# Kotstantinovskiy/SonicDiffusionBayesLab

Hardware: AMD Instinct MI355X
Metric: 512x512 images/sec at 50 DDIM steps (higher is better)
Workload: dtype bf16; 1 GPU; SD-1.5 512x512 DDIM 50 steps, CFG 7.5, batch=8/GPU (BASELINE configs[1]); global_batch=8, sample_size=64, parallelism=batch-shard x1, weights=SD-1.5-shaped synthetic seed 1234

## Files before the change

include/sd_hip.h:

```cpp
#ifndef SD_HIP_H
#define SD_HIP_H

#ifdef __cplusplus
extern "C" {
#endif

typedef struct sd_unet sd_unet;

typedef struct sd_unet_config {
    int sample_size;
    int in_channels;
    int out_channels;
    int num_levels;
    int block_out_channels[8];
    int layers_per_block;
    int attn_levels[8];
    int cross_attention_dim;
    int num_heads;
    int norm_num_groups;
    float norm_eps;
    int context_len;
    int weight_dtype;
    float fp8_act_scale_norm;
    float fp8_act_scale_ff;
// ... 26 lines not shown
long long sd_unet_workspace_bytes(sd_unet* u, int unet_batch, int cache_branch_id);

long long sd_unet_workspace_bytes_hw(sd_unet* u, int unet_batch, int cache_branch_id, int latent_h, int latent_w);

int sd_unet_set_context(sd_unet* u, void* stream, const float* encoder_hidden_states, int unet_batch,
                        int cache_branch_id, void* workspace, long long workspace_bytes);
int sd_unet_set_context_hw(sd_unet* u, void* stream, const float* encoder_hidden_states, int unet_batch,
                           int cache_branch_id, int latent_h, int latent_w, void* workspace, long long workspace_bytes);

int sd_unet_set_timestep_cond(sd_unet* u, void* stream, const float* cond);

int sd_unet_set_inpaint_cond_hw(sd_unet* u, void* stream, const float* mask, const float* masked_latents, int batch,
                                int latent_h, int latent_w);

int sd_unet_set_ip_adapter_hw(sd_unet* u, void* stream, const float* image_embeds, int unet_batch, int cache_branch_id,
                              int latent_h, int latent_w, float scale, void* workspace, long long workspace_bytes);

int sd_controlnet_create(const sd_unet_config* cfg, const int cond_embed_channels[4], sd_unet** out);
long long sd_controlnet_residual_bytes_hw(const sd_unet* u, int unet_batch, int latent_h, int latent_w);
int sd_controlnet_set_cond_hw(sd_unet* u, void* stream, const float* cond_image, int batch, int latent_h, int latent_w);
int sd_controlnet_forward_hw(sd_unet* u, void* stream, const float* latents, int latent_batch, int unet_batch, int latent_h,
                             int latent_w, float timestep, void* residuals, void* workspace, long long workspace_bytes);
int sd_unet_set_control_residuals_hw(sd_unet* u, const void* residuals, float scale, int unet_batch, int latent_h, int latent_w);

int sd_unet_set_tome(sd_unet* u, double ratio, int max_downsample);
int sd_unet_tome_block_count_hw(sd_unet* u, int latent_h, int latent_w);
int sd_unet_tome_block_info_hw(sd_unet* u, int block, int latent_h, int latent_w, int* h, int* w, int* r, long long* choice_off);
int sd_unet_set_tome_choice_hw(sd_unet* u, void* stream, const unsigned char* choice, long long n, int latent_h, int latent_w);
int sd_unet_tome_matching_hw(sd_unet* u, void* stream, int block, int unet_batch, int cache_branch_id, void* workspace, int* kept,
                             int* merged, int* dst_idx, int* tok, int* r, int* batch);

enum { SD_CACHE_OFF = 0, SD_CACHE_FULL_AND_STORE = 1, SD_CACHE_SKIP = 2 };

int sd_unet_forward(sd_unet* u, void* stream, const float* latents, int latent_batch, int unet_batch,
                    float timestep, float* eps_out, void* workspace, long long workspace_bytes, int cache_mode,
                    int cache_branch_id);
int sd_unet_forward_hw(sd_unet* u, void* stream, const float* latents, int latent_batch, int unet_batch, int latent_h,
                       int latent_w, float timestep, float* eps_out, void* workspace, long long workspace_bytes,
                       int cache_mode, int cache_branch_id);

typedef struct sd_unet sd_vae;
int sd_vae_create(const sd_unet_config* cfg, sd_vae** out);
int sd_vae_decode(sd_vae* v, void* stream, const float* latents, int batch, float latent_scale, float* images_out,
                  void* workspace, long long workspace_bytes);
int sd_vae_decode_hw(sd_vae* v, void* stream, const float* latents, int batch, int latent_h, int latent_w, float latent_scale,
                     float* images_out, void* workspace, long long workspace_bytes);

int sd_vae_encoder_create(const sd_unet_config* cfg, sd_vae** out);
int sd_vae_encode_hw(sd_vae* v, void* stream, const float* images, int batch, int latent_h, int latent_w, float* moments_out,
                     void* workspace, long long workspace_bytes);
int sd_vae_posterior_sample(void* stream, const float* moments, const float* noise_or_null, float scale, float* latents_out,
                            int batch, long long hw);

typedef struct sd_unet sd_taesd;
int sd_taesd_decoder_create(sd_taesd** out);
int sd_taesd_encoder_create(sd_taesd** out);
int sd_taesd_decode_hw(sd_taesd* v, void* stream, const float* latents, int batch, int latent_h, int latent_w, int out_mode,
                       float* images_out, void* workspace, long long workspace_bytes);
int sd_taesd_encode_hw(sd_taesd* v, void* stream, const float* images01, int batch, int latent_h, int latent_w, float* latents_out,
                       void* workspace, long long workspace_bytes);
int sd_op_conv64(void* stream, const void* X, const void* Wpacked, const float* bias, const void* R, void* Y, int B, int Hin,
                 int Win, int mode, int relu);
long long sd_op_conv64_pack(const float* w_oihw, void* out);
int sd_op_taesd_entry(void* stream, const float* x, const float* Wt, const float* bias, void* y, int B, int H, int W, int Cin,
                      int decoder);
int sd_op_taesd_exit(void* stream, const void* x, const void* Wp, const float* bias, float* y, int B, int H, int W, int Cout,
// ... 152 lines not shown
                    float eps);
int sd_op_tome_match(void* stream, const void* x, const unsigned char* choice, int B, int h, int w, int C, float* node_max,
                     int* node_idx, int* tok);
int sd_op_tome_select(void* stream, const float* node_max, const int* node_idx, int B, int num_src, int r, int* kept, int* merged,
                      int* dst_idx);
int sd_op_tome_merge(void* stream, const void* x, const int* tok, const int* kept, const int* merged, const int* dst_idx, void* out,
                     long long ldo, int B, int h, int w, int C, int r);
int sd_op_tome_unmerge(void* stream, const void* y, long long ldy, const void* residual, const int* tok, const int* kept,
                       const int* merged, const int* dst_idx, void* out, int B, int h, int w, int C, int r);
int sd_op_attention(void* stream, const void* Q, long long ldq, const void* K, long long ldk, const void* V,
                    long long ldv, void* O, long long ldo, int B, int heads, int Nq, int Nk, int D, float scale);
int sd_op_gemm_qkv_headmajor(void* stream, const void* X, long long ldx, const void* W, void* Q, void* KV, int M, int C,
                             int tokens, int K);
int sd_op_attention_headmajor(void* stream, const void* Q, long long ldq, const void* K, const void* V, void* O,
                              long long ldo, int B, int heads, int Nq, int Nk, int D, float scale);
int sd_op_clip_attention(void* stream, const void* qkv, void* out, int B, int L, int H, int heads);
int sd_op_vit_attention(void* stream, const void* qkv, void* out, int B, int L, int H, int heads);
int sd_op_bert_attention(void* stream, const void* q, long long ldq, const void* k, const void* v, long long ldkv,
                         const int* mask, void* out, long long ldo, int B, int heads, int Lq, int Lk);
int sd_op_reward_head(void* stream, const void* hidden, long long row_stride, const float* w, const float* bias, float mean,
                      float std, int B, int H, float* rewards, float* features);
int sd_op_clip_preprocess(void* stream, const unsigned char* images, int B, int H, int W, int S, int P, unsigned char* crop,
                          void* patches);
int sd_op_conv_in(void* stream, const float* x, int Bsrc, const float* Wt, const float* bias, void* y, int B, int H,
                  int W, int Cin, int Cout);
int sd_op_conv_in_cond(void* stream, const float* x, int Bsrc, const float* cond, int Bcond, const float* Wt,
                       const float* bias, void* y, int B, int H, int W, int Cout);
int sd_op_conv_in_add(void* stream, const float* x, int Bsrc, const void* addend, int Badd, const float* Wt, const float* bias,
                      void* y, int B, int H, int W, int Cout);
int sd_op_residual_add(void* stream, void* x, const long long* dst_off, const void* r, const long long* src_off,
                       const long long* count, int nseg, float scale);
int sd_op_conv_out(void* stream, const void* x, const void* Wp, const float* bias, float* y, int B, int H, int W,
                   int Cin, int Cout);
int sd_op_time_embedding(void* stream, float t, const void* W1, const float* b1, const void* W2, const float* b2,
                         float* scratch, float* temb, int dim_in, int dim);
int sd_op_timestep_cond(void* stream, float t, const float* cond, const void* Wc, float* row, float* emb, int cond_dim,
                        int dim);

int sd_op_ln_partials(int kind, int M, int N);
int sd_op_gemm_rowstats(void* stream, const void* X, long long ldx, const void* W, const float* bias, const void* R,
                        long long ldr, void* C, long long ldc, int M, int N, int K, float* rowstats);
int sd_op_gemm_ln(void* stream, const void* X, long long ldx, const void* Wg, const float* c1, const float* c2,
                  const float* rowstats, int parts, float eps, void* C, long long ldc, int M, int N, int K, int epi);
int sd_op_gemm_plan(void* stream, const void* X, long long ldx, const void* X2, long long ldx2, int K1, const void* W,
                    const float* bias, const float* bias2, const void* R, long long ldr, void* C, long long ldc, int M, int N,
                    int K, float* rowstats, float* stats, const float* ln_rs, int ln_parts, const float* ln_c1, float ln_eps,
                    void* KV, int hm_tokens);
int sd_op_xattn_fused_rowstats(void* stream, const void* X, const void* R, void* Y, const void* At, const void* Bw,
                               const float* bias, int M, int C, int rows_per_sample, int L, float* rowstats);
int sd_op_ip_xattn(void* stream, const void* R, void* Rout, const void* A, const void* Bt, const float* gamma, const float* beta,
                   float eps, long long M, int C, int rows_per_sample, int heads, int T);
int sd_op_xattn_fused(void* stream, const void* X, const void* R, void* Y, const void* At, const void* Bw,
                      const float* bias, int M, int C, int rows_per_sample, int L);
int sd_op_xattn_fused_ln(void* stream, const void* X, const void* R, void* Y, const void* At, const void* Bw,
                         const float* bias, int M, int C, int rows_per_sample, int L, const float* ln_rowstats, int ln_parts,
                         long long ln_rows, const float* c2, float eps, float* rowstats);
int sd_op_conv3x3_ablate(void* stream, const void* X, const void* W, void* Y, int B, int Hin, int Win, int Cin, int Cout,
                         int ablate);
int sd_op_xattn_fused_stamps(void* stream, const void* X, const void* R, void* Y, const void* At, const void* Bw,
                             const float* bias, int M, int C, int rows_per_sample, int L, unsigned long long* stamps);

int sd_op_gemm_fp8(void* stream, const void* X, long long ldx, const void* W, const float* wscale, float xscale,
                   const float* bias, const void* R, long long ldr, void* C, long long ldc, int M, int N, int K, int epi,
                   int out_fp8, float oscale);
int sd_op_conv3x3_fp8(void* stream, const void* X, const void* W, const float* wscale, float xscale, const float* bias,
                      const float* bias2, const void* R, void* Y, int B, int Hin, int Win, int Cin, int Cout, int stride,
// ... 13 lines not shown
```

sonicdiffusionbayeslab_amd/_lib.py:

```python
from __future__ import annotations

import ctypes as C
import os
import re
from typing import Optional

HERE = os.path.dirname(os.path.abspath(__file__))
LIB_PATH = os.environ.get("SD_AMD_LIB", os.path.join(HERE, "lib", "libsdhip.so"))
HEADER_PATH = os.path.normpath(os.path.join(HERE, "..", "include", "sd_hip.h"))

ABLATE_LIB_PATH = os.path.join(HERE, "lib", "libsdhip_ablate.so")

_lib: Optional[C.CDLL] = None
_ablate: Optional[C.CDLL] = None


class SdUnetConfig(C.Structure):
    _fields_ = [
        ("sample_size", C.c_int), ("in_channels", C.c_int), ("out_channels", C.c_int),
        ("num_levels", C.c_int), ("block_out_channels", C.c_int * 8), ("layers_per_block", C.c_int),
        ("attn_levels", C.c_int * 8), ("cross_attention_dim", C.c_int), ("num_heads", C.c_int),
        ("norm_num_groups", C.c_int), ("norm_eps", C.c_float), ("context_len", C.c_int),
        ("weight_dtype", C.c_int), ("fp8_act_scale_norm", C.c_float), ("fp8_act_scale_ff", C.c_float),
        ("time_cond_proj_dim", C.c_int),
# ... 36 lines not shown
        ("intermediate_size", C.c_int), ("max_positions", C.c_int), ("layer_norm_eps", C.c_float), ("hidden_act", C.c_int),
        ("position_embedding_absolute", C.c_int), ("max_text_len", C.c_int), ("reward_mean", C.c_float), ("reward_std", C.c_float),
    ]


class SdHipError(RuntimeError):
    pass


def declared_symbols() -> list:
    src = open(HEADER_PATH).read()
    src = re.sub(r"/\*.*?\*/", "", src, flags=re.S)
    return sorted(set(re.findall(r"\b(sd_[a-z0-9_]+)\s*\(", src)))


_vp, _i, _ll, _f = C.c_void_p, C.c_int, C.c_longlong, C.c_float
_SIGS = {
    "sd_last_error": (C.c_char_p, []),
    "sd_abi_version": (_i, []),
    "sd_unet_create": (_i, [C.POINTER(SdUnetConfigFull), C.POINTER(_vp)]),
    "sd_unet_destroy": (None, [_vp]),
    "sd_unet_num_params": (_i, [_vp]),
    "sd_unet_param_info": (_i, [_vp, _i, C.c_char_p, _i, C.POINTER(_ll), C.POINTER(_i)]),
    "sd_unet_load_param": (_i, [_vp, C.c_char_p, _vp, _ll]),
    "sd_unet_finalize": (_i, [_vp]),
    "sd_unet_debug_packed": (_ll, [_vp, C.c_char_p, _vp, _ll]),
    "sd_unet_calibrate_fp8": (_i, [_vp, _vp, _vp, _i, _i, _f, _f, _vp, _ll]),
    "sd_unet_fp8_scale_count": (_i, [_vp]),
    "sd_unet_fp8_scale_info": (_i, [_vp, _i, C.c_char_p, _i, C.POINTER(_f), C.POINTER(_f)]),
    "sd_unet_set_fp8_scale": (_i, [_vp, C.c_char_p, _f]),
    "sd_unet_workspace_bytes": (_ll, [_vp, _i, _i]),
    "sd_unet_set_context": (_i, [_vp, _vp, _vp, _i, _i, _vp, _ll]),
    "sd_unet_set_timestep_cond": (_i, [_vp, _vp, _vp]),
    "sd_unet_forward": (_i, [_vp, _vp, _vp, _i, _i, _f, _vp, _vp, _ll, _i, _i]),
    "sd_unet_workspace_bytes_hw": (_ll, [_vp, _i, _i, _i, _i]),
    "sd_unet_set_context_hw": (_i, [_vp, _vp, _vp, _i, _i, _i, _i, _vp, _ll]),
    "sd_unet_forward_hw": (_i, [_vp, _vp, _vp, _i, _i, _i, _i, _f, _vp, _vp, _ll, _i, _i]),
    "sd_unet_forward_profiled": (_i, [_vp, _vp, _vp, _i, _i, _f, _vp, _vp, _ll, _i, _i, C.POINTER(C.c_double),
                                      C.POINTER(_ll), C.POINTER(C.c_double), C.POINTER(C.c_double)]),
    "sd_unet_forward_op_times": (_ll, [_vp, _vp, _vp, _i, _i, _f, _vp, _vp, _ll, _i, _i, C.c_char_p, _ll]),
    "sd_vae_create": (_i, [C.POINTER(SdUnetConfigFull), C.POINTER(_vp)]),
    "sd_vae_decode": (_i, [_vp, _vp, _vp, _i, _f, _vp, _vp, _ll]),
    "sd_vae_decode_hw": (_i, [_vp, _vp, _vp, _i, _i, _i, _f, _vp, _vp, _ll]),
    "sd_vae_encoder_create": (_i, [C.POINTER(SdUnetConfigFull), C.POINTER(_vp)]),
    "sd_vae_encode_hw": (_i, [_vp, _vp, _vp, _i, _i, _i, _vp, _vp, _ll]),
    "sd_vae_posterior_sample": (_i, [_vp, _vp, _vp, _f, _vp, _i, _ll]),
    "sd_taesd_decoder_create": (_i, [C.POINTER(_vp)]),
    "sd_taesd_encoder_create": (_i, [C.POINTER(_vp)]),
    "sd_taesd_decode_hw": (_i, [_vp, _vp, _vp, _i, _i, _i, _i, _vp, _vp, _ll]),
    "sd_taesd_encode_hw": (_i, [_vp, _vp, _vp, _i, _i, _i, _vp, _vp, _ll]),
    "sd_op_conv64": (_i, [_vp, _vp, _vp, _vp, _vp, _vp, _i, _i, _i, _i, _i]),
    "sd_op_conv64_pack": (_ll, [_vp, _vp]),
    "sd_op_taesd_entry": (_i, [_vp, _vp, _vp, _vp, _vp, _i, _i, _i, _i, _i]),
    "sd_op_taesd_exit": (_i, [_vp, _vp, _vp, _vp, _vp, _i, _i, _i, _i, _i]),
    "sd_clip_create": (_i, [C.POINTER(SdClipConfig), C.POINTER(_vp)]),
    "sd_clip_encode": (_i, [_vp, _vp, _vp, _i, _vp, _vp, _ll]),
    "sd_clip_create_projected": (_i, [C.POINTER(SdClipConfig), _i, _i, C.POINTER(_vp)]),
    "sd_clip_text_embeds_workspace_bytes": (_ll, [_vp, _i]),
    "sd_clip_text_embeds": (_i, [_vp, _vp, _vp, _i, _vp, _vp, _ll]),
    "sd_clip_vision_create": (_i, [C.POINTER(SdClipVisionConfig), C.POINTER(_vp)]),
    "sd_clip_vision_workspace_bytes": (_ll, [_vp, _i, _i, _i]),
    "sd_clip_vision_encode": (_i, [_vp, _vp, _vp, _i, _i, _i, _vp, _vp, _ll]),
    "sd_clip_score": (_i, [_vp, _vp, _vp, _i, _i, _vp, _vp]),
    "sd_image_reward_create": (_i, [C.POINTER(SdImageRewardConfig), C.POINTER(_vp)]),
    "sd_image_reward_workspace_bytes": (_ll, [_vp, _i, _i, _i]),
    "sd_image_reward_score": (_i, [_vp, _vp, _vp, _vp, _vp, _i, _i, _i, _i, _vp, _vp, _vp, _ll]),
# ... 29 lines not shown
    "sd_controlnet_create": (_i, [C.POINTER(SdUnetConfigFull), C.POINTER(_i), C.POINTER(_vp)]),
    "sd_controlnet_residual_bytes_hw": (_ll, [_vp, _i, _i, _i]),
    "sd_controlnet_set_cond_hw": (_i, [_vp, _vp, _vp, _i, _i, _i]),
    "sd_controlnet_forward_hw": (_i, [_vp, _vp, _vp, _i, _i, _i, _i, _f, _vp, _vp, _ll]),
    "sd_unet_set_control_residuals_hw": (_i, [_vp, _vp, _f, _i, _i, _i]),
    "sd_op_conv_in_add": (_i, [_vp, _vp, _i, _vp, _i, _vp, _vp, _vp, _i, _i, _i, _i]),
    "sd_op_residual_add": (_i, [_vp, _vp, _vp, _vp, _vp, _vp, _i, _f]),
    "sd_op_conv_in_cond": (_i, [_vp, _vp, _i, _vp, _i, _vp, _vp, _vp, _i, _i, _i, _i]),
    "sd_op_gemm": (_i, [_vp, _vp, _ll, _vp, _ll, _i, _vp, _vp, _vp, _vp, _ll, _vp, _ll, _i, _i, _i, _i]),
    "sd_op_gemm_tile_rows": (_i, [_i, _i, _i]),
    "sd_op_gemm_splitk": (_i, [_i, _i, _i, _i]),
    "sd_op_gemm_batched": (_i, [_vp, _vp, _ll, _vp, _ll, _i, _vp, _vp, _ll, _vp, _ll, _i, _i, _i, _i, _i]),
    "sd_op_gemm_batched_softmax_ln": (_i, [_vp, _vp, _ll, _vp, _ll, _i, _vp, _ll, _i, _i, _i, _i, _vp, _i, _vp, _vp, _f]),
    "sd_op_conv3x3": (_i, [_vp, _vp, _vp, _vp, _vp, _vp, _vp, _i, _i, _i, _i, _i, _i, _i]),
    "sd_op_conv3x3_shortcut": (_i, [_vp, _vp, _vp, _vp, _vp, _i, _vp, _i, _vp, _vp, _i, _i, _i, _i, _i]),
    "sd_op_conv3x3_shortcut_groupnorm": (_i, [_vp, _vp, _vp, _vp, _vp, _i, _vp, _i, _vp, _vp, _i, _i, _i, _i, _i,
                                              _vp, _vp, _vp, _i, _f, _i]),
    "sd_op_conv3x3_down_asym": (_i, [_vp, _vp, _vp, _vp, _vp, _i, _i, _i, _i, _i]),
    "sd_op_conv3x3_ablate": (_i, [_vp, _vp, _vp, _vp, _i, _i, _i, _i, _i, _i]),
    "sd_op_conv3x3_upsample_subpixel": (_i, [_vp, _vp, _vp, _vp, _vp, _i, _i, _i, _i, _i]),
    "sd_op_conv3x3_upsample_subpixel_groupnorm": (_i, [_vp, _vp, _vp, _vp, _vp, _i, _i, _i, _i, _i, _vp, _vp, _vp, _i, _f, _i]),
    "sd_op_groupnorm": (_i, [_vp, _vp, _i, _vp, _i, _vp, _vp, _vp, _i, _i, _i, _f, _i]),
    "sd_op_conv3x3_groupnorm": (_i, [_vp, _vp, _vp, _vp, _vp, _vp, _vp, _i, _i, _i, _i, _i, _vp, _vp, _vp, _i, _f, _i]),
    "sd_op_conv3x3_splitk": (_i, [_i, _i, _i, _i, _i, _i, _i]),
    "sd_op_conv3x3_kernel": (_i, [_i, _i, _i, _i, _i, _i, _i, _i]),
    "sd_op_softmax_rows": (_i, [_vp, _vp, _ll, _i, _f]),
    "sd_op_layernorm": (_i, [_vp, _vp, _vp, _vp, _vp, _i, _i, _f]),
    "sd_op_attention": (_i, [_vp, _vp, _ll, _vp, _ll, _vp, _ll, _vp, _ll, _i, _i, _i, _i, _i, _f]),
    "sd_op_gemm_qkv_headmajor": (_i, [_vp, _vp, _ll, _vp, _vp, _vp, _i, _i, _i, _i]),
    "sd_op_attention_headmajor": (_i, [_vp, _vp, _ll, _vp, _vp, _vp, _ll, _i, _i, _i, _i, _i, _f]),
    "sd_op_clip_attention": (_i, [_vp, _vp, _vp, _i, _i, _i, _i]),
    "sd_op_conv_in": (_i, [_vp, _vp, _i, _vp, _vp, _vp, _i, _i, _i, _i, _i]),
    "sd_op_conv_out": (_i, [_vp, _vp, _vp, _vp, _vp, _i, _i, _i, _i, _i]),
    "sd_op_time_embedding": (_i, [_vp, _f, _vp, _vp, _vp, _vp, _vp, _vp, _i, _i]),
    "sd_op_timestep_cond": (_i, [_vp, _f, _vp, _vp, _vp, _vp, _i, _i]),
    "sd_op_ln_partials": (_i, [_i, _i, _i]),
    "sd_op_gemm_rowstats": (_i, [_vp, _vp, _ll, _vp, _vp, _vp, _ll, _vp, _ll, _i, _i, _i, _vp]),
    "sd_op_gemm_plan": (_i, [_vp, _vp, _ll, _vp, _ll, _i, _vp, _vp, _vp, _vp, _ll, _vp, _ll, _i, _i, _i, _vp, _vp, _vp, _i, _vp, _f,
                            _vp, _i]),
    "sd_op_gemm_ln": (_i, [_vp, _vp, _ll, _vp, _vp, _vp, _vp, _i, _f, _vp, _ll, _i, _i, _i, _i]),
    "sd_op_xattn_fused_rowstats": (_i, [_vp, _vp, _vp, _vp, _vp, _vp, _vp, _i, _i, _i, _i, _vp]),
    "sd_op_xattn_fused": (_i, [_vp, _vp, _vp, _vp, _vp, _vp, _vp, _i, _i, _i, _i]),
    "sd_op_xattn_fused_ln": (_i, [_vp, _vp, _vp, _vp, _vp, _vp, _vp, _i, _i, _i, _i, _vp, _i, _ll, _vp, _f, _vp]),
    "sd_op_xattn_fused_stamps": (_i, [_vp, _vp, _vp, _vp, _vp, _vp, _vp, _i, _i, _i, _i, _vp]),
    "sd_op_gemm_fp8": (_i, [_vp, _vp, _ll, _vp, _vp, _f, _vp, _vp, _ll, _vp, _ll, _i, _i, _i, _i, _i, _f]),
    "sd_op_conv3x3_fp8": (_i, [_vp, _vp, _vp, _vp, _f, _vp, _vp, _vp, _vp, _i, _i, _i, _i, _i, _i, _i]),
    "sd_op_groupnorm_fp8": (_i, [_vp, _vp, _i, _vp, _i, _vp, _vp, _vp, _i, _i, _i, _f, _i, _i, _f]),
    "sd_op_layernorm_fp8": (_i, [_vp, _vp, _vp, _vp, _vp, _i, _i, _i, _f, _f]),
    "sd_op_quantize_fp8": (_i, [_vp, _vp, _vp, _ll, _i, _i, _f]),
    "sd_op_amax_e4m3": (_i, [_vp, _vp, _ll, _vp]),
    "sd_unet_set_tome": (_i, [_vp, C.c_double, _i]),
    "sd_unet_tome_block_count_hw": (_i, [_vp, _i, _i]),
    "sd_unet_tome_block_info_hw": (_i, [_vp, _i, _i, _i, C.POINTER(_i), C.POINTER(_i), C.POINTER(_i), C.POINTER(_ll)]),
    "sd_unet_set_tome_choice_hw": (_i, [_vp, _vp, _vp, _ll, _i, _i]),
    "sd_unet_tome_matching_hw": (_i, [_vp, _vp, _i, _i, _i, _vp, _vp, _vp, _vp, _vp, C.POINTER(_i), C.POINTER(_i)]),
    "sd_op_tome_match": (_i, [_vp, _vp, _vp, _i, _i, _i, _i, _vp, _vp, _vp]),
    "sd_op_tome_select": (_i, [_vp, _vp, _vp, _i, _i, _i, _vp, _vp, _vp]),
    "sd_op_tome_merge": (_i, [_vp, _vp, _vp, _vp, _vp, _vp, _vp, _ll, _i, _i, _i, _i, _i]),
    "sd_op_tome_unmerge": (_i, [_vp, _vp, _ll, _vp, _vp, _vp, _vp, _vp, _vp, _i, _i, _i, _i, _i]),
}


def load() -> C.CDLL:
    global _lib
    if _lib is not None:
        return _lib
# ... 42 lines not shown
```

sonicdiffusionbayeslab_amd/csrc/common.h:

```cpp
#pragma once
#include <hip/hip_runtime.h>
#include <stdint.h>

typedef unsigned short bf16_t;

typedef __attribute__((ext_vector_type(8))) short bf16x8;
typedef __attribute__((ext_vector_type(4))) short bf16x4;
typedef __attribute__((ext_vector_type(4))) float f32x4;
typedef __attribute__((ext_vector_type(16))) float f32x16;
typedef __attribute__((ext_vector_type(2))) __bf16 bf16x2_t;
typedef __attribute__((ext_vector_type(2))) float f32x2_t;
typedef __attribute__((ext_vector_type(4))) unsigned u32x4;
typedef __attribute__((ext_vector_type(2))) unsigned u32x2;

typedef __attribute__((ext_vector_type(8))) int i32x8;
typedef __attribute__((ext_vector_type(8))) unsigned u32x8;
__device__ __forceinline__ i32x8 cat_u32x4(u32x4 lo, u32x4 hi) {
    const u32x8 r = __builtin_shufflevector(lo, hi, 0, 1, 2, 3, 4, 5, 6, 7);
    return __builtin_bit_cast(i32x8, r);
}

#define LDS_PTR(p) ((__attribute__((address_space(3))) void*)(p))
#define GLB_PTR(p) ((const __attribute__((address_space(1))) void*)(p))

__device__ __forceinline__ float bf2f(bf16_t u) { return __builtin_bit_cast(float, (unsigned)u << 16); }
__device__ __forceinline__ float bflo(unsigned u) { return __builtin_bit_cast(float, u << 16); }
__device__ __forceinline__ float bfhi(unsigned u) { return __builtin_bit_cast(float, u & 0xffff0000u); }
__device__ __forceinline__ bf16_t f2bf(float f) {
    __bf16 b = (__bf16)f;
    return __builtin_bit_cast(bf16_t, b);
}
__device__ __forceinline__ unsigned pack2bf(float lo, float hi) {
    f32x2_t v = {lo, hi};
    bf16x2_t r = __builtin_convertvector(v, bf16x2_t);
    return __builtin_bit_cast(unsigned, r);
}

__device__ __forceinline__ unsigned pack4fp8(float a, float b, float c, float d) {
    a = __builtin_amdgcn_fmed3f(a, -448.f, 448.f); b = __builtin_amdgcn_fmed3f(b, -448.f, 448.f);
    c = __builtin_amdgcn_fmed3f(c, -448.f, 448.f); d = __builtin_amdgcn_fmed3f(d, -448.f, 448.f);
    const int r = __builtin_amdgcn_cvt_pk_fp8_f32(a, b, 0, false);
    return (unsigned)__builtin_amdgcn_cvt_pk_fp8_f32(c, d, r, true);
}

__device__ __forceinline__ void glds16(const void* gsrc, void* lds_wave_base) {
    __builtin_amdgcn_global_load_lds(GLB_PTR(gsrc), LDS_PTR(lds_wave_base), 16, 0, 0);
}

__device__ __forceinline__ float silu_f(float x) {
    return x * __builtin_amdgcn_rcpf(1.0f + __builtin_amdgcn_exp2f(-1.4426950408889634f * x));
}
__device__ __forceinline__ float gelu_erf_f(float x) {
    const float z = fabsf(x) * 0.70710678118654752f;
    const float t = __builtin_amdgcn_rcpf(__builtin_fmaf(0.47047f, z, 1.0f));
    const float poly = t * (0.3480242f + t * (-0.0958798f + t * 0.7478556f));
    const float e = __builtin_amdgcn_exp2f(z * z * -1.4426950408889634f);
    const float half_erfc = 0.5f * poly * e;
    const float phi = x < 0.f ? half_erfc : 1.0f - half_erfc;
    return x * phi;
}

__device__ __forceinline__ f32x2_t geglu_pair(f32x2_t value, f32x2_t gate) {
    constexpr float C = 4.35f;
    const f32x2_t xc = {__builtin_amdgcn_fmed3f(gate[0], -C, C), __builtin_amdgcn_fmed3f(gate[1], -C, C)};
    const f32x2_t t = xc * (1.0f / C);
    const f32x2_t u = t * t;
    auto k = [](float c) { return f32x2_t{c, c}; };
    f32x2_t p = __builtin_elementwise_fma(u, k(-8.173780021e-01f), k(4.634953387e+00f));
    p = __builtin_elementwise_fma(p, u, k(-1.175370409e+01f));
    p = __builtin_elementwise_fma(p, u, k(1.781238736e+01f));
    p = __builtin_elementwise_fma(p, u, k(-1.828480159e+01f));
    p = __builtin_elementwise_fma(p, u, k(1.371556223e+01f));
    p = __builtin_elementwise_fma(p, u, k(-7.893326951e+00f));
    p = __builtin_elementwise_fma(p, u, k(3.560156552e+00f));
    p = __builtin_elementwise_fma(p, u, k(-1.257849752e+00f));
    p = __builtin_elementwise_fma(p, u, k(3.989407778e-01f));
    const f32x2_t phi = __builtin_elementwise_fma(xc, p, k(0.5f));
    return value * gate * phi;
}

template <int SHR>
__device__ __forceinline__ float row_shr_add(float v) {
    const int sh = __builtin_amdgcn_update_dpp(0, __builtin_bit_cast(int, v), 0x110 + SHR, 0xf, 0xf, true);
    return v + __builtin_bit_cast(float, sh);
// ... 102 lines not shown
```

sonicdiffusionbayeslab_amd/csrc/kernels.h:

```cpp
#pragma once
#include <vector>

#include "common.h"

struct GemmArgs {
    const bf16_t* X = nullptr;
    long ldx = 0;
    const bf16_t* X2 = nullptr;
    long ldx2 = 0;
    int K1 = 0;
    const bf16_t* W = nullptr;
    long ldw = 0;
    const float* bias = nullptr;
    const float* bias2 = nullptr;
    const bf16_t* R = nullptr;
    long ldr = 0;
    bf16_t* C = nullptr;
    long ldc = 0;
    int M = 0, N = 0, K = 0;
    int Hin = 0, Win = 0, Cin = 0, Hout = 0, Wout = 0, stride = 1, up = 0;
    int asym = 0;
    int splitk = 1;
    float* slab = nullptr;
    int defer_reduce = 0;
// ... 46 lines not shown
    const float* bias = nullptr;
    const bf16_t* R = nullptr;
    bf16_t* Y = nullptr;
    int B = 0, Hin = 0, Win = 0;
    int mode = 0;
    int relu = 0;
    int Hout = 0, Wout = 0, tiles_y = 0, tiles_x = 0, ntiles = 0;
    unsigned xbytes = 0;
};
int sd_conv64_out_size(int in, int mode);
void sd_conv64_pack(const float* w_oihw , bf16_t* out);
int sd_launch_conv64(const Conv64Args& a, hipStream_t stream);
int sd_launch_taesd_entry(const float* x, const float* Wt, const float* bias, bf16_t* y, int B, int H, int W, int Cin, int decoder,
                          hipStream_t stream);
int sd_launch_taesd_exit(const bf16_t* x, const bf16_t* Wp, const float* bias, float* y, int B, int H, int W, int Cout, int out_mode,
                         hipStream_t stream);

struct GroupNormArgs {
    const bf16_t* x1 = nullptr; int C1 = 0;
    const bf16_t* x2 = nullptr; int C2 = 0;
    const float* gamma = nullptr; const float* beta = nullptr;
    bf16_t* y = nullptr;
    int out_fp8 = 0, Cpad = 0;
    float oscale = 1.0f;
    const float* stats1 = nullptr; const float* stats2 = nullptr;
    const float* slab = nullptr; int splitk = 0;
    const float* sbias = nullptr; const float* sbias2 = nullptr;
    const bf16_t* sR = nullptr; long sldr = 0;
    bf16_t* x1w = nullptr;
    float* partial = nullptr;
    int B = 0, HW = 0, groups = 32, nsplit = 0;
    float eps = 1e-5f;
    int silu = 0;
};
int sd_groupnorm_nsplit(int B, int HW);
bool sd_groupnorm_uses_small(int B, int HW, int C1, int C2, int groups);
bool sd_groupnorm_slab_ok(int B, int HW, int C1, int C2, int groups);
size_t sd_groupnorm_scratch_bytes(int B, int HW, int groups);
int sd_launch_groupnorm(const GroupNormArgs& a, hipStream_t stream);

int sd_launch_softmax_rows(bf16_t* s, long rows, int cols, float scale, hipStream_t stream);
int sd_launch_softmax_rows_long(bf16_t* s, long rows, int cols, float scale, hipStream_t stream);
int sd_launch_pqconv(const float* x, const float* W, const float* bias, float* y, int B, int HW, float in_scale,
                     hipStream_t stream);

int sd_launch_layernorm(const bf16_t* x, const float* gamma, const float* beta, bf16_t* y, int rows, int C,
                        float eps, hipStream_t stream);
int sd_launch_layernorm_fp8(const bf16_t* x, const float* gamma, const float* beta, void* y, int rows, int C, int Cpad,
                            float eps, float oscale, hipStream_t stream);
int sd_launch_amax_e4m3(const void* y, long nbytes, unsigned* out, hipStream_t stream);
int sd_launch_quantize_fp8(const bf16_t* x, void* y, long rows, int C, int Cpad, float scale, hipStream_t stream);

struct AttnArgs {
    const bf16_t* Q = nullptr; long ldq = 0;
    const bf16_t* K = nullptr; long ldk = 0;
    const bf16_t* V = nullptr; long ldv = 0;
    bf16_t* O = nullptr; long ldo = 0;
    int B = 0, heads = 0, Nq = 0, Nk = 0, D = 0;
    float scale = 0.f;
    const void* consts = nullptr;
    int kv_head_major = 0;
    int q_prescaled = 0;
    int xcd_order = 1;
};
int sd_launch_attention(const AttnArgs& a, hipStream_t stream);

int sd_launch_gemv(const float* x, const bf16_t* W, const float* b, float* y, int N, int K, int silu_in,
                   hipStream_t stream);
int sd_launch_timestep_sinusoid(float t, float* out, int dim, hipStream_t stream);
int sd_launch_timestep_sinusoid_row(float t, const float* row, float* out, int dim, hipStream_t stream);
int sd_launch_f32_to_bf16(const float* src, bf16_t* dst, long n, hipStream_t stream);
int sd_launch_transpose_bf16(const bf16_t* src, bf16_t* dst, int B, int R, int Cc, hipStream_t stream, int perm16 = 0);

int sd_launch_retile32(const bf16_t* src, bf16_t* dst, int B, int R, int K, int RT, hipStream_t stream);
int sd_launch_replicate(const void* src, void* dst, long bytes, int rep, hipStream_t stream);

int sd_tome_check(int h, int w, int C, const char* who);
int sd_launch_tome_partition(const unsigned char* choice, int h, int w, int* tok, hipStream_t stream);
int sd_launch_tome_match(const bf16_t* x, const unsigned char* choice, int B, int h, int w, int C, float* node_max, int* node_idx,
                         int* tok, float* inv, hipStream_t stream);
int sd_launch_tome_select(const float* node_max, const int* node_idx, int B, int num_src, int r, int* kept, int* merged, int* dst_idx,
                          hipStream_t stream);
int sd_launch_tome_merge(const bf16_t* x, const int* tok, const int* kept, const int* merged, const int* dst_idx, bf16_t* out,
                         long ldo, int B, int h, int w, int C, int r, hipStream_t stream);
int sd_launch_tome_unmerge(const bf16_t* y, long ldy, const bf16_t* residual, const int* tok, const int* kept, const int* merged,
                           const int* dst_idx, bf16_t* out, int B, int h, int w, int C, int r, hipStream_t stream);

struct XattnArgs {
    const bf16_t* X = nullptr;
    const bf16_t* R = nullptr;
    bf16_t* Y = nullptr;
    const bf16_t* At = nullptr;
    const bf16_t* Bw = nullptr;
    const float* bias = nullptr;
    int M = 0, C = 0, rows_per_sample = 0, L = 0;
    float* rowstats = nullptr;
    const float* ln_rs = nullptr; int ln_np = 0; long ln_rows = 0;
    const float* ln_c2 = nullptr;
    float ln_eps = 1e-5f;
    unsigned long long* stamps = nullptr;
};
bool sd_xattn_fused_applicable(int rows_per_sample, int C, int heads, int L);
// ... 23 lines not shown
                        hipStream_t stream);
int sd_launch_vit_attention(const bf16_t* qkv, bf16_t* out, int B, int L, int H, int heads, hipStream_t stream);
int sd_launch_pool_rows(const bf16_t* src, const int* ids, int B, int L, int H, int eos_id, bf16_t* dst, hipStream_t stream);
int sd_launch_clip_score(const float* img, const float* txt, int B, int P, float* raw, float* score, hipStream_t stream);

int sd_bert_attention_check(int B, int Lq, int Lk, int heads);
int sd_bert_mask_check(const int* host_mask, int B, int Lk);
int sd_launch_bert_attention(const bf16_t* q, long ldq, const bf16_t* k, const bf16_t* v, long ldkv, const int* mask, bf16_t* out,
                             long ldo, int B, int heads, int Lq, int Lk, hipStream_t stream);
int sd_launch_reward_head(const bf16_t* hidden, long row_stride, const float* w, const float* wb, float mean, float stdv, int B,
                          int H, float* rewards, float* features, hipStream_t stream);

int sd_launch_conv_in(const float* x, int Bsrc, const float* Wt , const float* bias,
                      bf16_t* y, int B, int H, int W, int Cin, int Cout, hipStream_t stream);
int sd_launch_conv_in_cond(const float* x, int Bsrc, const float* cond, int Bcond, const float* Wt, const float* bias,
                           bf16_t* y, int B, int H, int W, int Cout, hipStream_t stream);
constexpr int SD_MAX_RES_SEGMENTS = 16;
int sd_launch_conv_in_add(const float* x, int Bsrc, const bf16_t* addend, int Badd, const float* Wt, const float* bias,
                          bf16_t* y, int B, int H, int W, int Cout, hipStream_t stream);
int sd_launch_residual_add(bf16_t* const* x, const bf16_t* const* r, const long* n, int nseg, float scale, hipStream_t stream);
int sd_launch_nchw_to_nhwc_bf16(const float* src, bf16_t* dst, int B, int C, long hw, hipStream_t stream);
int sd_launch_inpaint_cond_pack(const float* mask, const float* masked, float* cond, int B, long hw, hipStream_t stream);
int sd_launch_inpaint_prepare(const float* img, const float* mask, float* masked, float* lmask, int B, int H, int W,
                              hipStream_t stream);
int sd_launch_conv_in_image(const float* img, const float* Wt , const float* bias, bf16_t* y, int B, int H,
                            int W, int Cout, hipStream_t stream);
int sd_launch_vae_enc_out(const bf16_t* x, const bf16_t* Wp , const float* bias, const float* Wq ,
                          const float* bq, float* y, int B, int H, int W, int Cin, hipStream_t stream);
int sd_launch_vae_posterior(const float* moments, const float* noise, float scale, float* z, int B, int C, long hw,
                            hipStream_t stream);
int sd_launch_conv_out(const bf16_t* x, const bf16_t* Wp , const float* bias, float* y, int B,
                       int H, int W, int Cin, int Cout, hipStream_t stream);

struct StepCoef {
    float px, pe, p1, p2, pn;
    float yx, ye;
    float mx, me;
    float p3;
};
int sd_launch_sched_step(const float* eps, int cfg, float guidance, const float* x, const float* m1,
                         const float* m2, const float* m3, const float* noise, float* prev, float* y2, float* m_out,
                         StepCoef c, long n, hipStream_t stream);
int sd_launch_cfg_rescale_factors(const float* eps, int batch, long n_per_sample, float guidance, float rescale, float* k_out,
                                  hipStream_t stream);
int sd_launch_sched_step_rescaled(const float* eps, int cfg, float guidance, const float* x, const float* m1,
                                  const float* m2, const float* m3, const float* noise, float* prev, float* y2,
                                  float* m_out, StepCoef c, const float* k, long n_per_sample, long n, hipStream_t stream);
int sd_launch_sched_step_inpaint(const float* eps, int cfg, float guidance, const float* x, const float* m1,
                                 const float* m2, const float* m3, const float* noise, float* prev, float* y2,
                                 float* m_out, StepCoef c, const float* k, long n_per_sample, long n, const float* init,
                                 const float* blend_noise, const float* mask, float a, float s, long hw, hipStream_t stream);

int sd_launch_inception_conv(const bf16_t* x, const bf16_t* w, const float* bias, bf16_t* y, int B, int Hin, int Win, int Cin,
                             int Cout, int kh, int kw, int stride, int ph, int pw, int ldy, int coff, int relu ,
                             hipStream_t stream);
int sd_launch_inception_pool(const bf16_t* x, bf16_t* y, int B, int H, int W, int C, int stride, int pad, int avg, int ldy,
                             int coff, hipStream_t stream);
int sd_launch_inception_mean(const bf16_t* x, float* out, int B, int HW, int C, hipStream_t stream);
int sd_launch_inception_resize(const unsigned char* img, void* out, int B, int H, int W, int S, int out_fp32, hipStream_t stream);
```

sonicdiffusionbayeslab_amd/csrc/model.h:

```cpp
#pragma once
#include "../../include/sd_hip.h"
#include "common.h"
#include "kernels.h"

#include <stdlib.h>
#include <string.h>
#include <sys/mman.h>

#include <algorithm>
#include <map>
#include <new>
#include <set>
#include <string>
#include <tuple>
#include <unordered_map>
#include <vector>

namespace sdhip {

constexpr size_t NOFF = (size_t)-1;
constexpr int T_LATENTS = -2, T_EPS = -3;
constexpr int MAX_CONTROL_RES = SD_MAX_RES_SEGMENTS;

struct ParamSpec {
// ... 27 lines not shown
    size_t w = NOFF, b = NOFF, g = NOFF, be = NOFF;
    long b2idx = 0;
    int M = 0, N = 0, K = 0, K1 = 0, epi = 0;
    int B = 0, Hin = 0, Win = 0, Cin = 0, Hout = 0, Wout = 0, stride = 1, up = 0;
    int C1 = 0, C2 = 0, HW = 0, silu = 0, nsplit = 0;
    float eps = 0.f;
    int heads = 0, D = 0, Nq = 0, Nk = 0;
    long ldq = 0, ldk = 0, ldv = 0, ldo = 0, qoff = 0, koff = 0, voff = 0;
    int silu_in = 0, splitk = 1;
    int pool_by_ids = 0;
    int key_mask = 0;
    int defer = 0, slab_t = -1, slab_k = 0, slab_r = -1, slab_b2t = -1;
    size_t slab_b = NOFF;
    long slab_b2idx = 0;
    int wt = -1;
    size_t wx = NOFF;
    long xoff = 0, woff_el = 0, coff = 0, ldx_o = 0, ldw_o = 0, ldc_o = 0;
    float scale = 0.f;
    long wbs = 0;
    int rpb = 0, sm_valid = 0;
    int dt = 0, out_fp8 = 0, Cpad = 0, Kalg = 0;
    int sname = -1;
    int stats = -1, s1 = -1, s2 = -1;
    int subpix = 0;
    int asym = 0;
    int hm = 0;
    int qps = 0;
    int rs = -1, lnrs = -1, lnnp = 0;
    size_t c1 = NOFF;
    size_t wsc = NOFF;
    float xs = 1.f, os = 1.f;
    int scx1 = -1, scx2 = -1, scc1 = 0, scc2 = 0;
    size_t scw = NOFF;
    int nres = 0;
    int res_t[MAX_CONTROL_RES];
    int nwrap = 0;
    Wrap wraps[3];
};

struct HostBlob {
    unsigned char* p = nullptr;
    size_t n = 0, cap = 0;
    unsigned char* data() { return p; }
    const unsigned char* data() const { return p; }
    size_t size() const { return n; }
    bool empty() const { return n == 0; }
    bool reserve(size_t bytes) {
        if (bytes <= cap) return true;
        void* q = mmap(nullptr, bytes, PROT_READ | PROT_WRITE, MAP_PRIVATE | MAP_ANONYMOUS | MAP_POPULATE, -1, 0);
        if (q == MAP_FAILED) return false;
        (void)madvise(q, bytes, MADV_HUGEPAGE);
        if (p) { memcpy(q, p, n); munmap(p, cap); }
        p = (unsigned char*)q; cap = bytes;
        return true;
    }
    void resize(size_t bytes) {
        if (bytes > cap && !reserve(std::max(bytes, cap * 2))) throw std::bad_alloc();
        n = bytes;
    }
    void release() { if (p) munmap(p, cap); p = nullptr; n = cap = 0; }
    ~HostBlob() { release(); }
    HostBlob() = default;
    HostBlob(const HostBlob&) = delete;
    HostBlob& operator=(const HostBlob&) = delete;
};

struct Tn {
    size_t bytes = 0;
    int def = -1, last = -1;
    bool persistent = false;
    bool ctx = false;
    bool ctx_ip = false;
    size_t off = NOFF;
};

struct Plan {
    int UB = 0, branch = -1;
    int rep = 1;
    int lh = 0, lw = 0;
    int ip = 0;
    struct IpFold { int at, bt, C; size_t wqT, wo, wkv; int heads; };
    std::vector<IpFold> ip_fold;
    int ip_e = -1, ip_proj = -1, ip_tok = -1, ip_kv = -1;
    int cn = 0;
    std::vector<size_t> cn_off;
    std::vector<long> cn_count;
    struct TomeBlock { int tok, kept, merged, dst_idx, B, h, w, r; long choice_off; };
    std::vector<TomeBlock> tome;
    long tome_choice_bytes = 0;
    std::vector<Tn> tensors;
    std::vector<Op> ops;
    std::vector<char> skipped;
    std::vector<int> ctx_kv;
    std::vector<size_t> ctx_w;
    std::vector<int> ctx_c;
    int ctx_bf16 = -1;
    struct Fold { int kv, at, bw, C, heads; size_t wqT, wo; bool perm; int c2 = -1; size_t lnu = NOFF; int c1 = -1; size_t ones = NOFF; };
    std::vector<Fold> ctx_fold;
    int ctx_fold_scratch = -1;
    std::map<std::string, int> taps;
    size_t total_bytes = 0;
    ClipPrepGeom geom;
    std::vector<int> prep_tab;
    const int* dtab = nullptr;
};

}

struct sd_unet {
    int kind = 0;
    sd_unet_config cfg;
    sd_clip_config clip;
    sd_clip_vision_config vis;
    sd_image_reward_config ir;
    const int* ir_ids = nullptr;
    const int* ir_mask = nullptr;
    float* ir_features = nullptr;
    int text_proj = 0;
    int eos_id = -1;
    std::map<std::pair<int, int>, int*> prep_tabs;
    std::vector<sdhip::ParamSpec> params;
    std::unordered_map<std::string, int> pindex;
    std::unordered_map<std::string, size_t> woff;
    sdhip::HostBlob hblob;
    char* dweights = nullptr;
    bool finalized = false;
    bool debug_taps = false;
    bool fp8 = false;
    float s_norm = 8.f, s_ff = 2.f;
    std::vector<std::string> act_names;
    std::unordered_map<std::string, int> act_index;
    std::vector<float> act_scale, act_amax;
    int act_id(const std::string& name, float dflt) {
        auto it = act_index.find(name);
        if (it != act_index.end()) return it->second;
        act_index[name] = (int)act_names.size();
        act_names.push_back(name); act_scale.push_back(dflt); act_amax.push_back(0.f);
        return (int)act_names.size() - 1;
    }
    std::map<std::tuple<int, int, int, int, int, int, int, long long, int>, sdhip::Plan> plans;
    int last_rep = 1, last_ip = 0, last_cn = 0;
    int last_h = 0, last_w = 0;
    std::unordered_map<std::string, long> tproj_off;
    long tproj_total = 0;
    float* dcond = nullptr;
    bool cond_set = false;
    float* dinpaint = nullptr;
    size_t inpaint_cap = 0;
    int inpaint_b = 0, inpaint_h = 0, inpaint_w = 0;
    std::set<std::tuple<int, int, int, int>> ip_keys;
    const char* ctrl_res = nullptr;
    float ctrl_scale = 0.f;
    int ctrl_ub = 0, ctrl_h = 0, ctrl_w = 0;
    bool ctrl_enabled = false;
    bf16_t* cn_embed = nullptr;
    char* cn_scratch = nullptr;
    size_t cn_embed_cap = 0, cn_scratch_cap = 0;
    int cn_b = 0, cn_h = 0, cn_w = 0;
    int cond_embed[4] = {0, 0, 0, 0};
    double tome_ratio = 0.0;
    int tome_max_downsample = 0;
    unsigned char* tome_choice = nullptr;
    size_t tome_choice_cap = 0;
    long tome_choice_n = 0;
    bool unet_like() const { return kind == 0 || kind == 5; }
};

namespace sdhip {

inline int level_heads(const sd_unet_config& c, int level) {
    return c.num_heads_per_level[level] > 0 ? c.num_heads_per_level[level] : c.num_heads;
}
inline int block_heads(const sd_unet_config& c, const std::string& p) {
    if (p.compare(0, 12, "down_blocks.") == 0) return level_heads(c, atoi(p.c_str() + 12));
    if (p.compare(0, 10, "up_blocks.") == 0) return level_heads(c, c.num_levels - 1 - atoi(p.c_str() + 10));
    return level_heads(c, c.num_levels - 1);
}

void enumerate_params(sd_unet* u);
// ... 37 lines not shown
```

sonicdiffusionbayeslab_amd/csrc/norm.hip:

```cpp
#include "common.h"
#include "kernels.h"

#include <stdlib.h>

#include <algorithm>
#include <type_traits>

namespace {

struct GnGeom {
    int nchunks, rows_par, threads, cpg, C;
};

__host__ __device__ inline GnGeom gn_geom(int C, int groups) {
    GnGeom g;
    g.C = C;
    g.nchunks = C / 8;
    g.rows_par = g.nchunks >= 256 ? 1 : 256 / g.nchunks;
    const int act = g.rows_par * g.nchunks;
    g.threads = (act + 63) / 64 * 64;
    g.cpg = C / groups;
    return g;
}

// ... 97 lines not shown
    for (int i = tid; i < total; i += 256) {
        const int blk = i / cpg, c = gi * cpg + (i - blk * cpg);
        const long gb = (long)b * nblk + blk;
        const f32x2_t v = *(const f32x2_t*)(c < a.C1 ? a.stats1 + (gb * a.C1 + c) * 2 : a.stats2 + (gb * a.C2 + (c - a.C1)) * 2);
        s += v[0];
        q += v[1];
    }
    s = wave_sum(s);
    q = wave_sum(q);
    if (lane == 0) { red[wave * 2] = s; red[wave * 2 + 1] = q; }
    __syncthreads();
    if (tid == 0) {
        s = (red[0] + red[2]) + (red[4] + red[6]);
        q = (red[1] + red[3]) + (red[5] + red[7]);
        const float cnt = (float)a.HW * (float)cpg;
        const float mean = s / cnt;
        const float var = fmaxf(q / cnt - mean * mean, 0.f);
        float* st = a.partial + (long)a.B * a.nsplit * a.groups * 2 + (long)idx * 2;
        st[0] = mean;
        st[1] = rsqrtf(var + a.eps);
    }
}

template <bool SILU, bool FP8>
__global__ void gn_apply_kernel(const GroupNormArgs a) {
    const GnGeom g = gn_geom(a.C1 + a.C2, a.groups);
    const int tid = threadIdx.x;
    const int split = blockIdx.x, b = blockIdx.y;
    const bool active = tid < g.rows_par * g.nchunks;
    if (!active) return;
    const int prow = tid / g.nchunks, ch = tid - prow * g.nchunks;
    const int c0 = ch * 8;
    const float* st = a.partial + (long)a.B * a.nsplit * a.groups * 2 + (long)b * a.groups * 2;
    const int g0 = c0 / g.cpg, g1 = (c0 + 7) / g.cpg;
    const int nb = min(8, (g0 + 1) * g.cpg - c0);
    const float m0 = st[g0 * 2], r0 = st[g0 * 2 + 1], m1 = st[g1 * 2], r1 = st[g1 * 2 + 1];
    float sc[8], sf[8];
    {
        const f32x4 ga = *(const f32x4*)(a.gamma + c0), gb = *(const f32x4*)(a.gamma + c0 + 4);
        const f32x4 ba = *(const f32x4*)(a.beta + c0), bb = *(const f32x4*)(a.beta + c0 + 4);
#pragma unroll
        for (int j = 0; j < 8; ++j) {
            const float gm = j < 4 ? ga[j & 3] : gb[j & 3], bt = j < 4 ? ba[j & 3] : bb[j & 3];
            const float mean = j < nb ? m0 : m1, rstd = j < nb ? r0 : r1;
            sc[j] = rstd * gm;
            sf[j] = bt - mean * sc[j];
        }
    }
    const int per = (a.HW + a.nsplit - 1) / a.nsplit;
    const int pbeg = split * per, pend = min(a.HW, pbeg + per);
    auto apply = [&](const u32x4 v, long pix) {
        float f[8] = {bflo(v[0]), bfhi(v[0]), bflo(v[1]), bfhi(v[1]),
                      bflo(v[2]), bfhi(v[2]), bflo(v[3]), bfhi(v[3])};
#pragma unroll
        for (int j = 0; j < 8; ++j) {
            f[j] = f[j] * sc[j] + sf[j];
            if (SILU) f[j] = silu_f(f[j]);
        }
        if (FP8) {
            char* yr = (char*)a.y + pix * a.Cpad;
            const u32x2 o = {pack4fp8(f[0] * a.oscale, f[1] * a.oscale, f[2] * a.oscale, f[3] * a.oscale),
                             pack4fp8(f[4] * a.oscale, f[5] * a.oscale, f[6] * a.oscale, f[7] * a.oscale)};
            *(u32x2*)(yr + c0) = o;
            if (ch == g.nchunks - 1)
                for (int k = g.C; k < a.Cpad; k += 16) *(u32x4*)(yr + k) = u32x4{0u, 0u, 0u, 0u};
            return;
        }
        u32x4 o = {pack2bf(f[0], f[1]), pack2bf(f[2], f[3]), pack2bf(f[4], f[5]), pack2bf(f[6], f[7])};
        *(u32x4*)(a.y + pix * g.C + c0) = o;
    };
    const long base = (long)b * a.HW;
    const int rp = g.rows_par;
    int p = pbeg + prow;
    for (; p + 3 * rp < pend; p += 4 * rp) {
        const u32x4 v0 = *(const u32x4*)gn_src(a, base + p, c0);
        const u32x4 v1 = *(const u32x4*)gn_src(a, base + p + rp, c0);
        const u32x4 v2 = *(const u32x4*)gn_src(a, base + p + 2 * rp, c0);
        const u32x4 v3 = *(const u32x4*)gn_src(a, base + p + 3 * rp, c0);
        apply(v0, base + p); apply(v1, base + p + rp); apply(v2, base + p + 2 * rp); apply(v3, base + p + 3 * rp);
    }
    for (; p < pend; p += rp) apply(*(const u32x4*)gn_src(a, base + p, c0), base + p);
}

__device__ __forceinline__ float2 gn_unit_sums(const u32x2 v) {
    const float f0 = bflo(v[0]), f1 = bfhi(v[0]), f2 = bflo(v[1]), f3 = bfhi(v[1]);
    return make_float2((f0 + f1) + (f2 + f3), (f0 * f0 + f1 * f1) + (f2 * f2 + f3 * f3));
}
__device__ __forceinline__ void gn_mean_rstd(float ts, float tq, float cnt, float eps, float& mean, float& rstd) {
    mean = ts / cnt;
    rstd = rsqrtf(fmaxf(tq / cnt - mean * mean, 0.f) + eps);
}
template <bool SILU, bool FP8>
__device__ __forceinline__ void gn_unit_store(const GroupNormArgs& a, const u32x2 v, float mean, float rstd, long pix, int c, int C) {
    const f32x4 gm = *(const f32x4*)(a.gamma + c), bt = *(const f32x4*)(a.beta + c);
    float f[4] = {bflo(v[0]), bfhi(v[0]), bflo(v[1]), bfhi(v[1])};
#pragma unroll
    for (int jj = 0; jj < 4; ++jj) {
        f[jj] = (f[jj] - mean) * rstd * gm[jj] + bt[jj];
        if (SILU) f[jj] = silu_f(f[jj]);
    }
    if (FP8) {
        *(unsigned*)((char*)a.y + pix * a.Cpad + c) = pack4fp8(f[0] * a.oscale, f[1] * a.oscale, f[2] * a.oscale, f[3] * a.oscale);
// ... 400 lines not shown
    SD_REQUIRE(s && rows > 0, "softmax_rows: empty");
    SD_REQUIRE(cols % 8 == 0 && cols > 0 && cols <= 4096, "softmax_rows: cols=%d must be a multiple of 8 and <= 4096", cols);
    hipLaunchKernelGGL(softmax_rows_kernel, dim3((unsigned)((rows + 3) / 4)), dim3(256), 0, stream, s, rows, cols, scale);
    SD_CHECK_HIP(hipGetLastError());
    return 0;
}

size_t sd_groupnorm_scratch_bytes(int B, int HW, int groups) {
    return ((size_t)B * sd_groupnorm_nsplit(B, HW) * groups * 2 + (size_t)B * groups * 2) * sizeof(float);
}

int sd_groupnorm_nsplit(int B, int HW) {
    int n = (2048 + B - 1) / B;
    if (n > HW / 8) n = HW / 8;
    if (n < 1) n = 1;
    if (n > 256) n = 256;
    return n;
}

bool sd_groupnorm_uses_small(int B, int HW, int C1, int C2, int groups) {
    static const bool no_small = getenv("SD_GN_NO_SMALL") != nullptr;
    const int C = C1 + C2;
    return !no_small && HW <= 256 && (long)HW * (C / groups) <= 10240 && (C / groups) % 4 == 0 && C1 % 4 == 0 && B <= 65535;
}

bool sd_groupnorm_slab_ok(int B, int HW, int C1, int C2, int groups) {
    if (!sd_groupnorm_uses_small(B, HW, C1, C2, groups)) return false;
    const int cpg = (C1 + C2) / groups, G = cpg >= 80 ? 1 : 80 / cpg;
    return cpg >= 20 && cpg <= 80 && groups % G == 0 && C2 % 4 == 0 && (long)B * HW * C1 < (1L << 29);
}

int sd_launch_groupnorm(const GroupNormArgs& a, hipStream_t stream) {
    const int C = a.C1 + a.C2;
    SD_REQUIRE(a.x1 && a.y && a.gamma && a.beta && a.partial, "groupnorm: null operand");
    SD_REQUIRE(!a.out_fp8 || (a.Cpad >= C && a.Cpad % 128 == 0 && C % 16 == 0 && a.oscale > 0.f),
               "groupnorm fp8 out: Cpad=%d must be a multiple of 128 >= C=%d (C a multiple of 16)", a.Cpad, C);
    SD_REQUIRE(a.C1 % 8 == 0 && a.C2 % 8 == 0 && (a.C2 == 0 || a.x2), "groupnorm: C1=%d C2=%d must be multiples of 8", a.C1, a.C2);
    SD_REQUIRE(a.groups > 0 && a.groups <= 64 && C % a.groups == 0 && (C / a.groups >= 8 || C / a.groups == 4),
               "groupnorm: C=%d groups=%d needs C/groups >= 8 (or == 4)", C, a.groups);
    SD_REQUIRE(a.nsplit >= 1 && a.nsplit <= a.HW && a.B > 0 && a.HW > 0, "groupnorm: bad split %d for HW=%d", a.nsplit, a.HW);
    const GnGeom g = gn_geom(C, a.groups);
    SD_REQUIRE(g.threads <= 1024, "groupnorm: C=%d too wide", C);
    if (a.slab) {
        const int cpg = C / a.groups, G = cpg >= 80 ? 1 : 80 / cpg, ncol = G * (cpg / 4);
        SD_REQUIRE(a.splitk > 1 && a.splitk <= 64 && a.x1w && !a.out_fp8 && (!a.sR || a.sldr >= a.C1) && (a.C2 == 0 || a.x2),
                   "groupnorm with a deferred split-K reduce: splitk=%d, bf16 output, x1w and a residual stride >= C1", a.splitk);
        SD_REQUIRE(sd_groupnorm_slab_ok(a.B, a.HW, a.C1, a.C2, a.groups), "groupnorm with a deferred split-K reduce: HW=%d C=%d+%d "
                   "is not a shape gn_slab_kernel takes", a.HW, a.C1, a.C2);
        const dim3 grid(a.groups / G, a.B), blk((32 * ncol + 63) / 64 * 64);
        const size_t smem = ((size_t)G * a.HW * (cpg / 4) + 4 * G) * sizeof(float2);
        auto go = [&](auto kern) { hipLaunchKernelGGL(kern, grid, blk, smem, stream, a); };
        auto pick = [&](auto mi, auto un) {
            constexpr int MI = decltype(mi)::value, UN = decltype(un)::value;
            if (a.silu) go(gn_slab_kernel<true, MI, UN>); else go(gn_slab_kernel<false, MI, UN>);
        };
        using std::integral_constant;
        const int iters = (a.HW + 31) / 32, k = a.splitk;
        if (iters <= 2) {
            if (k % 8 == 0) pick(integral_constant<int, 2>{}, integral_constant<int, 8>{});
            else if (k % 4 == 0) pick(integral_constant<int, 2>{}, integral_constant<int, 4>{});
            else if (k % 2 == 0) pick(integral_constant<int, 2>{}, integral_constant<int, 2>{});
            else pick(integral_constant<int, 2>{}, integral_constant<int, 1>{});
        } else if (iters <= 4) {
            if (k % 4 == 0) pick(integral_constant<int, 4>{}, integral_constant<int, 4>{});
            else if (k % 2 == 0) pick(integral_constant<int, 4>{}, integral_constant<int, 2>{});
            else pick(integral_constant<int, 4>{}, integral_constant<int, 1>{});
        } else {
            if (k % 2 == 0) pick(integral_constant<int, 8>{}, integral_constant<int, 2>{});
            else pick(integral_constant<int, 8>{}, integral_constant<int, 1>{});
        }
        SD_CHECK_HIP(hipGetLastError());
        return 0;
    }
    if (sd_groupnorm_uses_small(a.B, a.HW, a.C1, a.C2, a.groups)) {
        const int units = (a.HW * (C / a.groups / 4) + 255) / 256;
        const dim3 grid(a.groups, a.B);
        auto go = [&](auto kern) { hipLaunchKernelGGL(kern, grid, dim3(256), 0, stream, a); };
        auto pick = [&](auto mu) {
            constexpr int MU = decltype(mu)::value;
            if (a.out_fp8) { if (a.silu) go(gn_small_kernel<true, true, MU>); else go(gn_small_kernel<false, true, MU>); }
            else { if (a.silu) go(gn_small_kernel<true, false, MU>); else go(gn_small_kernel<false, false, MU>); }
        };
        if (units <= 3) pick(std::integral_constant<int, 3>{});
        else if (units <= 5) pick(std::integral_constant<int, 5>{});
        else pick(std::integral_constant<int, 10>{});
        SD_CHECK_HIP(hipGetLastError());
        return 0;
    }
    dim3 grid(a.nsplit, a.B);
    if (a.stats1 != nullptr) {
        SD_REQUIRE(a.HW % 64 == 0 && (a.C2 == 0 || a.stats2 != nullptr), "groupnorm: producer statistics need HW %% 64 == 0 and both sources");
        hipLaunchKernelGGL(gn_finalize_stats_kernel, dim3(a.B * a.groups), dim3(256), 0, stream, a);
    } else {
        hipLaunchKernelGGL(gn_stats_kernel, grid, dim3(g.threads), (g.threads + g.nchunks) * sizeof(float4), stream, a);
        hipLaunchKernelGGL(gn_finalize_kernel, dim3((a.B * a.groups + 3) / 4), dim3(256), 0, stream, a);
    }
    if (a.out_fp8) {
        if (a.silu) hipLaunchKernelGGL((gn_apply_kernel<true, true>), grid, dim3(g.threads), 0, stream, a);
        else hipLaunchKernelGGL((gn_apply_kernel<false, true>), grid, dim3(g.threads), 0, stream, a);
    } else {
        if (a.silu) hipLaunchKernelGGL((gn_apply_kernel<true, false>), grid, dim3(g.threads), 0, stream, a);
        else hipLaunchKernelGGL((gn_apply_kernel<false, false>), grid, dim3(g.threads), 0, stream, a);
    }
    SD_CHECK_HIP(hipGetLastError());
    return 0;
}

static int launch_layernorm(const bf16_t* x, const float* gamma, const float* beta, bf16_t* y, int rows, int C, float eps,
                            bool fp8, int Cpad, float oscale, hipStream_t stream) {
    SD_REQUIRE(x && y && gamma && beta, "layernorm: null operand");
    SD_REQUIRE(C % 8 == 0 && C > 0 && C <= 1536, "layernorm: C=%d must be a multiple of 8 and <= 1536", C);
    SD_REQUIRE(rows > 0, "layernorm: no rows");
    SD_REQUIRE(!fp8 || (Cpad == (C + 127) / 128 * 128 && C % 16 == 0 && oscale > 0.f && Cpad - C <= 64 * 16),
               "layernorm fp8 out: Cpad=%d must be C=%d rounded up to 128 (C a multiple of 16)", Cpad, C);
    auto grouped = [&](auto kern, int lpr) {
        const int rows_per_block = 4 * (64 / lpr);
        hipLaunchKernelGGL(kern, dim3((rows + rows_per_block - 1) / rows_per_block), dim3(256), 0, stream, x, gamma, beta, y,
                           rows, eps, oscale);
    };
    if (fp8) {
        if (C == 320) grouped(layernorm_grouped_kernel<8, true>, 8);
        else if (C == 640) grouped(layernorm_grouped_kernel<16, true>, 16);
        else if (C == 1280) grouped(layernorm_grouped_kernel<32, true>, 32);
        else
            hipLaunchKernelGGL(layernorm_kernel<true>, dim3((rows + 3) / 4), dim3(256), 0, stream, x, gamma, beta, y, rows, C,
                               eps, Cpad, oscale);
    } else {
        if (C == 320) grouped(layernorm_grouped_kernel<8, false>, 8);
        else if (C == 640) grouped(layernorm_grouped_kernel<16, false>, 16);
// ... 38 lines not shown
```

sonicdiffusionbayeslab_amd/csrc/ops.hip:

```cpp
#include "model.h"

#include <stdlib.h>

namespace sdhip {

static void* g_scratch = nullptr;
static size_t g_scratch_bytes = 0;
void* op_scratch(size_t bytes) {
    if (bytes > g_scratch_bytes) {
        (void)hipDeviceSynchronize();
        if (g_scratch) (void)hipFree(g_scratch);
        g_scratch = nullptr;
        g_scratch_bytes = 0;
        if (hipMalloc(&g_scratch, bytes) != hipSuccess) return nullptr;
        g_scratch_bytes = bytes;
    }
    return g_scratch;
}

}

using namespace sdhip;

static void conv3x3_args(GemmArgs& a, const void* X, const void* W, const float* bias, const float* bias2, const void* R, void* Y,
// ... 410 lines not shown
                                  const float* bias, void* y, int B, int H, int W, int Cout) {
    return sd_launch_conv_in_cond(x, Bsrc, cond, Bcond, Wt, bias, (bf16_t*)y, B, H, W, Cout, (hipStream_t)stream);
}

extern "C" int sd_op_conv_in_add(void* stream, const float* x, int Bsrc, const void* addend, int Badd, const float* Wt,
                                 const float* bias, void* y, int B, int H, int W, int Cout) {
    return sd_launch_conv_in_add(x, Bsrc, (const bf16_t*)addend, Badd, Wt, bias, (bf16_t*)y, B, H, W, Cout, (hipStream_t)stream);
}

extern "C" int sd_op_residual_add(void* stream, void* x, const long long* dst_off, const void* r, const long long* src_off,
                                  const long long* count, int nseg, float scale) {
    SD_REQUIRE(x && r && dst_off && src_off && count, "sd_op_residual_add: null argument");
    SD_REQUIRE(nseg >= 1 && nseg <= MAX_CONTROL_RES, "sd_op_residual_add: %d segments (1 .. %d)", nseg, MAX_CONTROL_RES);
    bf16_t* xs[MAX_CONTROL_RES];
    const bf16_t* rs[MAX_CONTROL_RES];
    long n[MAX_CONTROL_RES];
    for (int k = 0; k < nseg; ++k) {
        SD_REQUIRE(dst_off[k] >= 0 && src_off[k] >= 0 && count[k] > 0, "sd_op_residual_add: segment %d", k);
        xs[k] = (bf16_t*)x + dst_off[k]; rs[k] = (const bf16_t*)r + src_off[k]; n[k] = (long)count[k];
    }
    return sd_launch_residual_add(xs, rs, n, nseg, scale, (hipStream_t)stream);
}

extern "C" int sd_op_conv_in(void* stream, const float* x, int Bsrc, const float* Wt, const float* bias, void* y, int B,
                             int H, int W, int Cin, int Cout) {
    return sd_launch_conv_in(x, Bsrc, Wt, bias, (bf16_t*)y, B, H, W, Cin, Cout, (hipStream_t)stream);
}

extern "C" int sd_op_conv_out(void* stream, const void* x, const void* Wp, const float* bias, float* y, int B, int H,
                              int W, int Cin, int Cout) {
    return sd_launch_conv_out((const bf16_t*)x, (const bf16_t*)Wp, bias, y, B, H, W, Cin, Cout, (hipStream_t)stream);
}

extern "C" int sd_op_time_embedding(void* stream, float t, const void* W1, const float* b1, const void* W2,
                                    const float* b2, float* scratch, float* temb, int dim_in, int dim) {
    int rc;
    if ((rc = sd_launch_timestep_sinusoid(t, scratch, dim_in, (hipStream_t)stream))) return rc;
    if ((rc = sd_launch_gemv(scratch, (const bf16_t*)W1, b1, scratch + dim_in, dim, dim_in, 0, (hipStream_t)stream))) return rc;
    return sd_launch_gemv(scratch + dim_in, (const bf16_t*)W2, b2, temb, dim, dim, 1, (hipStream_t)stream);
}

extern "C" int sd_op_timestep_cond(void* stream, float t, const float* cond, const void* Wc, float* row, float* emb,
                                   int cond_dim, int dim) {
    SD_REQUIRE(cond && Wc && row && emb, "timestep_cond: null operand");
    SD_REQUIRE(((uintptr_t)cond & 15) == 0 && cond_dim > 0, "timestep_cond: cond must be 16-byte aligned, cond_dim > 0");
    int rc;
    if ((rc = sd_launch_gemv(cond, (const bf16_t*)Wc, nullptr, row, dim, cond_dim, 0, (hipStream_t)stream))) return rc;
    return sd_launch_timestep_sinusoid_row(t, row, emb, dim, (hipStream_t)stream);
}

extern "C" int sd_op_gemm_fp8(void* stream, const void* X, long long ldx, const void* W, const float* wscale, float xscale,
                              const float* bias, const void* R, long long ldr, void* C, long long ldc, int M, int N, int K,
                              int epi, int out_fp8, float oscale) {
    if (ensure_zero_page()) return -2;
    SD_REQUIRE(epi == 0 || epi == 1, "sd_op_gemm_fp8: epi %d (0 = std, 1 = GEGLU)", epi);
    SD_REQUIRE(xscale > 0.f && (!out_fp8 || (epi == 1 && oscale > 0.f)), "sd_op_gemm_fp8: bad scales / fp8 output needs the GEGLU epilogue");
    GemmArgs a;
    a.X = (const bf16_t*)X; a.ldx = ldx; a.K1 = K; a.W = (const bf16_t*)W; a.bias = bias; a.R = (const bf16_t*)R; a.ldr = ldr;
    a.C = (bf16_t*)C; a.ldc = ldc; a.M = M; a.N = N; a.K = K; a.zero_page = zero_page();
    a.dt = 1; a.wscale = wscale; a.xscale_inv = 1.0f / xscale; a.out_fp8 = out_fp8; a.oscale = oscale;
    a.splitk = epi ? 1 : op_gemm_splitk(M, N, K, 1);
    if (splitk_slab(a, "sd_op_gemm_fp8")) return -1;
    return sd_launch_gemm(a, epi, (hipStream_t)stream);
}

extern "C" int sd_op_conv3x3_fp8(void* stream, const void* X, const void* W, const float* wscale, float xscale,
// ... 119 lines not shown
```

sonicdiffusionbayeslab_amd/csrc/plan.hip:

```cpp
#include "model.h"

#include <stdlib.h>

namespace sdhip {

namespace {

struct Builder {
    sd_unet* u;
    Plan& pl;
    int UB;
    std::vector<Wrap> wrapstack;
    std::map<int, int> stats_of;
    std::map<int, float> tscale;
    static std::string stem(const std::string& key) {
        const size_t n = key.rfind(".weight");
        return n == std::string::npos ? key : key.substr(0, n);
    }
    std::string error;
    float xscale(int t) {
        auto it = tscale.find(t);
        if (it == tscale.end()) {
            if (error.empty()) error = "fp8 consumer of a tensor without a scale";
            return 1.0f;
// ... 34 lines not shown
    int ctx_tensor(size_t bytes) {
        const int id = tensor(bytes, true);
        pl.tensors[id].ctx = true;
        return id;
    }
    int ctx_ip_tensor(size_t bytes) {
        const int id = ctx_tensor(bytes);
        pl.tensors[id].ctx_ip = true;
        return id;
    }
    int tensor(size_t bytes, bool persistent = false) {
        Tn t;
        t.bytes = (bytes + 255) / 256 * 256;
        t.persistent = persistent;
        pl.tensors.push_back(t);
        return (int)pl.tensors.size() - 1;
    }
    size_t W(const std::string& k) {
        auto it = u->woff.find(k);
        if (it == u->woff.end()) {
            if (error.empty()) error = "missing packed weight " + k;
            return 0;
        }
        return it->second;
    }
    Op& push(Op op) {
        op.nwrap = (int)wrapstack.size();
        for (int i = 0; i < op.nwrap; ++i) op.wraps[i] = wrapstack[i];
        pl.ops.push_back(op);
        return pl.ops.back();
    }
    static int pad128(int c) { return (c + 127) / 128 * 128; }
    int gn(int x1, int c1, int x2, int c2, int hw, const std::string& g, const std::string& b, float eps, int silu,
           bool fq = false) {
        Op o; o.kind = OP_GN; o.x1 = x1; o.C1 = c1; o.x2 = x2; o.C2 = c2; o.HW = hw; o.B = UB;
        o.g = W(g); o.be = W(b); o.eps = eps; o.silu = silu;
        o.nsplit = sd_groupnorm_nsplit(UB, hw);
        o.aux = tensor(sd_groupnorm_scratch_bytes(UB, hw, u->cfg.norm_num_groups));
        if (hw % 64 == 0 && !sd_groupnorm_uses_small(UB, hw, c1, c2, u->cfg.norm_num_groups) && stats_of.count(x1) &&
            (x2 < 0 || stats_of.count(x2))) {
            o.s1 = stats_of[x1];
            o.s2 = x2 >= 0 ? stats_of[x2] : -1;
        }
        if (fq) {
            o.out_fp8 = 1; o.Cpad = pad128(c1 + c2); o.sname = u->act_id(stem(g), u->s_norm); o.os = u->act_scale[o.sname];
            o.out = tensor((size_t)UB * hw * o.Cpad); tscale[o.out] = o.os;
        } else o.out = tensor((size_t)UB * hw * (c1 + c2) * 2);
        push(o);
        return o.out;
    }
    int conv3(int x, int hin, int win, int cin, int cout, int stride, int up, const std::string& w, const std::string& b,
              long b2idx, int b2t, int r, bool fq = false) {
        Op o; o.kind = OP_CONV3; o.x1 = x; o.B = UB; o.Hin = hin; o.Win = win; o.Cin = cin; o.N = cout;
        o.stride = stride; o.up = up;
        o.Hout = ((hin << up) + 2 - 3) / stride + 1;
        o.Wout = ((win << up) + 2 - 3) / stride + 1;
        o.M = UB * o.Hout * o.Wout; o.K = 9 * cin; o.Kalg = o.K;
        o.b = W(b); o.b2t = b2t; o.b2idx = b2idx; o.r = r;
        if (fq) { o.dt = 1; o.Cin = pad128(cin); o.K = 9 * o.Cin; o.w = W(w + ".fp8"); o.wsc = W(w + ".scale"); o.xs = xscale(x); }
        else o.w = W(w);
        static const bool subpix_off = getenv("SD_CONV_SUBPIXEL") && atoi(getenv("SD_CONV_SUBPIXEL")) == 0;
        if (up && !fq && !subpix_off && u->kind == 0 && stride == 1 && r < 0 && b2t < 0 && (hin * win) % 64 == 0 &&
            u->woff.count(w + ".sub")) {
            o.subpix = 1; o.K = 4 * cin; o.Kalg = 4 * cin;
            o.w = W(w + ".sub"); o.splitk = 1;
            o.out = tensor((size_t)o.M * cout * 2);
            if ((hin * win) % 128 == 0) want_stats(o, o.M, cout);
            push(o);
            return o.out;
        }
        o.splitk = sd_conv3x3_splitk(o.M, o.N, o.Cin, hin, win, stride, up, o.dt);
        if (o.splitk > 1) o.aux = tensor((size_t)o.splitk * o.M * o.N * 4);
        o.out = tensor((size_t)o.M * cout * 2);
        GemmArgs g;
        g.M = o.M; g.N = o.N; g.Cin = o.Cin; g.K = o.K; g.ldw = o.K; g.Hin = hin; g.Win = win; g.Hout = o.Hout; g.Wout = o.Wout;
        g.stride = stride; g.up = up; g.dt = o.dt;
        if (sd_conv_halo_mode(g) != 2) want_stats(o, o.M, cout);
        push(o);
        return o.out;
    }
    int gemm(int x1, int k1, int x2, int k2, int M, int N, const std::string& w, const std::string& b, int r, int epi,
             bool fq = false, const std::string& oname = "") {
        Op o; o.kind = OP_GEMM; o.x1 = x1; o.x2 = x2; o.K1 = k1; o.K = k1 + k2; o.Kalg = o.K; o.M = M; o.N = N; o.epi = epi;
        o.b = b.empty() ? NOFF : W(b); o.r = r;
        if (fq) { o.dt = 1; o.K = o.K1 = pad128(k1); o.w = W(w + ".fp8"); o.wsc = W(w + ".scale"); o.xs = xscale(x1); }
        else o.w = W(w);
        o.splitk = epi ? 1 : sd_gemm_splitk(M, N, o.dt ? o.K / 2 : o.K, o.dt ? 128 : 0);
        if (o.splitk > 1) o.aux = tensor((size_t)o.splitk * M * N * 4);
        if (!oname.empty()) {
            o.out_fp8 = 1; o.sname = u->act_id(oname, u->s_ff); o.os = u->act_scale[o.sname]; o.Cpad = pad128(N / 2);
            o.out = tensor((size_t)M * o.Cpad); tscale[o.out] = o.os;
        } else o.out = tensor((size_t)M * (epi ? N / 2 : N) * 2);
        push(o);
        return o.out;
    }
    int ln(int x, int M, int C, const std::string& g, const std::string& b, bool fq = false, float eps = 1e-5f) {
        Op o; o.kind = OP_LN; o.x1 = x; o.M = M; o.N = C; o.g = W(g); o.be = W(b); o.eps = eps;
        if (fq) {
            o.out_fp8 = 1; o.Cpad = pad128(C); o.sname = u->act_id(stem(g), u->s_norm); o.os = u->act_scale[o.sname];
            o.out = tensor((size_t)M * o.Cpad); tscale[o.out] = o.os;
        } else o.out = tensor((size_t)M * C * 2);
        push(o);
        return o.out;
    }
    int attn(int q, long qoff, long ldq, int kv, long koff, long voff, long ldkv, int nq, int nk, int C, int heads) {
        Op o; o.kind = OP_ATTN; o.x1 = q; o.x2 = kv; o.qoff = qoff; o.koff = koff; o.voff = voff;
        o.ldq = ldq; o.ldk = o.ldv = ldkv; o.ldo = C; o.B = UB; o.heads = heads; o.D = C / heads;
        o.Nq = nq; o.Nk = nk;
        o.out = tensor((size_t)UB * nq * C * 2);
        push(o);
        return o.out;
    }
    bool shortcut_fuse = !(getenv("SD_SHORTCUT_FUSE") && atoi(getenv("SD_SHORTCUT_FUSE")) == 0);
    int resnet(const std::string& p, int x1, int c1, int x2, int c2, int cout, int rh, int rw, int tproj_t) {
        const int hw = rh * rw, cin = c1 + c2, M = UB * hw;
        const bool fq = u->fp8;
        int t1 = gn(x1, c1, x2, c2, hw, p + "norm1.weight", p + "norm1.bias", u->cfg.norm_eps, 1, fq);
        int t2 = conv3(t1, rh, rw, cin, cout, 1, 0, p + "conv1.weight", p + "conv1.bias", u->tproj_off.at(p), tproj_t, -1, fq);
        int t3 = gn(t2, cout, -1, 0, hw, p + "norm2.weight", p + "norm2.bias", u->cfg.norm_eps, 1, fq);
        int sc = x1;
        if (cin != cout) {
            GemmArgs g;
            g.M = M; g.N = cout; g.Cin = cout; g.K = 9 * cout; g.ldw = g.K; g.Hin = g.Hout = rh; g.Win = g.Wout = rw;
            g.Csc1 = c1; g.Csc2 = x2 >= 0 ? c2 : 0;
            if (shortcut_fuse && !fq && u->unet_like() && u->woff.count(p + "conv2.bias+shortcut") && sd_conv_halo_shortcut_applicable(g)) {
                const int out = conv3(t3, rh, rw, cout, cout, 1, 0, p + "conv2.weight", p + "conv2.bias+shortcut", 0, -1, -1, fq);
                Op& o = pl.ops.back();
                o.scx1 = x1; o.scc1 = c1; o.scx2 = x2; o.scc2 = g.Csc2; o.scw = W(p + "conv_shortcut.weight");
                o.Kalg += cin;
                return out;
            }
            sc = gemm(x1, c1, x2, c2, M, cout, p + "conv_shortcut.weight", p + "conv_shortcut.bias", -1, 0);
        }
        return conv3(t3, rh, rw, cout, cout, 1, 0, p + "conv2.weight", p + "conv2.bias", 0, -1, sc, fq);
    }
    int tome_r(int rh, int rw, int C) {
        if (u->kind != 0 || u->fp8 || !(u->tome_ratio > 0.0) || rh <= 0 || pl.lh / rh > u->tome_max_downsample) return 0;
        const int N = rh * rw;
        if (rh % 2 || rw % 2 || N > 16384 || C % 64 || C > 1536) {
            if (error.empty()) error = "Token Merging needs even token-grid sides, at most 16384 tokens and C a multiple of 64 up to 1536 on "
                                       "every merging level (" + std::to_string(rh) + "x" + std::to_string(rw) + ", C = " + std::to_string(C) + ")";
            return 0;
        }
        return std::min(N - N / 4, (int)((double)N * u->tome_ratio));
    }
    int n_transformers = 0;
// ... 391 lines not shown
    void build_image_reward() {
        int Lv = 0;
        const int img = build_blip_vision(&Lv);
        if (img < 0) return;
        pl.taps["image_tokens"] = img;
        build_blip_text(img, Lv);
    }

    void build() {
        if (u->kind == 6) { build_image_reward(); return; }
        if (u->kind == 1) { build_vae(); return; }
        if (u->kind == 2) { build_clip(); return; }
        if (u->kind == 3) { build_vit(); return; }
        if (u->kind == 4) { build_vae_encoder(); return; }
        const sd_unet_config& c = u->cfg;
        const int nl = c.num_levels, c0 = c.block_out_channels[0], temb = 4 * c0;
        const int L = c.context_len;
        pl.ctx_bf16 = ctx_tensor((size_t)UB * L * c.cross_attention_dim * 2);
        size_t fold_max = 0;
        for (int i = 0; i < nl; ++i)
            if (c.attn_levels[i] || i == nl - 1) fold_max = std::max(fold_max, (size_t)level_heads(c, i) * 80 * c.block_out_channels[i]);
        pl.ctx_fold_scratch = ctx_tensor((size_t)3 * UB * fold_max * 2);
        if (pl.ip) {
            const int T = c.ip_adapter_tokens, CD = c.cross_attention_dim;
            int cmax = 0;
            for (int i = 0; i < nl; ++i) cmax = std::max(cmax, c.block_out_channels[i]);
            pl.ip_e = ctx_ip_tensor((size_t)UB * c.ip_adapter_embed_dim * 2);
            pl.ip_proj = ctx_ip_tensor((size_t)UB * T * CD * 2);
            pl.ip_tok = ctx_ip_tensor((size_t)UB * T * CD * 2);
            pl.ip_kv = ctx_ip_tensor((size_t)UB * T * 2 * cmax * 2);
        }
        int t_sin = tensor((size_t)c0 * 4), t_h1 = tensor((size_t)temb * 4), t_emb = tensor((size_t)temb * 4);
        int t_proj = tensor((size_t)u->tproj_total * 4);
        { Op o; o.kind = OP_SINUSOID; o.out = t_sin; o.N = c0; push(o); }
        { Op o; o.kind = OP_GEMV; o.x1 = t_sin; o.out = t_h1; o.N = temb; o.K = c0; o.w = W("time_embedding.linear_1.weight"); o.b = W("time_embedding.linear_1.bias"); push(o); }
        { Op o; o.kind = OP_GEMV; o.x1 = t_h1; o.out = t_emb; o.N = temb; o.K = temb; o.silu_in = 1; o.w = W("time_embedding.linear_2.weight"); o.b = W("time_embedding.linear_2.bias"); push(o); }
        { Op o; o.kind = OP_GEMV; o.x1 = t_emb; o.out = t_proj; o.N = (int)u->tproj_total; o.K = temb; o.silu_in = 1; o.w = W("tproj.weight"); o.b = W("tproj.bias"); push(o); }
        int rh = pl.lh, rw = pl.lw;
        int h;
        if (pl.rep > 1) { prefix_rep = pl.rep; UB /= pl.rep; }
        { Op o; o.kind = OP_CONV_IN; o.x1 = T_LATENTS; o.B = UB; o.Hin = rh; o.Win = rw; o.Cin = c.in_channels; o.N = c0;
          o.w = W("conv_in.weight"); o.b = W("conv_in.bias"); o.out = tensor((size_t)UB * rh * rw * c0 * 2); push(o); h = o.out; }
        const int h_skip = prefix_rep > 1 ? replicate(h, (size_t)UB * rh * rw * c0 * 2, prefix_rep) : h;
        pl.taps["conv_in"] = h_skip;
        int ch = c0;
        std::vector<int> skips{h_skip}, skip_ch{c0}, skip_hw{rh * rw};
        for (int i = 0; i < nl; ++i) {
            const int co = c.block_out_channels[i];
            const std::string bp = "down_blocks." + std::to_string(i) + ".";
            wrapstack.push_back(Wrap{0, i, 0});
            for (int j = 0; j < c.layers_per_block; ++j) {
                wrapstack.push_back(Wrap{0, i, j});
                h = resnet(bp + "resnets." + std::to_string(j) + ".", h, ch, -1, 0, co, rh, rw, t_proj);
                ch = co;
                if (c.attn_levels[i]) h = transformer(bp + "attentions." + std::to_string(j) + ".", h, co, rh, rw);
                wrapstack.pop_back();
                skips.push_back(h); skip_ch.push_back(co); skip_hw.push_back(rh * rw);
            }
            if (i < nl - 1) {
                wrapstack.push_back(Wrap{0, i, c.layers_per_block});
                const std::string d = bp + "downsamplers.0.conv.";
                h = conv3(h, rh, rw, co, co, 2, 0, d + "weight", d + "bias", 0, -1, -1);
                wrapstack.pop_back();
                rh /= 2; rw /= 2;
                skips.push_back(h); skip_ch.push_back(co); skip_hw.push_back(rh * rw);
            }
            wrapstack.pop_back();
            pl.taps["down" + std::to_string(i)] = h;
        }
        wrapstack.push_back(Wrap{1, 0, 0});
// ... 26 lines not shown
                if ((long)UB * skip_hw[i] * skip_ch[i] != pl.cn_count[i]) { error = "ControlNet residual layout"; return; }
                o.res_t[i] = skips[i];
                o.M += (int)pl.cn_count[i];
                stats_of.erase(skips[i]);
            }
            push(o);
        }
        skips.pop_back(); skip_ch.pop_back(); skip_hw.pop_back();
        const int nres = c.layers_per_block + 1;
        for (int i = 0; i < nl; ++i) {
            const int lev = nl - 1 - i, co = c.block_out_channels[lev], rb = nl - 1 - i;
            const std::string bp = "up_blocks." + std::to_string(i) + ".";
            wrapstack.push_back(Wrap{2, rb, 0});
            for (int j = 0; j < nres; ++j) {
                const int s = skips.back(), sc = skip_ch.back();
                skips.pop_back(); skip_ch.pop_back();
                const int rl = nres - 1 - j;
                wrapstack.push_back(Wrap{2, rb, rl});
                h = resnet(bp + "resnets." + std::to_string(j) + ".", h, ch, s, sc, co, rh, rw, t_proj);
                ch = co;
                if (c.attn_levels[lev]) h = transformer(bp + "attentions." + std::to_string(j) + ".", h, co, rh, rw);
                wrapstack.pop_back();
            }
            if (i < nl - 1) {
                wrapstack.push_back(Wrap{2, rb, 0});
                const std::string up = bp + "upsamplers.0.conv.";
                h = conv3(h, rh, rw, co, co, 1, 1, up + "weight", up + "bias", 0, -1, -1);
                wrapstack.pop_back();
                rh *= 2; rw *= 2;
            }
            wrapstack.pop_back();
            pl.taps["up" + std::to_string(i)] = h;
        }
        int g = gn(h, ch, -1, 0, rh * rw, "conv_norm_out.weight", "conv_norm_out.bias", c.norm_eps, 1);
        { Op o; o.kind = OP_CONV_OUT; o.x1 = g; o.out = T_EPS; o.B = UB; o.Hin = rh; o.Win = rw; o.Cin = ch; o.N = c.out_channels;
          o.w = W("conv_out.weight"); o.b = W("conv_out.bias"); push(o); }
    }
};

bool wrap_skipped(const Wrap& w, int branch) {
    const int cache_layer_id = branch % 3, cache_block_id = branch / 3;
    if (w.block_i > cache_block_id || w.type == 1) return true;
    if (w.block_i < cache_block_id) return false;
    return w.type == 0 ? w.layer_i >= cache_layer_id : w.layer_i > cache_layer_id;
}

void op_tensors(const Op& o, int ins[32], int& nin) {
    nin = 0;
    for (int t : {o.x1, o.x2, o.r, o.b2t, o.wt, o.s1, o.s2, o.lnrs, o.slab_t, o.slab_r, o.slab_b2t, o.scx1, o.scx2})
        if (t >= 0) ins[nin++] = t;
    for (int k = 0; k < o.nres; ++k) ins[nin++] = o.res_t[k];
}

void fuse_deferred_reduce(sd_unet* u, Plan& pl) {
    if (getenv("SD_GN_SLAB") && atoi(getenv("SD_GN_SLAB")) == 0) return;
    const int nops = (int)pl.ops.size();
    auto skipped = [&](const Op& o) {
        if (pl.branch < 0) return false;
        for (int k = 0; k < o.nwrap; ++k)
            if (wrap_skipped(o.wraps[k], pl.branch)) return true;
        return false;
    };
    std::vector<int> producer(pl.tensors.size(), -1);
    for (int i = 0; i < nops; ++i)
        if (pl.ops[i].out >= 0) producer[pl.ops[i].out] = i;
    for (int g = 0; g < nops; ++g) {
        Op& G = pl.ops[g];
        if (G.kind != OP_GN || G.out_fp8 || G.x1 < 0 || !sd_groupnorm_slab_ok(G.B, G.HW, G.C1, G.C2, u->cfg.norm_num_groups)) continue;
        const int p = producer[G.x1];
        if (p < 0 || p >= g) continue;
        Op& P = pl.ops[p];
        if (P.kind != OP_CONV3 && !(P.kind == OP_GEMM && P.epi == 0)) continue;
        if (P.splitk <= 1 || P.splitk > 64 || P.aux < 0 || P.dt || P.out_fp8 || P.defer || P.subpix) continue;
        if (P.kind == OP_GEMM && (P.coff || P.ldc_o || P.hm || P.rs >= 0 || P.lnrs >= 0)) continue;
        if ((long)G.B * G.HW != P.M || G.C1 != P.N || skipped(P) != skipped(G)) continue;
        bool first_reader = true;
        for (int i = p + 1; i < g && first_reader; ++i) {
            int ins[32], nin;
            op_tensors(pl.ops[i], ins, nin);
            for (int k = 0; k < nin; ++k)
                if (ins[k] == P.out) first_reader = false;
        }
// ... 161 lines not shown
```

sonicdiffusionbayeslab_amd/csrc/small.hip:

```cpp
#include "common.h"
#include "kernels.h"

namespace {

__device__ __forceinline__ float sinusoid_at(float t, int i, int dim) {
    const int half = dim / 2;
    const int k = i < half ? i : i - half;
    const float f = expf(-9.210340371976184f * (float)k / (float)half);
    const float e = t * f;
    return i < half ? cosf(e) : sinf(e);
}

__global__ void sinusoid_kernel(float t, float* __restrict__ out, int dim) {
    const int i = blockIdx.x * blockDim.x + threadIdx.x;
    if (i >= dim) return;
    out[i] = sinusoid_at(t, i, dim);
}

__global__ void sinusoid_row_kernel(float t, const float* __restrict__ row, float* __restrict__ out, int dim) {
    const int i = blockIdx.x * blockDim.x + threadIdx.x;
    if (i >= dim) return;
    out[i] = sinusoid_at(t, i, dim) + row[i];
}

__global__ __launch_bounds__(256) void gemv_kernel(const float* __restrict__ x, const bf16_t* __restrict__ W,
                                                   const float* __restrict__ b, float* __restrict__ y, int N, int K,
                                                   int silu_in) {
    const int lane = threadIdx.x & 63;
    const int n = blockIdx.x * 4 + (threadIdx.x >> 6);
    if (n >= N) return;
    const bf16_t* wr = W + (long)n * K;
    float acc = 0.f;
    for (int ch = lane; ch < K / 8; ch += 64) {
        const u32x4 w = *(const u32x4*)(wr + ch * 8);
        const f32x4 x0 = *(const f32x4*)(x + ch * 8), x1 = *(const f32x4*)(x + ch * 8 + 4);
        float xv[8] = {x0[0], x0[1], x0[2], x0[3], x1[0], x1[1], x1[2], x1[3]};
        if (silu_in) {
#pragma unroll
            for (int j = 0; j < 8; ++j) xv[j] = silu_f(xv[j]);
        }
        acc += bflo(w[0]) * xv[0] + bfhi(w[0]) * xv[1] + bflo(w[1]) * xv[2] + bfhi(w[1]) * xv[3] +
               bflo(w[2]) * xv[4] + bfhi(w[2]) * xv[5] + bflo(w[3]) * xv[6] + bfhi(w[3]) * xv[7];
    }
    acc = wave_sum(acc);
    if (lane == 0) y[n] = acc + (b ? b[n] : 0.f);
}

template <int CIN, bool IMG = false>
__global__ void conv_in_kernel(const float* __restrict__ x, int Bsrc, const float* __restrict__ Wt,
                               const float* __restrict__ bias, bf16_t* __restrict__ y, int H, int W, int Cout) {
    extern __shared__ __attribute__((aligned(16))) char smem[];
    float* patch = (float*)smem;
    const int yrow = blockIdx.x, b = blockIdx.y;
    const int bs = b % Bsrc;
    const int tid = threadIdx.x;
    const int PW = W + 2;
    for (int i = tid; i < CIN * 3 * PW; i += blockDim.x) {
        const int ci = i / (3 * PW), rem = i - ci * 3 * PW;
        const int dy = rem / PW, px = rem - dy * PW;
        const int iy = yrow + dy - 1, ix = px - 1;
        float v = 0.f;
        if (iy >= 0 && iy < H && ix >= 0 && ix < W) {
            v = x[(((long)bs * CIN + ci) * H + iy) * W + ix];
            if (IMG) v = 2.f * v - 1.f;
        }
        patch[i] = v;
    }
    __syncthreads();
    const int co = tid * 2;
    if (co >= Cout) return;
    float w0[CIN * 9], w1[CIN * 9];
#pragma unroll
    for (int k = 0; k < CIN * 9; ++k) {
        w0[k] = Wt[k * Cout + co];
        w1[k] = Wt[k * Cout + co + 1];
    }
    const float b0 = bias[co], b1 = bias[co + 1];
    bf16_t* yr = y + (((long)b * H + yrow) * W) * Cout + co;
// ... 253 lines not shown
        const bf16_t* src[T];
        bool ok[T];
#pragma unroll
        for (int t = 0; t < T; ++t) {
            const int iy = oy[t] + tap / 3 - 1, ix = ox[t] + tap % 3 - 1;
            ok[t] = valid[t] && iy >= 0 && iy < H && ix >= 0 && ix < W;
            const int cy = min(max(iy, 0), H - 1), cx = min(max(ix, 0), W - 1);
            src[t] = x + (base[t] + (long)cy * W + cx) * Cin + kg * 8;
        }
#pragma unroll 10
        for (int c0 = 0; c0 < Cin; c0 += 32) {
            bf16x8 wf = *(const bf16x8*)(wrow + (tap * Cin + c0) * 2);
            wf = l15 < 4 ? wf : zero8;
#pragma unroll
            for (int t = 0; t < T; ++t) {
                bf16x8 xf = *(const bf16x8*)(src[t] + c0);
                xf = ok[t] ? xf : zero8;
                acc[t] = __builtin_amdgcn_mfma_f32_16x16x32_bf16(wf, xf, acc[t], 0, 0, 0);
            }
        }
    }
    if (kg == 0) {
#pragma unroll
        for (int t = 0; t < T; ++t) {
            if (!valid[t]) continue;
            const long b = base[t] / ((long)H * W);
#pragma unroll
            for (int j = 0; j < 4; ++j)
                if (j < Cout) y[((b * Cout + j) * H + oy[t]) * W + ox[t]] = acc[t][j] + bias[j];
        }
    }
}

__global__ void sched_step_kernel(const float* __restrict__ eps, int cfg, float guidance,
                                  const float* __restrict__ x, const float* __restrict__ m1,
                                  const float* __restrict__ m2, const float* __restrict__ m3,
                                  const float* __restrict__ noise, float* __restrict__ prev,
                                  float* __restrict__ y2, float* __restrict__ m_out, StepCoef c, long n4) {
    const long i = (long)blockIdx.x * blockDim.x + threadIdx.x;
    if (i >= n4) return;
    f32x4 e = ((const f32x4*)eps)[i];
    if (cfg) {
        const f32x4 et = ((const f32x4*)eps)[i + n4];
        e = e + guidance * (et - e);
    }
    const f32x4 xv = ((const f32x4*)x)[i];
    f32x4 p = c.px * xv + c.pe * e;
    if (m1) p += c.p1 * ((const f32x4*)m1)[i];
    if (m2) p += c.p2 * ((const f32x4*)m2)[i];
    if (m3) p += c.p3 * ((const f32x4*)m3)[i];
    if (noise) p += c.pn * ((const f32x4*)noise)[i];
    if (y2) ((f32x4*)y2)[i] = c.yx * xv + c.ye * e;
    if (m_out) ((f32x4*)m_out)[i] = c.mx * xv + c.me * e;
    ((f32x4*)prev)[i] = p;
}

constexpr int RESCALE_THREADS = 512;

__device__ __forceinline__ f32x4 cfg_combine(f32x4 e, f32x4 et, float guidance) { return e + guidance * (et - e); }

__device__ __forceinline__ double wave_sum_f64(double v) {
#pragma unroll
    for (int o = 32; o > 0; o >>= 1) v += __shfl_xor(v, o);
    return v;
}

// ... 218 lines not shown
}

int sd_launch_f32_to_bf16(const float* src, bf16_t* dst, long n, hipStream_t stream) {
    SD_REQUIRE(src && dst && n > 0 && n % 4 == 0, "f32_to_bf16: n=%ld must be a positive multiple of 4", n);
    const long n4 = n / 4;
    hipLaunchKernelGGL(f32_to_bf16_kernel, dim3((unsigned)((n4 + 255) / 256)), dim3(256), 0, stream, src, dst, n4);
    SD_CHECK_HIP(hipGetLastError());
    return 0;
}

int sd_launch_timestep_sinusoid(float t, float* out, int dim, hipStream_t stream) {
    SD_REQUIRE(out && dim > 0 && dim % 2 == 0, "sinusoid: bad dim %d", dim);
    hipLaunchKernelGGL(sinusoid_kernel, dim3((dim + 255) / 256), dim3(256), 0, stream, t, out, dim);
    SD_CHECK_HIP(hipGetLastError());
    return 0;
}

int sd_launch_timestep_sinusoid_row(float t, const float* row, float* out, int dim, hipStream_t stream) {
    SD_REQUIRE(row && out && dim > 0 && dim % 2 == 0, "sinusoid_row: bad operands (dim %d)", dim);
    hipLaunchKernelGGL(sinusoid_row_kernel, dim3((dim + 255) / 256), dim3(256), 0, stream, t, row, out, dim);
    SD_CHECK_HIP(hipGetLastError());
    return 0;
}

int sd_launch_gemv(const float* x, const bf16_t* W, const float* b, float* y, int N, int K, int silu_in,
                   hipStream_t stream) {
    SD_REQUIRE(x && W && y, "gemv: null operand");
    SD_REQUIRE(K % 8 == 0 && N > 0, "gemv: K=%d must be a multiple of 8", K);
    hipLaunchKernelGGL(gemv_kernel, dim3((N + 3) / 4), dim3(256), 0, stream, x, W, b, y, N, K, silu_in);
    SD_CHECK_HIP(hipGetLastError());
    return 0;
}

__global__ void xattn_expand_kernel(const bf16_t* __restrict__ kv, bf16_t* __restrict__ out, int L, int C, int NH,
                                    int col_off, float scale, int S) {
    const int row = blockIdx.x;
    const int j = row % S, h = (row / S) % NH, b = row / (S * NH);
    const int d = C / NH;
    const bf16_t* src = kv + ((long)b * L + (j < L ? j : 0)) * 2 * C + col_off;
    bf16_t* dst = out + (long)row * C;
    for (int c = threadIdx.x * 2; c < C; c += blockDim.x * 2) {
        unsigned v = 0;
        if (j < L && c / d == h) {
            const unsigned u = *(const unsigned*)(src + c);
            v = pack2bf(bflo(u) * scale, bfhi(u) * scale);
        }
        *(unsigned*)(dst + c) = v;
    }
}

__global__ void transpose_bf16_kernel(const bf16_t* __restrict__ src, bf16_t* __restrict__ dst, int R, int Cc, int perm16) {
    __shared__ bf16_t tile[32][33];
    const int b = blockIdx.z, r0 = blockIdx.y * 32, c0 = blockIdx.x * 32;
    const int tx = threadIdx.x & 31, ty = threadIdx.x >> 5;
    const bf16_t* s = src + (long)b * R * Cc;
    bf16_t* d = dst + (long)b * R * Cc;
    for (int i = ty; i < 32; i += 8)
        if (r0 + i < R && c0 + tx < Cc) tile[i][tx] = s[(long)(r0 + i) * Cc + c0 + tx];
    __syncthreads();
    for (int i = ty; i < 32; i += 8)
        if (c0 + i < Cc && r0 + tx < R) {
            int rr = r0 + tx;
            if (perm16) rr = (rr & ~12) | ((rr & 4) << 1) | ((rr & 8) >> 1);
            d[(long)(c0 + i) * R + rr] = tile[tx][i];
        }
}
// ... 151 lines not shown
int sd_launch_conv_in_image(const float* img, const float* Wt, const float* bias, bf16_t* y, int B, int H, int W, int Cout,
                            hipStream_t stream) {
    SD_REQUIRE(img && Wt && bias && y, "conv_in_image: null operand");
    SD_REQUIRE(Cout % 2 == 0 && Cout / 2 <= 1024, "conv_in_image: Cout=%d", Cout);
    SD_REQUIRE(B > 0 && B <= 65535 && H > 0 && W > 0 && W <= 4096, "conv_in_image: B=%d H=%d W=%d", B, H, W);
    const int threads = (Cout / 2 + 63) / 64 * 64;
    const size_t smem = (size_t)3 * 3 * (W + 2) * sizeof(float);
    SD_REQUIRE(smem <= 64 * 1024, "conv_in_image: W=%d needs %zu bytes of LDS (64 KiB per workgroup)", W, smem);
    hipLaunchKernelGGL((conv_in_kernel<3, true>), dim3(H, B), dim3(threads), smem, stream, img, B, Wt, bias, y, H, W, Cout);
    SD_CHECK_HIP(hipGetLastError());
    return 0;
}

int sd_launch_conv_out(const bf16_t* x, const bf16_t* Wp, const float* bias, float* y, int B, int H, int W, int Cin,
                       int Cout, hipStream_t stream) {
    SD_REQUIRE(x && Wp && bias && y, "conv_out: null operand");
    SD_REQUIRE(Cin % 8 == 0 && Cout >= 1 && Cout <= 4, "conv_out: Cin=%d Cout=%d", Cin, Cout);
    const long npix = (long)B * H * W;
    static const bool no_mfma = getenv("SD_CONV_OUT_VALU") != nullptr;
    const size_t smem = (size_t)4 * 9 * Cin * 2;
    if (!no_mfma && Cin % 32 == 0 && smem <= 64 * 1024) {
        static const int tiles = getenv("SD_CONV_OUT_TILES") ? atoi(getenv("SD_CONV_OUT_TILES")) : 1;
        if (tiles == 2)
            hipLaunchKernelGGL(conv_out_mfma_kernel<2>, dim3((unsigned)((npix + 127) / 128)), dim3(256), smem, stream, x, Wp, bias, y,
                               B, H, W, Cin, Cout);
        else
            hipLaunchKernelGGL(conv_out_mfma_kernel<1>, dim3((unsigned)((npix + 63) / 64)), dim3(256), smem, stream, x, Wp, bias, y,
                               B, H, W, Cin, Cout);
        SD_CHECK_HIP(hipGetLastError());
        return 0;
    }
    hipLaunchKernelGGL(conv_out_kernel, dim3((unsigned)((npix + 3) / 4)), dim3(256), 0, stream, x, Wp, bias, y, B, H, W,
                       Cin, Cout);
    SD_CHECK_HIP(hipGetLastError());
    return 0;
}

int sd_launch_sched_step(const float* eps, int cfg, float guidance, const float* x, const float* m1,
                         const float* m2, const float* m3, const float* noise, float* prev, float* y2, float* m_out,
                         StepCoef c, long n, hipStream_t stream) {
    SD_REQUIRE(eps && x && prev, "sched_step: null operand");
    SD_REQUIRE(n > 0 && n % 4 == 0, "sched_step: n=%ld must be a positive multiple of 4", n);
    const long n4 = n / 4;
    hipLaunchKernelGGL(sched_step_kernel, dim3((unsigned)((n4 + 255) / 256)), dim3(256), 0, stream, eps, cfg, guidance,
                       x, m1, m2, m3, noise, prev, y2, m_out, c, n4);
    SD_CHECK_HIP(hipGetLastError());
    return 0;
}

int sd_launch_cfg_rescale_factors(const float* eps, int batch, long n_per_sample, float guidance, float rescale, float* k_out,
                                  hipStream_t stream) {
    SD_REQUIRE(eps && k_out, "cfg_rescale_factors: null operand");
    SD_REQUIRE(batch > 0 && batch <= 65535, "cfg_rescale_factors: batch=%d", batch);
    SD_REQUIRE(n_per_sample >= 4 && n_per_sample % 4 == 0,
               "cfg_rescale_factors: n_per_sample=%ld must be a positive multiple of 4", n_per_sample);
    hipLaunchKernelGGL(cfg_rescale_factors_kernel, dim3(batch), dim3(RESCALE_THREADS), 0, stream, eps, batch,
                       n_per_sample / 4, guidance, rescale, k_out);
    SD_CHECK_HIP(hipGetLastError());
    return 0;
}

int sd_launch_sched_step_rescaled(const float* eps, int cfg, float guidance, const float* x, const float* m1,
                                  const float* m2, const float* m3, const float* noise, float* prev, float* y2,
                                  float* m_out, StepCoef c, const float* k, long n_per_sample, long n, hipStream_t stream) {
    SD_REQUIRE(eps && x && prev && k, "sched_step_rescaled: null operand");
    SD_REQUIRE(n > 0 && n % 4 == 0, "sched_step_rescaled: n=%ld must be a positive multiple of 4", n);
// ... 31 lines not shown
```

sonicdiffusionbayeslab_amd/csrc/unet.hip:

```cpp
#include "model.h"

#include <stdarg.h>
#include <stdio.h>
#include <stdlib.h>

#include <chrono>

static thread_local char g_err[1024] = "";
void sd_set_error(const char* fmt, ...) {
    va_list ap;
    va_start(ap, fmt);
    vsnprintf(g_err, sizeof(g_err), fmt, ap);
    va_end(ap);
}
extern "C" const char* sd_last_error(void) { return g_err; }
extern "C" int sd_abi_version(void) { return 3; }

static void* g_zero_page = nullptr;

namespace sdhip {

int ensure_zero_page() {
    if (g_zero_page) return 0;
    SD_CHECK_HIP(hipMalloc(&g_zero_page, 4096));
    SD_CHECK_HIP(hipMemset(g_zero_page, 0, 4096));
    const unsigned short one_chunk[8] = {0x3F80, 0, 0, 0, 0, 0, 0, 0};
    SD_CHECK_HIP(hipMemcpy((char*)g_zero_page + 256, one_chunk, sizeof(one_chunk), hipMemcpyHostToDevice));
    return 0;
}
const void* zero_page() { return g_zero_page; }

int run_op(sd_unet* u, const Plan& pl, const Op& o, char* ws, const float* latents, int latent_batch, float* eps_out,
           float timestep, hipStream_t stream) {
    auto T = [&](int id) -> char* { return id >= 0 ? ws + pl.tensors[id].off : id == T_EPS ? (char*)eps_out : nullptr; };
    const char* wb = u->dweights;
    switch (o.kind) {
        case OP_SINUSOID:
            if (u->cond_set) return sd_launch_timestep_sinusoid_row(timestep, u->dcond, (float*)T(o.out), o.N, stream);
            return sd_launch_timestep_sinusoid(timestep, (float*)T(o.out), o.N, stream);
        case OP_GEMV:
            return sd_launch_gemv((const float*)T(o.x1), (const bf16_t*)(wb + o.w), (const float*)(wb + o.b),
                                  (float*)T(o.out), o.N, o.K, o.silu_in, stream);
        case OP_CONV_IN:
            if (u->kind == 0 && o.Cin == 9) {
                SD_REQUIRE(u->inpaint_b > 0, "forward: this UNet has in_channels = 9 and no inpainting condition is set "
                                             "(sd_unet_set_inpaint_cond_hw: mask and masked-image latents)");
                SD_REQUIRE(u->inpaint_h == o.Hin && u->inpaint_w == o.Win && o.B % u->inpaint_b == 0,
                           "forward: the inpainting condition was set for batch %d at %dx%d, the forward runs batch %d at %dx%d",
                           u->inpaint_b, u->inpaint_h, u->inpaint_w, o.B, o.Hin, o.Win);
                return sd_launch_conv_in_cond(latents, latent_batch, u->dinpaint, u->inpaint_b, (const float*)(wb + o.w),
                                              (const float*)(wb + o.b), (bf16_t*)T(o.out), o.B, o.Hin, o.Win, o.N, stream);
            }
            if (u->kind == 5) {
                SD_REQUIRE(u->cn_b > 0, "controlnet_forward: no conditioning image is set (sd_controlnet_set_cond_hw)");
                SD_REQUIRE(u->cn_h == o.Hin && u->cn_w == o.Win && o.B % u->cn_b == 0,
                           "controlnet_forward: the conditioning image was set for batch %d at %dx%d, the forward runs batch %d at %dx%d",
                           u->cn_b, u->cn_h, u->cn_w, o.B, o.Hin, o.Win);
                return sd_launch_conv_in_add(latents, latent_batch, u->cn_embed, u->cn_b, (const float*)(wb + o.w),
                                             (const float*)(wb + o.b), (bf16_t*)T(o.out), o.B, o.Hin, o.Win, o.N, stream);
            }
            return sd_launch_conv_in(o.x1 >= 0 ? (const float*)T(o.x1) : latents, o.x1 >= 0 ? o.B : latent_batch,
                                     (const float*)(wb + o.w), (const float*)(wb + o.b), (bf16_t*)T(o.out), o.B, o.Hin,
                                     o.Win, o.Cin, o.N, stream);
        case OP_PQCONV:
            return sd_launch_pqconv(latents, (const float*)(wb + o.w), (const float*)(wb + o.b), (float*)T(o.out), o.B,
                                    o.HW, timestep , stream);
        case OP_SOFTMAX:
            if (o.N > 4096) return sd_launch_softmax_rows_long((bf16_t*)T(o.x1), o.M, o.N, o.scale, stream);
            return sd_launch_softmax_rows((bf16_t*)T(o.x1), o.M, o.N, o.scale, stream);
        case OP_GN: {
            GroupNormArgs a;
            a.x1 = (const bf16_t*)T(o.x1); a.C1 = o.C1; a.x2 = (const bf16_t*)T(o.x2); a.C2 = o.C2;
            a.gamma = (const float*)(wb + o.g); a.beta = (const float*)(wb + o.be);
            a.y = (bf16_t*)T(o.out); a.partial = (float*)T(o.aux);
            a.B = o.B; a.HW = o.HW; a.groups = u->cfg.norm_num_groups; a.nsplit = o.nsplit; a.eps = o.eps; a.silu = o.silu;
            a.out_fp8 = o.out_fp8; a.Cpad = o.Cpad; a.oscale = o.os;
            a.stats1 = (const float*)T(o.s1); a.stats2 = (const float*)T(o.s2);
            if (o.slab_t >= 0) {
                a.slab = (const float*)T(o.slab_t); a.splitk = o.slab_k; a.x1w = (bf16_t*)T(o.x1);
                a.sbias = o.slab_b != NOFF ? (const float*)(wb + o.slab_b) : nullptr;
                a.sbias2 = o.slab_b2t >= 0 ? (const float*)T(o.slab_b2t) + o.slab_b2idx : nullptr;
                a.sR = (const bf16_t*)T(o.slab_r); a.sldr = o.C1;
            }
            return sd_launch_groupnorm(a, stream);
        }
        case OP_CONV3: {
            GemmArgs a;
            a.X = (const bf16_t*)T(o.x1); a.W = (const bf16_t*)(wb + o.w); a.bias = (const float*)(wb + o.b);
            a.bias2 = o.b2t >= 0 ? (const float*)T(o.b2t) + o.b2idx : nullptr;
            a.R = (const bf16_t*)T(o.r); a.ldr = o.N; a.C = (bf16_t*)T(o.out); a.ldc = o.N;
            a.M = o.M; a.N = o.N; a.K = o.K; a.K1 = o.K;
            a.Hin = o.Hin; a.Win = o.Win; a.Cin = o.Cin; a.Hout = o.Hout; a.Wout = o.Wout; a.stride = o.stride; a.up = o.up;
            a.zero_page = g_zero_page; a.splitk = o.splitk; a.slab = (float*)T(o.aux); a.defer_reduce = o.defer;
            if (o.dt) { a.dt = 1; a.wscale = (const float*)(wb + o.wsc); a.xscale_inv = 1.0f / o.xs; }
            a.stats = (float*)T(o.stats);
            a.asym = o.asym;
            if (o.subpix) { a.subpix = 1; a.up = 0; a.w_batch_stride = (long)o.N * 4 * o.Cin; }
            if (o.scw != NOFF) {
                a.Xs1 = (const bf16_t*)T(o.scx1); a.Csc1 = o.scc1; a.Xs2 = (const bf16_t*)T(o.scx2); a.Csc2 = o.scc2;
                a.Wsc = (const bf16_t*)(wb + o.scw); a.ldwsc = o.scc1 + o.scc2;
            }
            return sd_launch_conv3x3(a, stream);
        }
        case OP_GEMM: {
            GemmArgs a;
            a.X = o.wx != NOFF ? (const bf16_t*)(wb + o.wx) : (const bf16_t*)T(o.x1) + o.xoff;
            a.ldx = o.ldx_o ? o.ldx_o : o.K1; a.X2 = (const bf16_t*)T(o.x2); a.ldx2 = o.K - o.K1; a.K1 = o.K1;
            a.W = o.wt >= 0 ? (const bf16_t*)T(o.wt) + o.woff_el : (const bf16_t*)(wb + o.w); a.ldw = o.ldw_o;
            a.bias = o.b != NOFF ? (const float*)(wb + o.b) : nullptr;
            a.R = (const bf16_t*)T(o.r); a.ldr = o.N; a.C = (bf16_t*)T(o.out) + o.coff;
// ... 79 lines not shown
        case OP_BERT_ATTN:
            return sd_launch_bert_attention((const bf16_t*)T(o.x1) + o.qoff, o.ldq, (const bf16_t*)T(o.x2) + o.koff,
                                            (const bf16_t*)T(o.x2) + o.voff, o.ldk, o.key_mask ? u->ir_mask : nullptr,
                                            (bf16_t*)T(o.out), o.ldo, o.B, o.heads, o.Nq, o.Nk, stream);
        case OP_REWARD_HEAD:
            return sd_launch_reward_head((const bf16_t*)T(o.x1), (long)o.Nq * o.N, (const float*)(wb + o.w), (const float*)(wb + o.b),
                                         u->ir.reward_mean, u->ir.reward_std, o.B, o.N, eps_out, u->ir_features, stream);
        case OP_CLIP_ATTN:
            return sd_launch_clip_attention((const bf16_t*)T(o.x1), (bf16_t*)T(o.out), o.B, o.Nq, o.N, o.heads, stream);
        case OP_QGELU:
            if (o.epi) return sd_launch_gelu_erf((bf16_t*)T(o.x1), (long)o.M * o.N, stream);
            return sd_launch_quick_gelu((bf16_t*)T(o.x1), (long)o.M * o.N, stream);
        case OP_VIT_PREP:
            return sd_launch_clip_preprocess((const unsigned char*)latents, o.B, pl.geom, pl.dtab, (unsigned char*)T(o.aux),
                                             (bf16_t*)T(o.out), o.Cin, o.K, nullptr, stream);
        case OP_VIT_EMBED:
            return sd_launch_vit_embed((const bf16_t*)T(o.x1), (const float*)(wb + o.b), (const bf16_t*)(wb + o.g),
                                       (bf16_t*)T(o.out), o.B, o.Nq, o.N, stream);
        case OP_VIT_ATTN:
            return sd_launch_vit_attention((const bf16_t*)T(o.x1), (bf16_t*)T(o.out), o.B, o.Nq, o.N, o.heads, stream);
        case OP_POOL:
            return sd_launch_pool_rows((const bf16_t*)T(o.x1), o.pool_by_ids ? (const int*)latents : nullptr, o.B, o.Nq, o.N, u->eos_id,
                                       (bf16_t*)T(o.out), stream);
        case OP_TO_F32:
            return sd_launch_bf16_to_f32((const bf16_t*)T(o.x1), eps_out, (long)o.M * o.N, stream);
        case OP_CONV_IN_IMG:
            return sd_launch_conv_in_image(latents, (const float*)(wb + o.w), (const float*)(wb + o.b), (bf16_t*)T(o.out), o.B,
                                           o.Hin, o.Win, o.N, stream);
        case OP_ENC_OUT:
            return sd_launch_vae_enc_out((const bf16_t*)T(o.x1), (const bf16_t*)(wb + o.w), (const float*)(wb + o.b),
                                         (const float*)(wb + o.g), (const float*)(wb + o.be), eps_out, o.B, o.Hin, o.Win, o.Cin,
                                         stream);
        case OP_CONV_OUT:
            return sd_launch_conv_out((const bf16_t*)T(o.x1), (const bf16_t*)(wb + o.w), (const float*)(wb + o.b), eps_out,
                                      o.B, o.Hin, o.Win, o.Cin, o.N, stream);
    }
    sd_set_error("unet: unknown op kind %d", o.kind);
    return -1;
}

}

using namespace sdhip;

static sd_unet* new_handle(int kind, const sd_unet_config* cfg) {
    sd_unet* u = new sd_unet();
    u->kind = kind;
    if (cfg) {
        u->cfg = *cfg;
        if (kind != 0) u->cfg.ip_adapter_tokens = u->cfg.ip_adapter_embed_dim = 0;
        if (kind != 0 && kind != 5) u->cfg.time_cond_proj_dim = 0;
        u->debug_taps = getenv("SD_DEBUG_TAPS") != nullptr;
    } else {
        memset(&u->cfg, 0, sizeof(u->cfg));
        u->cfg.num_levels = 1;
    }
    return u;
}

static int check_vae_levels(const sd_unet_config* cfg, const char* who) {
    for (int i = 0; i < cfg->num_levels; ++i) {
        const int c = cfg->block_out_channels[i], cpg = cfg->norm_num_groups ? c / cfg->norm_num_groups : 0;
        SD_REQUIRE(c % 64 == 0 && c % cfg->norm_num_groups == 0 && (cpg >= 8 || cpg == 4),
                   "%s: block_out_channels[%d]=%d must be a multiple of 64 with 4 or >= 8 channels per group", who, i, c);
    }
    return 0;
// ... 308 lines not shown
extern "C" int sd_image_reward_score(sd_unet* u, void* stream, const unsigned char* images, const int* input_ids,
                                     const int* attention_mask, int batch, int text_len, int height, int width, float* rewards,
                                     float* features_or_null, void* workspace, long long workspace_bytes) {
    SD_REQUIRE(u && u->kind == 6, "image_reward: not an ImageReward handle");
    SD_REQUIRE(images && input_ids && attention_mask && rewards && workspace && batch > 0, "image_reward: null argument");
    SD_REQUIRE(text_len >= 1 && text_len <= u->ir.max_text_len, "image_reward: text_len %d (1..max_text_len = %d)", text_len,
               u->ir.max_text_len);
    if (check_image_size(height, width, "image_reward")) return -1;
    Plan* pl;
    int rc = get_plan(u, batch, -1, &pl, text_len, height, width);
    if (rc) return rc;
    if (check_workspace(*pl, "image_reward", workspace, workspace_bytes)) return -1;
    {
        std::vector<int> hm((size_t)batch * text_len);
        SD_CHECK_HIP(hipMemcpyAsync(hm.data(), attention_mask, hm.size() * sizeof(int), hipMemcpyDeviceToHost, (hipStream_t)stream));
        SD_CHECK_HIP(hipStreamSynchronize((hipStream_t)stream));
        if (sd_bert_mask_check(hm.data(), batch, text_len)) return -1;
    }
    u->ir_ids = input_ids; u->ir_mask = attention_mask; u->ir_features = features_or_null;
    rc = run_plan(u, *pl, "image_reward", workspace, workspace_bytes, images, batch, rewards, 0.f, stream);
    u->ir_ids = u->ir_mask = nullptr; u->ir_features = nullptr;
    return rc;
}

extern "C" int sd_clip_score(void* stream, const float* image_embeds, const float* text_embeds, int batch, int dim,
                             float* raw, float* score) {
    return sd_launch_clip_score(image_embeds, text_embeds, batch, dim, raw, score, (hipStream_t)stream);
}

extern "C" void sd_unet_destroy(sd_unet* u) {
    if (!u) return;
    if (u->dweights) (void)hipFree(u->dweights);
    if (u->dcond) (void)hipFree(u->dcond);
    if (u->dinpaint) (void)hipFree(u->dinpaint);
    if (u->tome_choice) (void)hipFree(u->tome_choice);
    if (u->cn_embed) (void)hipFree(u->cn_embed);
    if (u->cn_scratch) (void)hipFree(u->cn_scratch);
    for (auto& kv : u->prep_tabs)
        if (kv.second) (void)hipFree(kv.second);
    delete u;
}

extern "C" int sd_unet_num_params(const sd_unet* u) { return u ? (int)u->params.size() : -1; }

extern "C" int sd_unet_param_info(const sd_unet* u, int index, char* name, int name_cap, long long shape[4], int* ndim) {
    SD_REQUIRE(u && index >= 0 && index < (int)u->params.size(), "param_info: bad index %d", index);
    const ParamSpec& p = u->params[index];
    if (name && name_cap > 0) snprintf(name, name_cap, "%s", p.name.c_str());
    for (int i = 0; i < 4; ++i) shape[i] = i < (int)p.shape.size() ? p.shape[i] : 1;
    if (ndim) *ndim = (int)p.shape.size();
    return 0;
}

extern "C" int sd_unet_load_param(sd_unet* u, const char* name, const float* host_data, long long numel) {
    SD_REQUIRE(u && name && host_data, "load_param: null argument");
    SD_REQUIRE(!u->finalized, "load_param: handle already finalized");
    auto it = u->pindex.find(name);
    SD_REQUIRE(it != u->pindex.end(), "load_param: unknown parameter '%s'", name);
    ParamSpec& p = u->params[it->second];
    SD_REQUIRE(p.numel() == numel, "load_param: '%s' expects %lld elements, got %lld", name, p.numel(), numel);
    p.data.assign(host_data, host_data + numel);
    p.loaded = true;
    return 0;
}

extern "C" int sd_unet_finalize(sd_unet* u) {
// ... 108 lines not shown
                                     unet_batch * NP, C, 0, (hipStream_t)stream))) return rc;
        }
        if (f.c2 >= 0) {
            if ((rc = sd_launch_gemv((const float*)(u->dweights + f.lnu), kexp, nullptr, (float*)(ws + pl.tensors[f.c2].off),
                                     unet_batch * NP, C, 0, (hipStream_t)stream))) return rc;
        }
        {
            if ((rc = gemm(vexp, unet_batch * NP, C, f.wo, C, kexp))) return rc;
            bf16_t* bw_dst = (bf16_t*)(ws + pl.tensors[f.bw].off);
            if ((rc = sd_launch_transpose_bf16(kexp, f.perm ? tmp : bw_dst, unet_batch, NP, C, (hipStream_t)stream, f.perm ? 1 : 0)))
                return rc;
            if (f.perm && (rc = sd_launch_retile32(tmp, bw_dst, unet_batch, C, NP, 32, (hipStream_t)stream))) return rc;
        }
    }
    return 0;
}

extern "C" int sd_unet_set_timestep_cond(sd_unet* u, void* stream, const float* cond) {
    SD_REQUIRE(u && u->unet_like(), "set_timestep_cond: not a UNet or ControlNet handle");
    if (!cond) {
        u->cond_set = false;
        return 0;
    }
    const int d = u->cfg.time_cond_proj_dim, c0 = u->cfg.block_out_channels[0];
    SD_REQUIRE(d > 0, "set_timestep_cond: the UNet has no time_embedding.cond_proj (time_cond_proj_dim = 0)");
    SD_REQUIRE(u->finalized && u->dcond, "set_timestep_cond: parameters not finalized");
    SD_REQUIRE(((uintptr_t)cond & 15) == 0, "set_timestep_cond: cond must be 16-byte aligned");
    const int rc = sd_launch_gemv(cond, (const bf16_t*)(u->dweights + u->woff.at("time_embedding.cond_proj.weight")), nullptr,
                                  u->dcond, c0, d, 0, (hipStream_t)stream);
    if (rc) return rc;
    u->cond_set = true;
    return 0;
}

extern "C" int sd_unet_set_inpaint_cond_hw(sd_unet* u, void* stream, const float* mask, const float* masked_latents, int batch,
                                           int latent_h, int latent_w) {
    SD_REQUIRE(u && u->kind == 0, "set_inpaint_cond: not a UNet handle");
    SD_REQUIRE(u->cfg.in_channels == 9, "set_inpaint_cond: the UNet has in_channels = %d (an inpainting UNet has 9)",
               u->cfg.in_channels);
    if (!mask && !masked_latents) {
        u->inpaint_b = 0;
        return 0;
    }
    SD_REQUIRE(mask && masked_latents && batch > 0, "set_inpaint_cond: null argument");
    SD_REQUIRE((((uintptr_t)mask | (uintptr_t)masked_latents) & 15) == 0, "set_inpaint_cond: operands must be 16-byte aligned");
    if (check_latent_size(u, latent_h, latent_w, "set_inpaint_cond")) return -1;
    const size_t bytes = (size_t)batch * 5 * latent_h * latent_w * sizeof(float);
    if (bytes > u->inpaint_cap) {
        if (u->dinpaint) (void)hipFree(u->dinpaint);
        u->dinpaint = nullptr; u->inpaint_cap = 0; u->inpaint_b = 0;
        SD_CHECK_HIP(hipMalloc((void**)&u->dinpaint, bytes));
        u->inpaint_cap = bytes;
    }
    u->inpaint_b = 0;
    const int rc = sd_launch_inpaint_cond_pack(mask, masked_latents, u->dinpaint, batch, (long)latent_h * latent_w,
                                               (hipStream_t)stream);
    if (rc) return rc;
    u->inpaint_b = batch; u->inpaint_h = latent_h; u->inpaint_w = latent_w;
    return 0;
}

static int check_ip_set(const sd_unet* u, const char* who, int unet_batch, int cache_branch_id, int latent_h, int latent_w) {
    SD_REQUIRE(ip_active(u, unet_batch, cache_branch_id, latent_h, latent_w),
               "%s: the handle runs with an IP-Adapter image prompt, but none is set for batch %d, cache branch %d at %dx%d "
               "(sd_unet_set_ip_adapter_hw after sd_unet_set_context_hw, same workspace; image_embeds = NULL clears the others)",
               who, unet_batch, cache_branch_id < 0 ? -1 : cache_branch_id, latent_h, latent_w);
// ... 201 lines not shown
    u->tome_choice_n = n;
    return 0;
}

extern "C" int sd_unet_forward(sd_unet* u, void* stream, const float* latents, int latent_batch, int unet_batch,
                               float timestep, float* eps_out, void* workspace, long long workspace_bytes,
                               int cache_mode, int cache_branch_id) {
    SD_REQUIRE(u && u->kind == 0, "forward: not a UNet handle");
    return sd_unet_forward_hw(u, stream, latents, latent_batch, unet_batch, u->cfg.sample_size, u->cfg.sample_size, timestep,
                              eps_out, workspace, workspace_bytes, cache_mode, cache_branch_id);
}

extern "C" int sd_unet_forward_hw(sd_unet* u, void* stream, const float* latents, int latent_batch, int unet_batch,
                                  int latent_h, int latent_w, float timestep, float* eps_out, void* workspace,
                                  long long workspace_bytes, int cache_mode, int cache_branch_id) {
    SD_REQUIRE(u && u->kind == 0, "forward: not a UNet handle");
    SD_REQUIRE(latents && eps_out && workspace, "forward: null argument");
    if (check_latent_size(u, latent_h, latent_w, "forward")) return -1;
    SD_REQUIRE(latent_batch > 0 && unet_batch % latent_batch == 0, "forward: unet batch %d not a multiple of latent batch %d",
               unet_batch, latent_batch);
    SD_REQUIRE(cache_mode >= 0 && cache_mode <= 2, "forward: cache_mode %d", cache_mode);
    SD_REQUIRE(cache_mode == SD_CACHE_OFF || cache_branch_id >= 0, "forward: DeepCache modes need cache_branch_id >= 0");
    Plan* pl;
    const int rep = plan_rep(u, latent_batch, unet_batch);
    const int ip = u->ip_keys.empty() ? 0 : 1;
    if (ip && check_ip_set(u, "forward", unet_batch, cache_branch_id, latent_h, latent_w)) return -1;
    const int cn = u->ctrl_res ? 1 : 0;
    if (cn && check_control_set(u, "forward", unet_batch, latent_h, latent_w, cache_mode, cache_branch_id)) return -1;
    u->last_rep = rep; u->last_ip = ip; u->last_cn = cn;
    u->last_h = latent_h; u->last_w = latent_w;
    int rc = get_plan(u, unet_batch, cache_branch_id, &pl, rep, latent_h, latent_w, ip, cn);
    if (rc) return rc;
    if ((rc = ensure_tome_choice(u, pl->tome_choice_bytes, stream))) return rc;
    return run_plan(u, *pl, "forward", workspace, workspace_bytes, latents, latent_batch, eps_out, timestep, stream, cache_mode);
}

extern "C" int sd_unet_set_tome(sd_unet* u, double ratio, int max_downsample) {
    SD_REQUIRE(u && u->kind == 0, "set_tome: not a UNet handle");
    if (!(ratio > 0.0)) {
        SD_REQUIRE(ratio == 0.0, "set_tome: ratio %g (0 .. 0.75)", ratio);
        u->tome_ratio = 0.0; u->tome_max_downsample = 0;
        return 0;
    }
    SD_REQUIRE(ratio <= 0.75, "set_tome: ratio %g (0 .. 0.75: a 2x2 cell has three src tokens)", ratio);
    SD_REQUIRE(max_downsample == 1 || max_downsample == 2, "set_tome: max_downsample %d (1 or 2)", max_downsample);
    SD_REQUIRE(!u->fp8, "set_tome: Token Merging is not built for fp8 handles");
    u->tome_ratio = ratio; u->tome_max_downsample = max_downsample;
    return 0;
}

static int tome_layout(sd_unet* u, const char* who, int latent_h, int latent_w, Plan** pl) {
    SD_REQUIRE(u && u->kind == 0, "%s: not a UNet handle", who);
    if (check_latent_size(u, latent_h, latent_w, who)) return -1;
    return get_plan(u, 1, -1, pl, 1, latent_h, latent_w);
}

extern "C" int sd_unet_tome_block_count_hw(sd_unet* u, int latent_h, int latent_w) {
    Plan* pl;
    if (tome_layout(u, "tome_block_count", latent_h, latent_w, &pl)) return -1;
    return (int)pl->tome.size();
}

extern "C" int sd_unet_tome_block_info_hw(sd_unet* u, int block, int latent_h, int latent_w, int* h, int* w, int* r, long long* choice_off) {
    Plan* pl;
    if (tome_layout(u, "tome_block_info", latent_h, latent_w, &pl)) return -1;
    SD_REQUIRE(block >= 0 && block < (int)pl->tome.size(), "tome_block_info: block %d of %zu", block, pl->tome.size());
    const Plan::TomeBlock& tb = pl->tome[block];
// ... 353 lines not shown
```

sonicdiffusionbayeslab_amd/models.py:

```python
from __future__ import annotations

import hashlib
import math
import os
import time
from dataclasses import dataclass
from typing import Callable, List, Optional, Union

import torch

from . import dist as sdist
from .registry import models_registry
from .schedulers import PNDMConfigStub
from .unet import CACHE_FULL_AND_STORE, CACHE_OFF, CACHE_SKIP, LATENT_CHANNELS, HipUNet2DConditionModel
from .vae import HipVaeDecoder, HipVaeEncoder, VaeConfig, load_vae_state_dict, make_synthetic_vae_state_dict
from .weights import (SD2_CONTEXT_DIM, SD2_HEADS, UNetConfig, check_projection_layout, load_scheduler_config, load_unet_config,
                      load_unet_state_dict, make_synthetic_state_dict, sd2_unet_config)


@dataclass
class StableDiffusionPipelineOutput:
    images: torch.Tensor
    nsfw_content_detected: Optional[list] = None

# ... 910 lines not shown
        if sample_mode not in ("sample", "argmax"):
            raise ValueError(f"sample_mode={sample_mode!r}: 'sample' or 'argmax'")
        t_start, _ = self.img2img_steps(num_inference_steps, strength)
        img = self._image_tensor(image)
        ih, iw = int(img.shape[2]), int(img.shape[3])
        self.check_size(ih, iw)
        for name, v, iv in (("height", height, ih), ("width", width, iw)):
            if v is not None and v != iv:
                raise ValueError(f"{name}={v} disagrees with the image ({ih}x{iw}): the image defines the size of the call")
        n_prompt = 1 if isinstance(prompt, str) else len(prompt) if prompt is not None else int(prompt_embeds.shape[0])
        if img.shape[0] != n_prompt:
            raise ValueError(f"image batch {img.shape[0]} does not match the prompt batch {n_prompt}")
        return img, ih, iw, t_start

    def _img2img_start(self, img, sample_mode, generator, device, first_timestep):
        shape = (img.shape[0], LATENT_CHANNELS, img.shape[2] // self.vae_scale_factor, img.shape[3] // self.vae_scale_factor)
        init = self._image_latents(img.to(device), shape, sample_mode, generator)
        noise = sdist.randn(shape, generator)
        return self.scheduler.add_noise(init, noise, first_timestep), init

    @torch.no_grad()
    def _call_img2img(self, prompt, image, strength, sample_mode, height, width, num_inference_steps, timesteps, sigmas,
                      guidance_scale, negative_prompt, num_images_per_prompt, eta, generator, latents, prompt_embeds,
                      negative_prompt_embeds, output_type, return_dict, guidance_rescale, step_noise, collect_x0,
                      ip_args=(None, None), control=None):
        img, ih, iw, t_start = self._img2img_args(image, strength, sample_mode, prompt, prompt_embeds, height, width, latents,
                                                  num_inference_steps)
        device, batch_size, do_cfg, ctx = self._begin(prompt, ih, iw, guidance_scale, negative_prompt,
                                                      num_images_per_prompt, prompt_embeds, negative_prompt_embeds,
                                                      guidance_rescale, timesteps, sigmas, *ip_args)
        unet_batch = ctx.shape[0]
        self.scheduler.set_timesteps(num_inference_steps, device=device)
        ts_host = list(self.scheduler._timesteps_list)[t_start * self.scheduler.order:]
        dc = self._deepcache
        start, _ = self._img2img_start(img, sample_mode, generator, device, ts_host[0])
        self.img2img_start_latents = start
        latents = self._start_loop(batch_size, device, None, start, ctx, dc.cache_branch_id if dc is not None else -1, control)
        eps = self._eps_buffer(unet_batch, device)
        self._num_timesteps = len(ts_host)
        x0_preds = []
        is_lcm = hasattr(self.scheduler, "config") and "timestep_scaling" in self.scheduler.config

        torch.cuda.synchronize(device)
        start_time = time.time()
        for i, t in enumerate(ts_host):
            mode = CACHE_OFF
            if dc is not None:
                mode = CACHE_FULL_AND_STORE if ts_host.index(t) % dc.cache_interval == 0 else CACHE_SKIP
            self._control_step(i, len(ts_host), latents, unet_batch, t)
            self._tome_step()
            self.unet.forward_latents(latents, unet_batch, float(t), out=eps, cache_mode=mode)
            kw = {}
            if is_lcm and step_noise is not None and i < len(ts_host) - 1:
                kw["noise"] = step_noise[i]
            if do_cfg and guidance_rescale > 0.0:
                kw["guidance_rescale"] = guidance_rescale
            step = self.scheduler.step_fused(eps, guidance_scale, latents, t, cfg=do_cfg, eta=eta, generator=generator, **kw)
            latents, x0 = step[0], step[1]
            if collect_x0:
                x0_preds.append(x0[0:1])
        self._control_end()
        torch.cuda.synchronize(device)
        execution_time = time.time() - start_time
        return self._finish(latents, x0_preds, output_type, return_dict, execution_time)

    @staticmethod
# ... 33 lines not shown
            if tuple(latents.shape) != want:
                raise ValueError(f"latents {tuple(latents.shape)} do not match the image: expected {want}")
        return img, mask, ih, iw, t_start

    def inpaint_prepare(self, image: torch.Tensor, mask: torch.Tensor):
        from . import _lib
        lib = _lib.load()
        self._ensure_unet()
        img = image.to(self.unet.device, torch.float32).contiguous()
        m = mask.to(self.unet.device, torch.float32).contiguous()
        b, _, h, w = img.shape
        if h % 8 or w % 8 or tuple(m.shape) != (b, 1, h, w):
            raise ValueError(f"inpaint_prepare: image {tuple(img.shape)} (sides multiples of 8) and mask {tuple(m.shape)}")
        masked = torch.empty_like(img)
        lmask = torch.empty((b, 1, h // 8, w // 8), dtype=torch.float32, device=img.device)
        _lib.check(lib.sd_inpaint_prepare(_lib.current_stream(), img.data_ptr(), m.data_ptr(), masked.data_ptr(),
                                          lmask.data_ptr(), b, h, w), "sd_inpaint_prepare")
        return masked, lmask

    @torch.no_grad()
    def _call_inpaint(self, prompt, image, mask_image, strength, sample_mode, height, width, num_inference_steps, timesteps,
                      sigmas, guidance_scale, negative_prompt, num_images_per_prompt, eta, generator, latents, prompt_embeds,
                      negative_prompt_embeds, output_type, return_dict, guidance_rescale, step_noise, collect_x0,
                      ip_args=(None, None)):
        img, mask, ih, iw, t_start = self._inpaint_args(image, mask_image, strength, sample_mode, prompt, prompt_embeds, height,
                                                        width, latents, num_inference_steps)
        device, batch_size, do_cfg, ctx = self._begin(prompt, ih, iw, guidance_scale, negative_prompt,
                                                      num_images_per_prompt, prompt_embeds, negative_prompt_embeds,
                                                      guidance_rescale, timesteps, sigmas, *ip_args)
        nine = self.unet_config.in_channels == 9
        unet_batch = ctx.shape[0]
        self.scheduler.set_timesteps(num_inference_steps, device=device)
        ts_host = list(self.scheduler._timesteps_list)[t_start * self.scheduler.order:]
        dc = self._deepcache
        img = img.to(device)
        masked_img, lmask = self.inpaint_prepare(img, mask)
        shape = (batch_size, LATENT_CHANNELS, ih // self.vae_scale_factor, iw // self.vae_scale_factor)
        init = None
        if not (nine and latents is not None):
            init = self._image_latents(img, shape, sample_mode, generator)
        noise = (latents if latents is not None else sdist.randn(shape, generator)).to(device, torch.float32).contiguous()
        if nine:
            masked_latents = self._image_latents(masked_img, shape, sample_mode, generator)
            self.unet.set_inpaint_cond(lmask, masked_latents)
        start = noise if float(strength) == 1.0 else self.scheduler.add_noise(init, noise, ts_host[0])
        self.inpaint_image_latents, self.inpaint_latent_mask = init, lmask
        latents = self._start_loop(batch_size, device, None, start, ctx, dc.cache_branch_id if dc is not None else -1)
        self.img2img_start_latents = latents
        eps = self._eps_buffer(unet_batch, device)
        self._num_timesteps = len(ts_host)
        x0_preds = []
        is_lcm = hasattr(self.scheduler, "config") and "timestep_scaling" in self.scheduler.config

        torch.cuda.synchronize(device)
        start_time = time.time()
        for i, t in enumerate(ts_host):
            mode = CACHE_OFF
            if dc is not None:
                mode = CACHE_FULL_AND_STORE if ts_host.index(t) % dc.cache_interval == 0 else CACHE_SKIP
            self._tome_step()
            self.unet.forward_latents(latents, unet_batch, float(t), out=eps, cache_mode=mode)
            kw = {}
            if is_lcm and step_noise is not None and i < len(ts_host) - 1:
                kw["noise"] = step_noise[i]
            if do_cfg and guidance_rescale > 0.0:
                kw["guidance_rescale"] = guidance_rescale
# ... 22 lines not shown
            raise NotImplementedError("padding_mask_crop is not built (the crop-and-paste of StableDiffusionInpaintPipeline; "
                                      "without it upstream composites nothing in pixel space, and neither does this)")
        n_prompt = 1 if isinstance(prompt, str) else len(prompt) if prompt is not None else \
            int(prompt_embeds.shape[0]) if prompt_embeds is not None else None
        control = self._control_args(control_image, controlnet_conditioning_scale, control_guidance_start,
                                     control_guidance_end, guess_mode, mask_image, n_prompt)
        if mask_image is not None:
            if image is None:
                raise ValueError("mask_image without image: inpainting needs the image the mask refers to")
            return self._call_inpaint(prompt, image, mask_image, 1.0 if strength is STRENGTH_UNSET else strength, sample_mode,
                                      height, width, num_inference_steps, timesteps, sigmas, guidance_scale, negative_prompt,
                                      num_images_per_prompt, eta, generator, latents, prompt_embeds, negative_prompt_embeds,
                                      output_type, return_dict, guidance_rescale, step_noise, collect_x0,
                                      (ip_adapter_image, ip_adapter_image_embeds))
        if self.unet_config.in_channels == 9:
            raise ValueError("this UNet has 9 input channels (an inpainting checkpoint: latents | mask | masked-image latents): "
                             "it runs only with image= and mask_image=, not as " +
                             ("plain image-to-image" if image is not None else "text-to-image"))
        if strength is STRENGTH_UNSET:
            strength = 0.8
        if image is not None:
            return self._call_img2img(prompt, image, strength, sample_mode, height, width, num_inference_steps, timesteps,
                                      sigmas, guidance_scale, negative_prompt, num_images_per_prompt, eta, generator, latents,
                                      prompt_embeds, negative_prompt_embeds, output_type, return_dict, guidance_rescale,
                                      step_noise, collect_x0, (ip_adapter_image, ip_adapter_image_embeds), control)
        device, batch_size, do_cfg, ctx = self._begin(prompt, height, width, guidance_scale, negative_prompt,
                                                      num_images_per_prompt, prompt_embeds, negative_prompt_embeds,
                                                      guidance_rescale, timesteps, sigmas, ip_adapter_image, ip_adapter_image_embeds)
        cfgu = self.unet_config
        unet_batch = ctx.shape[0]

        self.scheduler.set_timesteps(num_inference_steps, device=device)
        ts_host = list(self.scheduler._timesteps_list)
        dc = self._deepcache
        latents = self._start_loop(batch_size, device, generator, latents, ctx, dc.cache_branch_id if dc is not None else -1,
                                   control)
        eps = self._eps_buffer(unet_batch, device)
        self._num_timesteps = len(ts_host)
        x0_preds = []
        is_lcm = hasattr(self.scheduler, "config") and "timestep_scaling" in self.scheduler.config

        torch.cuda.synchronize(device)
        start_time = time.time()
        for i, t in enumerate(ts_host):
            mode = CACHE_OFF
            if dc is not None:
                cur = ts_host.index(t)
                mode = CACHE_FULL_AND_STORE if (cur - 0) % dc.cache_interval == 0 else CACHE_SKIP
            self._control_step(i, len(ts_host), latents, unet_batch, t)
            self._tome_step()
            self.unet.forward_latents(latents, unet_batch, float(t), out=eps, cache_mode=mode)
            kw = {}
            if is_lcm and step_noise is not None and i < len(ts_host) - 1:
                kw["noise"] = step_noise[i]
            if do_cfg and guidance_rescale > 0.0:
                kw["guidance_rescale"] = guidance_rescale
            step = self.scheduler.step_fused(eps, guidance_scale, latents, t, cfg=do_cfg,
                                             eta=eta, generator=generator, **kw)
            if len(step) == 1:
                latents = step[0]
            else:
                latents, x0 = step[0], step[1]
                if collect_x0:
                    x0_preds.append(x0[0:1])
        self._control_end()
        torch.cuda.synchronize(device)
# ... 156 lines not shown
            if t in t_inter:
                latents = self._step_with(self.scheduler_inter, eps, latents, t, unet_batch, do_cfg, guidance_scale,
                                          eta, generator, x0_preds, guidance_rescale)
                _push_history(self.scheduler_main, self._combined(eps, do_cfg, guidance_scale, self.scheduler_inter),
                              latents)
            else:
                latents = self._step_with(self.scheduler_main, eps, latents, t, unet_batch, do_cfg, guidance_scale,
                                          eta, generator, x0_preds, guidance_rescale)
                if _is_dpm(self.scheduler_inter):
                    _push_history(self.scheduler_inter, self._combined(eps, do_cfg, guidance_scale, self.scheduler_main),
                                  latents)
        torch.cuda.synchronize(device)
        return self._finish(latents, x0_preds, output_type, return_dict, time.time() - start_time)


@models_registry.add_to_registry("stable_diffusion_model_skip_timesteps")
class StableDiffusionModelSkipTimesteps(_VariantBase):

    @torch.no_grad()
    def call(self, prompt=None, height=None, width=None, num_inference_steps: int = 50, skip_timesteps=None,
             timesteps=None, sigmas=None, guidance_scale: float = 7.5, negative_prompt=None,
             num_images_per_prompt: int = 1, eta: float = 0.0, generator=None, latents=None, prompt_embeds=None,
             negative_prompt_embeds=None, output_type: str = "pil", return_dict: bool = True,
             guidance_rescale: float = 0.0, ip_adapter_image=None, ip_adapter_image_embeds=None, **kwargs):
        self._refuse_image(kwargs)
        skip = set(int(i) for i in (skip_timesteps or []))
        device, batch_size, do_cfg, ctx = self._begin(prompt, height, width, guidance_scale, negative_prompt,
                                                      num_images_per_prompt, prompt_embeds, negative_prompt_embeds,
                                                      guidance_rescale, timesteps, sigmas, ip_adapter_image, ip_adapter_image_embeds)
        c = self.unet_config
        unet_batch = ctx.shape[0]
        self.scheduler.set_timesteps(num_inference_steps, device=device)
        ts_host = list(self.scheduler._timesteps_list)
        latents = self._start_loop(batch_size, device, generator, latents, ctx, -1)
        eps = self._eps_buffer(unet_batch, device)
        self._num_timesteps = len(ts_host)
        x0_preds = []
        torch.cuda.synchronize(device)
        start_time = time.time()
        for i, t in enumerate(ts_host):
            if i in skip:
                continue
            latents = self._step_with(self.scheduler, eps, latents, t, unet_batch, do_cfg, guidance_scale, eta,
                                      generator, x0_preds, guidance_rescale)
        torch.cuda.synchronize(device)
        return self._finish(latents, x0_preds, output_type, return_dict, time.time() - start_time)


def _fuse_synthetic_lora(sd, seed: int, scale: float, rank: int):
    g = torch.Generator().manual_seed(seed)
    for name in list(sd.keys()):
        if any(k in name for k in (".to_q.weight", ".to_k.weight", ".to_v.weight", ".to_out.0.weight")):
            w = sd[name]
            o, i = w.shape
            a = torch.randn((rank, i), generator=g) / (i ** 0.5)
            b = torch.randn((o, rank), generator=g) * (0.02 / rank ** 0.5)
            sd[name] = (w + scale * (b @ a)).to(torch.bfloat16).float()
```

sonicdiffusionbayeslab_amd/unet.py:

```python
from __future__ import annotations

import ctypes as C
from typing import Dict, Optional

import torch

from . import _lib
from .weights import UNetConfig, param_shapes

CACHE_OFF, CACHE_FULL_AND_STORE, CACHE_SKIP = 0, 1, 2
LATENT_CHANNELS = 4


def _c_config(cfg: UNetConfig, weight_dtype: str = "bf16", fp8_act_scales=(0.0, 0.0)) -> _lib.SdUnetConfigFull:
    c = _lib.SdUnetConfigFull()
    if weight_dtype not in _lib.DTYPES:
        raise ValueError(f"weight_dtype {weight_dtype!r}: one of {sorted(_lib.DTYPES)}")
    c.weight_dtype = _lib.DTYPES[weight_dtype]
    c.fp8_act_scale_norm, c.fp8_act_scale_ff = float(fp8_act_scales[0]), float(fp8_act_scales[1])
    c.sample_size, c.in_channels, c.out_channels = cfg.sample_size, cfg.in_channels, cfg.out_channels
    c.num_levels = len(cfg.block_out_channels)
    for i, v in enumerate(cfg.block_out_channels):
        c.block_out_channels[i] = v
        c.attn_levels[i] = int(cfg.attn_levels[i])
# ... 85 lines not shown
            self._ws_key = None

    def set_context(self, encoder_hidden_states: torch.Tensor, height: Optional[int] = None,
                    width: Optional[int] = None) -> None:
        h, w = self.latent_size(height, width)
        ehs = encoder_hidden_states.to(self.device, torch.float32).contiguous()
        ub = ehs.shape[0]
        if ehs.shape[1] != self.config.context_len or ehs.shape[2] != self.config.cross_attention_dim:
            raise ValueError(f"encoder_hidden_states must be [N,{self.config.context_len},"
                             f"{self.config.cross_attention_dim}], got {tuple(ehs.shape)}")
        ws = self._workspace(ub, h, w)
        _lib.check(self._lib.sd_unet_set_context_hw(self._handle, _lib.current_stream(), ehs.data_ptr(), ub,
                                                    self.cache_branch_id, h, w, self._ws_ptr(ws), ws.numel() - 256),
                   "sd_unet_set_context_hw")
        self._ctx_keepalive = ehs
        self._ctx_key = (encoder_hidden_states.data_ptr(), encoder_hidden_states._version, ub, h, w)

    def set_timestep_cond(self, cond: Optional[torch.Tensor]) -> None:
        if cond is None:
            _lib.check(self._lib.sd_unet_set_timestep_cond(self._handle, _lib.current_stream(), None), "sd_unet_set_timestep_cond")
            self._cond = None
            return
        d = self.config.time_cond_proj_dim
        if d is None:
            raise ValueError("timestep_cond given, but this UNet has no time_embedding.cond_proj (time_cond_proj_dim is None)")
        row = cond.detach().to(self.device, torch.float32).reshape(-1).contiguous()
        if row.numel() != d:
            raise ValueError(f"timestep_cond must be [{d}] or [1, {d}], got {tuple(cond.shape)}")
        if row.data_ptr() % 16:
            row = row.clone()
        _lib.check(self._lib.sd_unet_set_timestep_cond(self._handle, _lib.current_stream(), row.data_ptr()),
                   "sd_unet_set_timestep_cond")
        self._cond = row

    def set_inpaint_cond(self, mask: torch.Tensor, masked_latents: torch.Tensor) -> None:
        if self.config.in_channels != 9:
            raise ValueError(f"set_inpaint_cond: this UNet has in_channels = {self.config.in_channels} (an inpainting UNet has 9)")
        m = mask.detach().to(self.device, torch.float32).contiguous()
        z = masked_latents.detach().to(self.device, torch.float32).contiguous()
        if m.dim() != 4 or z.dim() != 4 or m.shape[1] != 1 or z.shape[1] != LATENT_CHANNELS or m.shape[0] != z.shape[0] \
                or m.shape[2:] != z.shape[2:]:
            raise ValueError(f"set_inpaint_cond: mask [B,1,h,w] and masked_latents [B,{LATENT_CHANNELS},h,w], got "
                             f"{tuple(m.shape)} and {tuple(z.shape)}")
        b, _, h, w = z.shape
        _lib.check(self._lib.sd_unet_set_inpaint_cond_hw(self._handle, _lib.current_stream(), m.data_ptr(), z.data_ptr(), b, h, w),
                   "sd_unet_set_inpaint_cond_hw")
        self._inpaint_key = (b, h, w)

    def clear_inpaint_cond(self) -> None:
        _lib.check(self._lib.sd_unet_set_inpaint_cond_hw(self._handle, _lib.current_stream(), None, None, 0, 0, 0),
                   "sd_unet_set_inpaint_cond_hw")
        self._inpaint_key = None

    def _drop_ip_keys(self) -> None:
        for ub, branch, h, w in self._ip_keys:
            _lib.check(self._lib.sd_unet_set_ip_adapter_hw(self._handle, _lib.current_stream(), None, ub, branch, h, w, 0.0, None, 0),
                       "sd_unet_set_ip_adapter_hw")
        self._ip_keys = set()
        self._ip_call = None

    def set_ip_adapter(self, image_embeds: torch.Tensor, scale: float = 1.0, height: Optional[int] = None,
                       width: Optional[int] = None) -> None:
        e = self.config.ip_adapter_embed_dim
        if e is None:
            raise ValueError("set_ip_adapter: this UNet was built without an IP-Adapter (ip_adapter_embed_dim is None)")
        if isinstance(scale, dict) or not isinstance(scale, (int, float)) or isinstance(scale, bool):
# ... 279 lines not shown
```

Before: 11.64 images/s.

## Precompute timestep embedding table and fuse exit GroupNorm+SiLU into conv_out

Adds a per-run table of time-embedding projections, computed once for all scheduler timesteps as batched GEMVs, so each UNet forward skips the sinusoid and three GEMV ops and reads a precomputed row instead. Separately, the final GroupNorm+SiLU before conv_out now runs in statistics-only mode, and a new fused kernel applies the normalization while loading conv_out inputs, avoiding a full write and read of the normalized activation. This adds device memory for the table and new code paths, both disabled via environment flags.

Result: no change. 11.68 images/s (median of 6 runs) (+0.4%).

```diff
diff --git a/include/sd_hip.h b/include/sd_hip.h
--- a/include/sd_hip.h
+++ b/include/sd_hip.h
@@ -82,6 +82,8 @@
 
 enum { SD_CACHE_OFF = 0, SD_CACHE_FULL_AND_STORE = 1, SD_CACHE_SKIP = 2 };
 
+int sd_unet_set_timesteps(sd_unet* u, void* stream, const float* ts, int n);
+int sd_unet_timestep_rows(const sd_unet* u);
 int sd_unet_forward(sd_unet* u, void* stream, const float* latents, int latent_batch, int unet_batch,
                     float timestep, float* eps_out, void* workspace, long long workspace_bytes, int cache_mode,
                     int cache_branch_id);
@@ -300,6 +302,9 @@
                        const long long* count, int nseg, float scale);
 int sd_op_conv_out(void* stream, const void* x, const void* Wp, const float* bias, float* y, int B, int H, int W,
                    int Cin, int Cout);
+int sd_op_norm_conv_out_applicable(int B, int H, int W, int Cin, int Cout, int groups);
+int sd_op_norm_conv_out(void* stream, const void* x, const float* gamma, const float* beta, const void* Wp, const float* bias,
+                        float* y, int B, int H, int W, int Cin, int Cout, int groups, float eps);
 int sd_op_time_embedding(void* stream, float t, const void* W1, const float* b1, const void* W2, const float* b2,
                          float* scratch, float* temb, int dim_in, int dim);
 int sd_op_timestep_cond(void* stream, float t, const float* cond, const void* Wc, float* row, float* emb, int cond_dim,
diff --git a/sonicdiffusionbayeslab_amd/_lib.py b/sonicdiffusionbayeslab_amd/_lib.py
--- a/sonicdiffusionbayeslab_amd/_lib.py
+++ b/sonicdiffusionbayeslab_amd/_lib.py
@@ -92,6 +92,8 @@
     "sd_unet_workspace_bytes": (_ll, [_vp, _i, _i]),
     "sd_unet_set_context": (_i, [_vp, _vp, _vp, _i, _i, _vp, _ll]),
     "sd_unet_set_timestep_cond": (_i, [_vp, _vp, _vp]),
+    "sd_unet_set_timesteps": (_i, [_vp, _vp, _vp, _i]),
+    "sd_unet_timestep_rows": (_i, [_vp]),
     "sd_unet_forward": (_i, [_vp, _vp, _vp, _i, _i, _f, _vp, _vp, _ll, _i, _i]),
     "sd_unet_workspace_bytes_hw": (_ll, [_vp, _i, _i, _i, _i]),
     "sd_unet_set_context_hw": (_i, [_vp, _vp, _vp, _i, _i, _i, _i, _vp, _ll]),
@@ -187,6 +189,8 @@
     "sd_op_clip_attention": (_i, [_vp, _vp, _vp, _i, _i, _i, _i]),
     "sd_op_conv_in": (_i, [_vp, _vp, _i, _vp, _vp, _vp, _i, _i, _i, _i, _i]),
     "sd_op_conv_out": (_i, [_vp, _vp, _vp, _vp, _vp, _i, _i, _i, _i, _i]),
+    "sd_op_norm_conv_out_applicable": (_i, [_i, _i, _i, _i, _i, _i]),
+    "sd_op_norm_conv_out": (_i, [_vp, _vp, _vp, _vp, _vp, _vp, _vp, _i, _i, _i, _i, _i, _i, _f]),
     "sd_op_time_embedding": (_i, [_vp, _f, _vp, _vp, _vp, _vp, _vp, _vp, _i, _i]),
     "sd_op_timestep_cond": (_i, [_vp, _f, _vp, _vp, _vp, _vp, _i, _i]),
     "sd_op_ln_partials": (_i, [_i, _i, _i]),
diff --git a/sonicdiffusionbayeslab_amd/csrc/common.h b/sonicdiffusionbayeslab_amd/csrc/common.h
--- a/sonicdiffusionbayeslab_amd/csrc/common.h
+++ b/sonicdiffusionbayeslab_amd/csrc/common.h
@@ -50,6 +50,34 @@
 __device__ __forceinline__ float silu_f(float x) {
     return x * __builtin_amdgcn_rcpf(1.0f + __builtin_amdgcn_exp2f(-1.4426950408889634f * x));
 }
+__device__ __forceinline__ void gn_chunk_coeffs(const float* __restrict__ st, const float* __restrict__ gamma,
+                                                const float* __restrict__ beta, int c0, int cpg, float (&sc)[8], float (&sf)[8]) {
+    const int g0 = c0 / cpg, g1 = (c0 + 7) / cpg;
+    const int nb = min(8, (g0 + 1) * cpg - c0);
+    const float m0 = st[g0 * 2], r0 = st[g0 * 2 + 1], m1 = st[g1 * 2], r1 = st[g1 * 2 + 1];
+    const f32x4 ga = *(const f32x4*)(gamma + c0), gb = *(const f32x4*)(gamma + c0 + 4);
+    const f32x4 ba = *(const f32x4*)(beta + c0), bb = *(const f32x4*)(beta + c0 + 4);
+#pragma unroll
+    for (int j = 0; j < 8; ++j) {
+        const float gm = j < 4 ? ga[j & 3] : gb[j & 3], bt = j < 4 ? ba[j & 3] : bb[j & 3];
+        const float mean = j < nb ? m0 : m1, rstd = j < nb ? r0 : r1;
+        sc[j] = rstd * gm;
+        sf[j] = bt - mean * sc[j];
+    }
+}
+template <bool SILU>
+__device__ __forceinline__ void gn_chunk_norm(const u32x4 v, const float (&sc)[8], const float (&sf)[8], float (&f)[8]) {
+    const float x[8] = {bflo(v[0]), bfhi(v[0]), bflo(v[1]), bfhi(v[1]), bflo(v[2]), bfhi(v[2]), bflo(v[3]), bfhi(v[3])};
+#pragma unroll
+    for (int j = 0; j < 8; ++j) {
+        f[j] = x[j] * sc[j] + sf[j];
+        if (SILU) f[j] = silu_f(f[j]);
+    }
+}
+__device__ __forceinline__ u32x4 gn_chunk_pack(const float (&f)[8]) {
+    return u32x4{pack2bf(f[0], f[1]), pack2bf(f[2], f[3]), pack2bf(f[4], f[5]), pack2bf(f[6], f[7])};
+}
+
 __device__ __forceinline__ float gelu_erf_f(float x) {
     const float z = fabsf(x) * 0.70710678118654752f;
     const float t = __builtin_amdgcn_rcpf(__builtin_fmaf(0.47047f, z, 1.0f));
diff --git a/sonicdiffusionbayeslab_amd/csrc/kernels.h b/sonicdiffusionbayeslab_amd/csrc/kernels.h
--- a/sonicdiffusionbayeslab_amd/csrc/kernels.h
+++ b/sonicdiffusionbayeslab_amd/csrc/kernels.h
@@ -102,8 +102,12 @@
     int B = 0, HW = 0, groups = 32, nsplit = 0;
     float eps = 1e-5f;
     int silu = 0;
+    int stats_only = 0;
 };
 int sd_groupnorm_nsplit(int B, int HW);
+inline const float* sd_groupnorm_stats(const float* partial, int B, int nsplit, int groups) {
+    return partial + (long)B * nsplit * groups * 2;
+}
 bool sd_groupnorm_uses_small(int B, int HW, int C1, int C2, int groups);
 bool sd_groupnorm_slab_ok(int B, int HW, int C1, int C2, int groups);
 size_t sd_groupnorm_scratch_bytes(int B, int HW, int groups);
@@ -138,6 +142,9 @@
 int sd_launch_gemv(const float* x, const bf16_t* W, const float* b, float* y, int N, int K, int silu_in,
                    hipStream_t stream);
 int sd_launch_timestep_sinusoid(float t, float* out, int dim, hipStream_t stream);
+int sd_launch_timestep_sinusoid_rows(const float* ts_host, int rows, float* out, int dim, hipStream_t stream);
+int sd_launch_gemv_rows(const float* x, long ldx, const bf16_t* W, const float* b, float* y, long ldy, int N, int K, int silu_in,
+                        int rows, hipStream_t stream);
 int sd_launch_timestep_sinusoid_row(float t, const float* row, float* out, int dim, hipStream_t stream);
 int sd_launch_f32_to_bf16(const float* src, bf16_t* dst, long n, hipStream_t stream);
 int sd_launch_transpose_bf16(const bf16_t* src, bf16_t* dst, int B, int R, int Cc, hipStream_t stream, int perm16 = 0);
@@ -227,6 +234,10 @@
 int sd_launch_conv_out(const bf16_t* x, const bf16_t* Wp , const float* bias, float* y, int B,
                        int H, int W, int Cin, int Cout, hipStream_t stream);
 
+bool sd_norm_conv_out_applicable(int B, int H, int W, int Cin, int Cout, int groups);
+int sd_launch_norm_conv_out(const bf16_t* x, const float* stats, const float* gamma, const float* beta, const bf16_t* Wp,
+                            const float* bias, float* y, int B, int H, int W, int Cin, int Cout, int groups, hipStream_t stream);
+
 struct StepCoef {
     float px, pe, p1, p2, pn;
     float yx, ye;
diff --git a/sonicdiffusionbayeslab_amd/csrc/model.h b/sonicdiffusionbayeslab_amd/csrc/model.h
--- a/sonicdiffusionbayeslab_amd/csrc/model.h
+++ b/sonicdiffusionbayeslab_amd/csrc/model.h
@@ -83,6 +83,8 @@
     float xs = 1.f, os = 1.f;
     int scx1 = -1, scx2 = -1, scc1 = 0, scc2 = 0;
     size_t scw = NOFF;
+    int stats_only = 0, gst = -1;
+    int temb = 0;
     int nres = 0;
     int res_t[MAX_CONTROL_RES];
     int nwrap = 0;
@@ -139,6 +141,7 @@
     struct TomeBlock { int tok, kept, merged, dst_idx, B, h, w, r; long choice_off; };
     std::vector<TomeBlock> tome;
     long tome_choice_bytes = 0;
+    int t_proj = -1;
     std::vector<Tn> tensors;
     std::vector<Op> ops;
     std::vector<char> skipped;
@@ -196,6 +199,12 @@
     long tproj_total = 0;
     float* dcond = nullptr;
     bool cond_set = false;
+    float* temb_tab = nullptr;
+    float* temb_scratch = nullptr;
+    size_t temb_tab_cap = 0, temb_scratch_cap = 0;
+    long temb_stride = 0;
+    std::vector<float> temb_ts;
+    const float* temb_row = nullptr;
     float* dinpaint = nullptr;
     size_t inpaint_cap = 0;
     int inpaint_b = 0, inpaint_h = 0, inpaint_w = 0;
diff --git a/sonicdiffusionbayeslab_amd/csrc/norm.hip b/sonicdiffusionbayeslab_amd/csrc/norm.hip
--- a/sonicdiffusionbayeslab_amd/csrc/norm.hip
+++ b/sonicdiffusionbayeslab_amd/csrc/norm.hip
@@ -153,31 +153,13 @@
     const int prow = tid / g.nchunks, ch = tid - prow * g.nchunks;
     const int c0 = ch * 8;
     const float* st = a.partial + (long)a.B * a.nsplit * a.groups * 2 + (long)b * a.groups * 2;
-    const int g0 = c0 / g.cpg, g1 = (c0 + 7) / g.cpg;
-    const int nb = min(8, (g0 + 1) * g.cpg - c0);
-    const float m0 = st[g0 * 2], r0 = st[g0 * 2 + 1], m1 = st[g1 * 2], r1 = st[g1 * 2 + 1];
     float sc[8], sf[8];
-    {
-        const f32x4 ga = *(const f32x4*)(a.gamma + c0), gb = *(const f32x4*)(a.gamma + c0 + 4);
-        const f32x4 ba = *(const f32x4*)(a.beta + c0), bb = *(const f32x4*)(a.beta + c0 + 4);
-#pragma unroll
-        for (int j = 0; j < 8; ++j) {
-            const float gm = j < 4 ? ga[j & 3] : gb[j & 3], bt = j < 4 ? ba[j & 3] : bb[j & 3];
-            const float mean = j < nb ? m0 : m1, rstd = j < nb ? r0 : r1;
-            sc[j] = rstd * gm;
-            sf[j] = bt - mean * sc[j];
-        }
-    }
+    gn_chunk_coeffs(st, a.gamma, a.beta, c0, g.cpg, sc, sf);
     const int per = (a.HW + a.nsplit - 1) / a.nsplit;
     const int pbeg = split * per, pend = min(a.HW, pbeg + per);
     auto apply = [&](const u32x4 v, long pix) {
-        float f[8] = {bflo(v[0]), bfhi(v[0]), bflo(v[1]), bfhi(v[1]),
-                      bflo(v[2]), bfhi(v[2]), bflo(v[3]), bfhi(v[3])};
-#pragma unroll
-        for (int j = 0; j < 8; ++j) {
-            f[j] = f[j] * sc[j] + sf[j];
-            if (SILU) f[j] = silu_f(f[j]);
-        }
+        float f[8];
+        gn_chunk_norm<SILU>(v, sc, sf, f);
         if (FP8) {
             char* yr = (char*)a.y + pix * a.Cpad;
             const u32x2 o = {pack4fp8(f[0] * a.oscale, f[1] * a.oscale, f[2] * a.oscale, f[3] * a.oscale),
@@ -187,8 +169,7 @@
                 for (int k = g.C; k < a.Cpad; k += 16) *(u32x4*)(yr + k) = u32x4{0u, 0u, 0u, 0u};
             return;
         }
-        u32x4 o = {pack2bf(f[0], f[1]), pack2bf(f[2], f[3]), pack2bf(f[4], f[5]), pack2bf(f[6], f[7])};
-        *(u32x4*)(a.y + pix * g.C + c0) = o;
+        *(u32x4*)(a.y + pix * g.C + c0) = gn_chunk_pack(f);
     };
     const long base = (long)b * a.HW;
     const int rp = g.rows_par;
@@ -655,7 +636,9 @@
 
 int sd_launch_groupnorm(const GroupNormArgs& a, hipStream_t stream) {
     const int C = a.C1 + a.C2;
-    SD_REQUIRE(a.x1 && a.y && a.gamma && a.beta && a.partial, "groupnorm: null operand");
+    SD_REQUIRE(a.x1 && (a.y || a.stats_only) && a.gamma && a.beta && a.partial, "groupnorm: null operand");
+    SD_REQUIRE(!a.stats_only || (!a.slab && !a.out_fp8 && !sd_groupnorm_uses_small(a.B, a.HW, a.C1, a.C2, a.groups)),
+               "groupnorm: statistics only is a mode of the split path (HW=%d C=%d+%d runs the single-launch kernel)", a.HW, a.C1, a.C2);
     SD_REQUIRE(!a.out_fp8 || (a.Cpad >= C && a.Cpad % 128 == 0 && C % 16 == 0 && a.oscale > 0.f),
                "groupnorm fp8 out: Cpad=%d must be a multiple of 128 >= C=%d (C a multiple of 16)", a.Cpad, C);
     SD_REQUIRE(a.C1 % 8 == 0 && a.C2 % 8 == 0 && (a.C2 == 0 || a.x2), "groupnorm: C1=%d C2=%d must be multiples of 8", a.C1, a.C2);
@@ -718,6 +701,10 @@
         hipLaunchKernelGGL(gn_stats_kernel, grid, dim3(g.threads), (g.threads + g.nchunks) * sizeof(float4), stream, a);
         hipLaunchKernelGGL(gn_finalize_kernel, dim3((a.B * a.groups + 3) / 4), dim3(256), 0, stream, a);
     }
+    if (a.stats_only) {
+        SD_CHECK_HIP(hipGetLastError());
+        return 0;
+    }
     if (a.out_fp8) {
         if (a.silu) hipLaunchKernelGGL((gn_apply_kernel<true, true>), grid, dim3(g.threads), 0, stream, a);
         else hipLaunchKernelGGL((gn_apply_kernel<false, true>), grid, dim3(g.threads), 0, stream, a);
diff --git a/sonicdiffusionbayeslab_amd/csrc/ops.hip b/sonicdiffusionbayeslab_amd/csrc/ops.hip
--- a/sonicdiffusionbayeslab_amd/csrc/ops.hip
+++ b/sonicdiffusionbayeslab_amd/csrc/ops.hip
@@ -466,6 +466,31 @@
     return sd_launch_conv_out((const bf16_t*)x, (const bf16_t*)Wp, bias, y, B, H, W, Cin, Cout, (hipStream_t)stream);
 }
 
+extern "C" int sd_op_norm_conv_out_applicable(int B, int H, int W, int Cin, int Cout, int groups) {
+    return sd_norm_conv_out_applicable(B, H, W, Cin, Cout, groups) ? 1 : 0;
+}
+
+extern "C" int sd_op_norm_conv_out(void* stream, const void* x, const float* gamma, const float* beta, const void* Wp,
+                                   const float* bias, float* y, int B, int H, int W, int Cin, int Cout, int groups, float eps) {
+    SD_REQUIRE(B > 0 && H > 0 && W > 0 && Cin > 0 && groups > 0, "sd_op_norm_conv_out: B=%d %dx%d Cin=%d groups=%d", B, H, W, Cin, groups);
+    const int HW = H * W;
+    const bool off = getenv("SD_EXIT_FUSE") && atoi(getenv("SD_EXIT_FUSE")) == 0;
+    const bool fused = !off && sd_norm_conv_out_applicable(B, H, W, Cin, Cout, groups);
+    const size_t gn_bytes = (sd_groupnorm_scratch_bytes(B, HW, groups) + 255) / 256 * 256;
+    char* scratch = (char*)op_scratch(gn_bytes + (fused ? 0 : (size_t)B * HW * Cin * 2));
+    SD_REQUIRE(scratch, "sd_op_norm_conv_out: cannot allocate scratch");
+    GroupNormArgs a;
+    a.x1 = (const bf16_t*)x; a.C1 = Cin; a.gamma = gamma; a.beta = beta; a.B = B; a.HW = HW; a.groups = groups; a.eps = eps;
+    a.silu = 1; a.nsplit = sd_groupnorm_nsplit(B, HW); a.partial = (float*)scratch;
+    a.stats_only = fused ? 1 : 0;
+    a.y = fused ? nullptr : (bf16_t*)(scratch + gn_bytes);
+    if (int rc = sd_launch_groupnorm(a, (hipStream_t)stream)) return rc;
+    if (fused)
+        return sd_launch_norm_conv_out((const bf16_t*)x, sd_groupnorm_stats(a.partial, B, a.nsplit, groups), gamma, beta,
+                                       (const bf16_t*)Wp, bias, y, B, H, W, Cin, Cout, groups, (hipStream_t)stream);
+    return sd_launch_conv_out(a.y, (const bf16_t*)Wp, bias, y, B, H, W, Cin, Cout, (hipStream_t)stream);
+}
+
 extern "C" int sd_op_time_embedding(void* stream, float t, const void* W1, const float* b1, const void* W2,
                                     const float* b2, float* scratch, float* temb, int dim_in, int dim) {
     int rc;
diff --git a/sonicdiffusionbayeslab_amd/csrc/plan.hip b/sonicdiffusionbayeslab_amd/csrc/plan.hip
--- a/sonicdiffusionbayeslab_amd/csrc/plan.hip
+++ b/sonicdiffusionbayeslab_amd/csrc/plan.hip
@@ -90,7 +90,7 @@
     }
     static int pad128(int c) { return (c + 127) / 128 * 128; }
     int gn(int x1, int c1, int x2, int c2, int hw, const std::string& g, const std::string& b, float eps, int silu,
-           bool fq = false) {
+           bool fq = false, bool stats_only = false) {
         Op o; o.kind = OP_GN; o.x1 = x1; o.C1 = c1; o.x2 = x2; o.C2 = c2; o.HW = hw; o.B = UB;
         o.g = W(g); o.be = W(b); o.eps = eps; o.silu = silu;
         o.nsplit = sd_groupnorm_nsplit(UB, hw);
@@ -103,7 +103,8 @@
         if (fq) {
             o.out_fp8 = 1; o.Cpad = pad128(c1 + c2); o.sname = u->act_id(stem(g), u->s_norm); o.os = u->act_scale[o.sname];
             o.out = tensor((size_t)UB * hw * o.Cpad); tscale[o.out] = o.os;
-        } else o.out = tensor((size_t)UB * hw * (c1 + c2) * 2);
+        } else if (stats_only) o.stats_only = 1;
+        else o.out = tensor((size_t)UB * hw * (c1 + c2) * 2);
         push(o);
         return o.out;
     }
@@ -170,6 +171,7 @@
         return o.out;
     }
     bool shortcut_fuse = !(getenv("SD_SHORTCUT_FUSE") && atoi(getenv("SD_SHORTCUT_FUSE")) == 0);
+    bool exit_fuse = !(getenv("SD_EXIT_FUSE") && atoi(getenv("SD_EXIT_FUSE")) == 0);
     int resnet(const std::string& p, int x1, int c1, int x2, int c2, int cout, int rh, int rw, int tproj_t) {
         const int hw = rh * rw, cin = c1 + c2, M = UB * hw;
         const bool fq = u->fp8;
@@ -627,10 +629,11 @@
         }
         int t_sin = tensor((size_t)c0 * 4), t_h1 = tensor((size_t)temb * 4), t_emb = tensor((size_t)temb * 4);
         int t_proj = tensor((size_t)u->tproj_total * 4);
-        { Op o; o.kind = OP_SINUSOID; o.out = t_sin; o.N = c0; push(o); }
-        { Op o; o.kind = OP_GEMV; o.x1 = t_sin; o.out = t_h1; o.N = temb; o.K = c0; o.w = W("time_embedding.linear_1.weight"); o.b = W("time_embedding.linear_1.bias"); push(o); }
-        { Op o; o.kind = OP_GEMV; o.x1 = t_h1; o.out = t_emb; o.N = temb; o.K = temb; o.silu_in = 1; o.w = W("time_embedding.linear_2.weight"); o.b = W("time_embedding.linear_2.bias"); push(o); }
-        { Op o; o.kind = OP_GEMV; o.x1 = t_emb; o.out = t_proj; o.N = (int)u->tproj_total; o.K = temb; o.silu_in = 1; o.w = W("tproj.weight"); o.b = W("tproj.bias"); push(o); }
+        pl.t_proj = t_proj;
+        { Op o; o.kind = OP_SINUSOID; o.temb = 1; o.out = t_sin; o.N = c0; push(o); }
+        { Op o; o.kind = OP_GEMV; o.temb = 1; o.x1 = t_sin; o.out = t_h1; o.N = temb; o.K = c0; o.w = W("time_embedding.linear_1.weight"); o.b = W("time_embedding.linear_1.bias"); push(o); }
+        { Op o; o.kind = OP_GEMV; o.temb = 1; o.x1 = t_h1; o.out = t_emb; o.N = temb; o.K = temb; o.silu_in = 1; o.w = W("time_embedding.linear_2.weight"); o.b = W("time_embedding.linear_2.bias"); push(o); }
+        { Op o; o.kind = OP_GEMV; o.temb = 1; o.x1 = t_emb; o.out = t_proj; o.N = (int)u->tproj_total; o.K = temb; o.silu_in = 1; o.w = W("tproj.weight"); o.b = W("tproj.bias"); push(o); }
         int rh = pl.lh, rw = pl.lw;
         int h;
         if (pl.rep > 1) { prefix_rep = pl.rep; UB /= pl.rep; }
@@ -723,6 +726,14 @@
             wrapstack.pop_back();
             pl.taps["up" + std::to_string(i)] = h;
         }
+        if (exit_fuse && u->kind == 0 && !u->fp8 && sd_norm_conv_out_applicable(UB, rh, rw, ch, c.out_channels, c.norm_num_groups)) {
+            gn(h, ch, -1, 0, rh * rw, "conv_norm_out.weight", "conv_norm_out.bias", c.norm_eps, 1, false, true);
+            const Op G = pl.ops.back();
+            Op o; o.kind = OP_CONV_OUT; o.x1 = h; o.gst = G.aux; o.nsplit = G.nsplit; o.g = G.g; o.be = G.be;
+            o.out = T_EPS; o.B = UB; o.Hin = rh; o.Win = rw; o.Cin = ch; o.N = c.out_channels;
+            o.w = W("conv_out.weight"); o.b = W("conv_out.bias"); push(o);
+            return;
+        }
         int g = gn(h, ch, -1, 0, rh * rw, "conv_norm_out.weight", "conv_norm_out.bias", c.norm_eps, 1);
         { Op o; o.kind = OP_CONV_OUT; o.x1 = g; o.out = T_EPS; o.B = UB; o.Hin = rh; o.Win = rw; o.Cin = ch; o.N = c.out_channels;
           o.w = W("conv_out.weight"); o.b = W("conv_out.bias"); push(o); }
@@ -738,7 +749,7 @@
 
 void op_tensors(const Op& o, int ins[32], int& nin) {
     nin = 0;
-    for (int t : {o.x1, o.x2, o.r, o.b2t, o.wt, o.s1, o.s2, o.lnrs, o.slab_t, o.slab_r, o.slab_b2t, o.scx1, o.scx2})
+    for (int t : {o.x1, o.x2, o.r, o.b2t, o.wt, o.s1, o.s2, o.lnrs, o.slab_t, o.slab_r, o.slab_b2t, o.scx1, o.scx2, o.gst})
         if (t >= 0) ins[nin++] = t;
     for (int k = 0; k < o.nres; ++k) ins[nin++] = o.res_t[k];
 }
diff --git a/sonicdiffusionbayeslab_amd/csrc/small.hip b/sonicdiffusionbayeslab_amd/csrc/small.hip
--- a/sonicdiffusionbayeslab_amd/csrc/small.hip
+++ b/sonicdiffusionbayeslab_amd/csrc/small.hip
@@ -1,5 +1,9 @@
 #include "common.h"
 #include "kernels.h"
+
+#include <stdlib.h>
+
+#include <algorithm>
 
 namespace {
 
@@ -21,6 +25,19 @@
     const int i = blockIdx.x * blockDim.x + threadIdx.x;
     if (i >= dim) return;
     out[i] = sinusoid_at(t, i, dim) + row[i];
+}
+
+constexpr int TS_ROWS_MAX = 64;
+struct TsBlock { float t[TS_ROWS_MAX]; };
+__global__ void sinusoid_rows_kernel(TsBlock ts, float* __restrict__ out, int dim) {
+    const int i = blockIdx.x * blockDim.x + threadIdx.x;
+    if (i >= dim) return;
+    out[(long)blockIdx.y * dim + i] = sinusoid_at(ts.t[blockIdx.y], i, dim);
+}
+
+__device__ __forceinline__ float gemv_chunk(const u32x4 w, const float (&xv)[8]) {
+    return bflo(w[0]) * xv[0] + bfhi(w[0]) * xv[1] + bflo(w[1]) * xv[2] + bfhi(w[1]) * xv[3] +
+           bflo(w[2]) * xv[4] + bfhi(w[2]) * xv[5] + bflo(w[3]) * xv[6] + bfhi(w[3]) * xv[7];
 }
 
 __global__ __launch_bounds__(256) void gemv_kernel(const float* __restrict__ x, const bf16_t* __restrict__ W,
@@ -39,11 +56,53 @@
 #pragma unroll
             for (int j = 0; j < 8; ++j) xv[j] = silu_f(xv[j]);
         }
-        acc += bflo(w[0]) * xv[0] + bfhi(w[0]) * xv[1] + bflo(w[1]) * xv[2] + bfhi(w[1]) * xv[3] +
-               bflo(w[2]) * xv[4] + bfhi(w[2]) * xv[5] + bflo(w[3]) * xv[6] + bfhi(w[3]) * xv[7];
+        acc += gemv_chunk(w, xv);
     }
     acc = wave_sum(acc);
     if (lane == 0) y[n] = acc + (b ? b[n] : 0.f);
+}
+
+template <int R>
+__global__ __launch_bounds__(256) void gemv_rows_kernel(const float* __restrict__ x, long ldx, const bf16_t* __restrict__ W,
+                                                        const float* __restrict__ b, float* __restrict__ y, long ldy, int N, int K,
+                                                        int silu_in, int rows, int nper) {
+    extern __shared__ __attribute__((aligned(16))) char smem[];
+    float* xs = (float*)smem;
+    const int tid = threadIdx.x, lane = tid & 63;
+    const int r0 = blockIdx.y * R, nr = min(R, rows - r0);
+    for (int i = tid; i < nr * (K / 4); i += 256) {
+        const int r = i / (K / 4), c4 = i - r * (K / 4);
+        f32x4 v = *(const f32x4*)(x + (long)(r0 + r) * ldx + c4 * 4);
+        if (silu_in) {
+#pragma unroll
+            for (int j = 0; j < 4; ++j) v[j] = silu_f(v[j]);
+        }
+        *(f32x4*)(xs + r * K + c4 * 4) = v;
+    }
+    __syncthreads();
+    const int n_end = min(N, ((int)blockIdx.x + 1) * nper);
+    for (int n = blockIdx.x * nper + (tid >> 6); n < n_end; n += 4) {
+        const bf16_t* wr = W + (long)n * K;
+        float acc[R];
+#pragma unroll
+        for (int r = 0; r < R; ++r) acc[r] = 0.f;
+        for (int ch = lane; ch < K / 8; ch += 64) {
+            const u32x4 w = *(const u32x4*)(wr + ch * 8);
+#pragma unroll
+            for (int r = 0; r < R; ++r) {
+                if (r >= nr) continue;
+                const f32x4 x0 = *(const f32x4*)(xs + r * K + ch * 8), x1 = *(const f32x4*)(xs + r * K + ch * 8 + 4);
+                const float xv[8] = {x0[0], x0[1], x0[2], x0[3], x1[0], x1[1], x1[2], x1[3]};
+                acc[r] += gemv_chunk(w, xv);
+            }
+        }
+#pragma unroll
+        for (int r = 0; r < R; ++r) {
+            if (r >= nr) continue;
+            const float a = wave_sum(acc[r]);
+            if (lane == 0) y[(long)(r0 + r) * ldy + n] = a + (b ? b[n] : 0.f);
+        }
+    }
 }
 
 template <int CIN, bool IMG = false>
@@ -363,6 +422,111 @@
     }
 }
 
+constexpr int NCO_THREADS = 512, NCO_MAXIT = 8, NCO_LDS_BYTES = 160 * 1024;
+__host__ __device__ inline int nco_pixel_pitch(int C) { return 2 * C + 32; }
+__host__ __device__ inline int nco_weight_pitch(int C) { return 18 * C + ((18 * C) % 128 == 0 ? 32 : 0); }
+__host__ __device__ inline size_t nco_lds_bytes(int W, int C) { return (size_t)4 * nco_weight_pitch(C) + (size_t)3 * W * nco_pixel_pitch(C); }
+
+template <int U>
+__global__ __launch_bounds__(NCO_THREADS) void norm_conv_out_kernel(const bf16_t* __restrict__ x, const float* __restrict__ stats,
+                                                                    const float* __restrict__ gamma, const float* __restrict__ beta,
+                                                                    const bf16_t* __restrict__ Wp, const float* __restrict__ bias,
+                                                                    float* __restrict__ y, int H, int W, int C, int Cout, int groups,
+                                                                    int band, int nbands) {
+    extern __shared__ __attribute__((aligned(16))) char smem[];
+    const int tid = threadIdx.x, lane = tid & 63, wave = tid >> 6;
+    const int K = 9 * C, pitch = nco_pixel_pitch(C), wpitch = nco_weight_pitch(C);
+    char* rows = smem + 4 * wpitch;
+    const int rowbytes = W * pitch;
+    int b, y0;
+    {
+        const int G = gridDim.x, L = blockIdx.x;
+        const int q = G >> 3, r = G & 7, xcd = L & 7, idx = L >> 3;
+        const int v = (xcd < r ? xcd * (q + 1) : r * (q + 1) + (xcd - r) * q) + idx;
+        b = v / nbands;
+        y0 = (v - b * nbands) * band;
+    }
+    const int y1 = min(H, y0 + band);
+    const int nchunks = C >> 3, rows_par = NCO_THREADS / nchunks;
+    const bool active = tid < rows_par * nchunks;
+    const int prow = tid / nchunks, c0 = (tid - prow * nchunks) * 8;
+    float sc[8], sf[8];
+    if (active) gn_chunk_coeffs(stats + (long)b * groups * 2, gamma, beta, c0, C / groups, sc, sf);
+    u32x4 raw[NCO_MAXIT], raw2[NCO_MAXIT];
+    auto load_row = [&](int iy, u32x4 (&r)[NCO_MAXIT]) {
+        if (!active || iy < 0 || iy >= H) return;
+        const bf16_t* src = x + (((long)b * H + iy) * W) * C + c0;
+#pragma unroll
+        for (int it = 0; it < NCO_MAXIT; ++it) {
+            const int px = prow + it * rows_par;
+            if (px < W) r[it] = *(const u32x4*)(src + (long)px * C);
+        }
+    };
+    auto store_row = [&](int iy, const u32x4 (&r)[NCO_MAXIT]) {
+        if (!active || iy < 0 || iy >= H) return;
+        char* dst = rows + (iy % 3) * rowbytes + c0 * 2;
+#pragma unroll
+        for (int it = 0; it < NCO_MAXIT; ++it) {
+            const int px = prow + it * rows_par;
+            if (px < W) {
+                float f[8];
+                gn_chunk_norm<true>(r[it], sc, sf, f);
+                *(u32x4*)(dst + px * pitch) = gn_chunk_pack(f);
+            }
+        }
+    };
+    load_row(y0 - 1, raw);
+    load_row(y0, raw2);
+    for (int i = tid; i < 4 * (K / 8); i += NCO_THREADS) {
+        const int row = i / (K / 8), col = i - row * (K / 8);
+        u32x4 v = {0u, 0u, 0u, 0u};
+        if (row < Cout) v = *(const u32x4*)(Wp + (long)i * 8);
+        *(u32x4*)(smem + row * wpitch + col * 16) = v;
+    }
+    store_row(y0 - 1, raw);
+    load_row(y0 + 1, raw);
+    store_row(y0, raw2);
+    const int l15 = lane & 15, kg = lane >> 4;
+    const bf16x8 zero8 = {0, 0, 0, 0, 0, 0, 0, 0};
+    const char* wrow = smem + (l15 & 3) * wpitch + kg * 16;
+    const int tiles = (W + 15) >> 4;
+    for (int yy = y0; yy < y1; ++yy) {
+        store_row(yy + 1, raw);
+        __syncthreads();
+        if (yy + 1 < y1) load_row(yy + 2, raw);
+        for (int t = wave; t < tiles; t += NCO_THREADS / 64) {
+            const int px = t * 16 + l15;
+            const bool valid = px < W;
+            f32x4 acc = {0.f, 0.f, 0.f, 0.f};
+#pragma unroll 1
+            for (int tap = 0; tap < 9; ++tap) {
+                const int iy = yy + tap / 3 - 1, ix = px + tap % 3 - 1;
+                const bool ok = valid && iy >= 0 && iy < H && ix >= 0 && ix < W;
+                const int cy = min(max(iy, 0), H - 1), cx = min(max(ix, 0), W - 1);
+                const char* src = rows + (cy % 3) * rowbytes + cx * pitch + kg * 16;
+#pragma unroll 1
+                for (int cc = 0; cc < C; cc += 32 * U) {
+                    bf16x8 wf[U], xf[U];
+#pragma unroll
+                    for (int k = 0; k < U; ++k) {
+                        wf[k] = *(const bf16x8*)(wrow + (tap * C + cc + 32 * k) * 2);
+                        xf[k] = *(const bf16x8*)(src + (cc + 32 * k) * 2);
+                    }
+#pragma unroll
+                    for (int k = 0; k < U; ++k)
+                        acc = __builtin_amdgcn_mfma_f32_16x16x32_bf16(l15 < 4 ? wf[k] : zero8, ok ? xf[k] : zero8, acc, 0, 0, 0);
+                }
+            }
+            if (kg == 0 && valid) {
+#pragma unroll
+                for (int j = 0; j < 4; ++j)
+                    if (j < Cout) y[(((long)b * Cout + j) * H + yy) * W + px] = acc[j] + bias[j];
+            }
+        }
+        __syncthreads();
+    }
+}
+
 __global__ void sched_step_kernel(const float* __restrict__ eps, int cfg, float guidance,
                                   const float* __restrict__ x, const float* __restrict__ m1,
                                   const float* __restrict__ m2, const float* __restrict__ m3,
@@ -647,6 +811,31 @@
     return 0;
 }
 
+int sd_launch_timestep_sinusoid_rows(const float* ts_host, int rows, float* out, int dim, hipStream_t stream) {
+    SD_REQUIRE(ts_host && out && rows > 0 && dim > 0 && dim % 2 == 0, "sinusoid_rows: rows=%d dim=%d", rows, dim);
+    for (int r0 = 0; r0 < rows; r0 += TS_ROWS_MAX) {
+        const int nr = std::min(TS_ROWS_MAX, rows - r0);
+        TsBlock ts;
+        for (int r = 0; r < TS_ROWS_MAX; ++r) ts.t[r] = r < nr ? ts_host[r0 + r] : 0.f;
+        hipLaunchKernelGGL(sinusoid_rows_kernel, dim3((dim + 255) / 256, nr), dim3(256), 0, stream, ts, out + (long)r0 * dim, dim);
+    }
+    SD_CHECK_HIP(hipGetLastError());
+    return 0;
+}
+
+int sd_launch_gemv_rows(const float* x, long ldx, const bf16_t* W, const float* b, float* y, long ldy, int N, int K, int silu_in,
+                        int rows, hipStream_t stream) {
+    SD_REQUIRE(x && W && y, "gemv_rows: null operand");
+    SD_REQUIRE(K % 8 == 0 && N > 0 && rows > 0 && rows <= 65535 * 8, "gemv_rows: N=%d K=%d rows=%d (K a multiple of 8)", N, K, rows);
+    SD_REQUIRE(ldx >= K && ldx % 4 == 0 && ldy >= N && ((uintptr_t)x & 15) == 0, "gemv_rows: ldx=%ld ldy=%ld (16-byte aligned rows of x)", ldx, ldy);
+    constexpr int R = 8, NPER = 64;
+    SD_REQUIRE((size_t)R * K * 4 <= 64 * 1024, "gemv_rows: K=%d needs %zu bytes of LDS (64 KiB per workgroup)", K, (size_t)R * K * 4);
+    hipLaunchKernelGGL(gemv_rows_kernel<R>, dim3((N + NPER - 1) / NPER, (rows + R - 1) / R), dim3(256), (size_t)R * K * 4, stream, x, ldx,
+                       W, b, y, ldy, N, K, silu_in, rows, NPER);
+    SD_CHECK_HIP(hipGetLastError());
+    return 0;
+}
+
 __global__ void xattn_expand_kernel(const bf16_t* __restrict__ kv, bf16_t* __restrict__ out, int L, int C, int NH,
                                     int col_off, float scale, int S) {
     const int row = blockIdx.x;
@@ -864,6 +1053,43 @@
     }
     hipLaunchKernelGGL(conv_out_kernel, dim3((unsigned)((npix + 3) / 4)), dim3(256), 0, stream, x, Wp, bias, y, B, H, W,
                        Cin, Cout);
+    SD_CHECK_HIP(hipGetLastError());
+    return 0;
+}
+
+bool sd_norm_conv_out_applicable(int B, int H, int W, int C, int Cout, int groups) {
+    if (B <= 0 || H <= 0 || W <= 0 || C <= 0 || C % 32 != 0 || C / 8 > NCO_THREADS || Cout < 1 || Cout > 4) return false;
+    if (groups <= 0 || groups > 64 || C % groups != 0 || !(C / groups >= 8 || C / groups == 4)) return false;
+    if ((long)H * W > (1L << 24) || sd_groupnorm_uses_small(B, H * W, C, 0, groups)) return false;
+    const int rows_par = NCO_THREADS / (C / 8);
+    if ((W + rows_par - 1) / rows_par > NCO_MAXIT) return false;
+    return nco_lds_bytes(W, C) <= (size_t)NCO_LDS_BYTES;
+}
+
+int sd_launch_norm_conv_out(const bf16_t* x, const float* stats, const float* gamma, const float* beta, const bf16_t* Wp,
+                            const float* bias, float* y, int B, int H, int W, int Cin, int Cout, int groups, hipStream_t stream) {
+    SD_REQUIRE(x && stats && gamma && beta && Wp && bias && y, "norm_conv_out: null operand");
+    SD_REQUIRE(sd_norm_conv_out_applicable(B, H, W, Cin, Cout, groups),
+               "norm_conv_out: B=%d %dx%d Cin=%d Cout=%d groups=%d is not a shape the fused exit takes", B, H, W, Cin, Cout, groups);
+    SD_REQUIRE((((uintptr_t)x | (uintptr_t)Wp | (uintptr_t)gamma | (uintptr_t)beta) & 15) == 0, "norm_conv_out: operands must be 16-byte aligned");
+    const int band = (int)std::max(1L, ((long)B * H + 255) / 256), nbands = (H + band - 1) / band;
+    SD_REQUIRE((long)B * nbands < (1L << 31), "norm_conv_out: too many bands");
+    const size_t smem = nco_lds_bytes(W, Cin);
+    static bool attr_set = false;
+    if (!attr_set) {
+        SD_CHECK_HIP(hipFuncSetAttribute((const void*)norm_conv_out_kernel<10>, hipFuncAttributeMaxDynamicSharedMemorySize, NCO_LDS_BYTES));
+        SD_CHECK_HIP(hipFuncSetAttribute((const void*)norm_conv_out_kernel<2>, hipFuncAttributeMaxDynamicSharedMemorySize, NCO_LDS_BYTES));
+        SD_CHECK_HIP(hipFuncSetAttribute((const void*)norm_conv_out_kernel<1>, hipFuncAttributeMaxDynamicSharedMemorySize, NCO_LDS_BYTES));
+        attr_set = true;
+    }
+    const int steps = Cin / 32;
+    auto go = [&](auto kern) {
+        hipLaunchKernelGGL(kern, dim3((unsigned)(B * nbands)), dim3(NCO_THREADS), smem, stream, x, stats, gamma, beta, Wp, bias, y, H, W,
+                           Cin, Cout, groups, band, nbands);
+    };
+    if (steps % 10 == 0) go(norm_conv_out_kernel<10>);
+    else if (steps % 2 == 0) go(norm_conv_out_kernel<2>);
+    else go(norm_conv_out_kernel<1>);
     SD_CHECK_HIP(hipGetLastError());
     return 0;
 }
diff --git a/sonicdiffusionbayeslab_amd/csrc/unet.hip b/sonicdiffusionbayeslab_amd/csrc/unet.hip
--- a/sonicdiffusionbayeslab_amd/csrc/unet.hip
+++ b/sonicdiffusionbayeslab_amd/csrc/unet.hip
@@ -32,8 +32,12 @@
 
 int run_op(sd_unet* u, const Plan& pl, const Op& o, char* ws, const float* latents, int latent_batch, float* eps_out,
            float timestep, hipStream_t stream) {
-    auto T = [&](int id) -> char* { return id >= 0 ? ws + pl.tensors[id].off : id == T_EPS ? (char*)eps_out : nullptr; };
+    auto T = [&](int id) -> char* {
+        if (id >= 0 && id == pl.t_proj && u->temb_row) return (char*)u->temb_row;
+        return id >= 0 ? ws + pl.tensors[id].off : id == T_EPS ? (char*)eps_out : nullptr;
+    };
     const char* wb = u->dweights;
+    if (o.temb && u->temb_row) return 0;
     switch (o.kind) {
         case OP_SINUSOID:
             if (u->cond_set) return sd_launch_timestep_sinusoid_row(timestep, u->dcond, (float*)T(o.out), o.N, stream);
@@ -76,6 +80,7 @@
             a.B = o.B; a.HW = o.HW; a.groups = u->cfg.norm_num_groups; a.nsplit = o.nsplit; a.eps = o.eps; a.silu = o.silu;
             a.out_fp8 = o.out_fp8; a.Cpad = o.Cpad; a.oscale = o.os;
             a.stats1 = (const float*)T(o.s1); a.stats2 = (const float*)T(o.s2);
+            a.stats_only = o.stats_only;
             if (o.slab_t >= 0) {
                 a.slab = (const float*)T(o.slab_t); a.splitk = o.slab_k; a.x1w = (bf16_t*)T(o.x1);
                 a.sbias = o.slab_b != NOFF ? (const float*)(wb + o.slab_b) : nullptr;
@@ -221,6 +226,12 @@
                                          (const float*)(wb + o.g), (const float*)(wb + o.be), eps_out, o.B, o.Hin, o.Win, o.Cin,
                                          stream);
         case OP_CONV_OUT:
+            if (o.gst >= 0)
+                return sd_launch_norm_conv_out((const bf16_t*)T(o.x1),
+                                               sd_groupnorm_stats((const float*)T(o.gst), o.B, o.nsplit, u->cfg.norm_num_groups),
+                                               (const float*)(wb + o.g), (const float*)(wb + o.be), (const bf16_t*)(wb + o.w),
+                                               (const float*)(wb + o.b), eps_out, o.B, o.Hin, o.Win, o.Cin, o.N,
+                                               u->cfg.norm_num_groups, stream);
             return sd_launch_conv_out((const bf16_t*)T(o.x1), (const bf16_t*)(wb + o.w), (const float*)(wb + o.b), eps_out,
                                       o.B, o.Hin, o.Win, o.Cin, o.N, stream);
     }
@@ -595,6 +606,8 @@
     if (!u) return;
     if (u->dweights) (void)hipFree(u->dweights);
     if (u->dcond) (void)hipFree(u->dcond);
+    if (u->temb_tab) (void)hipFree(u->temb_tab);
+    if (u->temb_scratch) (void)hipFree(u->temb_scratch);
     if (u->dinpaint) (void)hipFree(u->dinpaint);
     if (u->tome_choice) (void)hipFree(u->tome_choice);
     if (u->cn_embed) (void)hipFree(u->cn_embed);
@@ -769,6 +782,55 @@
     u->cond_set = true;
     return 0;
 }
+
+static bool temb_table_off() { return getenv("SD_TEMB_TABLE") && atoi(getenv("SD_TEMB_TABLE")) == 0; }
+
+extern "C" int sd_unet_set_timesteps(sd_unet* u, void* stream, const float* ts, int n) {
+    SD_REQUIRE(u && u->kind == 0, "set_timesteps: not a UNet handle");
+    SD_REQUIRE(u->finalized, "set_timesteps: parameters not finalized");
+    SD_REQUIRE(n >= 0 && n <= 65536 && (ts || n == 0), "set_timesteps: %d timesteps", n);
+    u->temb_ts.clear();
+    if (n == 0 || temb_table_off() || u->cond_set) return 0;
+    std::vector<float> uniq;
+    for (int i = 0; i < n; ++i) {
+        SD_REQUIRE(ts[i] == ts[i], "set_timesteps: timestep %d is NaN", i);
+        if (std::find(uniq.begin(), uniq.end(), ts[i]) == uniq.end()) uniq.push_back(ts[i]);
+    }
+    const int m = (int)uniq.size(), c0 = u->cfg.block_out_channels[0], temb = 4 * c0, N = (int)u->tproj_total;
+    const long stride = ((long)N + 63) / 64 * 64;
+    const size_t tab_bytes = (size_t)m * stride * 4, scr_bytes = (size_t)m * (c0 + 2 * temb) * 4;
+    if (tab_bytes > u->temb_tab_cap) {
+        if (u->temb_tab) (void)hipFree(u->temb_tab);
+        u->temb_tab = nullptr; u->temb_tab_cap = 0;
+        SD_CHECK_HIP(hipMalloc((void**)&u->temb_tab, tab_bytes));
+        u->temb_tab_cap = tab_bytes;
+    }
+    if (scr_bytes > u->temb_scratch_cap) {
+        if (u->temb_scratch) (void)hipFree(u->temb_scratch);
+        u->temb_scratch = nullptr; u->temb_scratch_cap = 0;
+        SD_CHECK_HIP(hipMalloc((void**)&u->temb_scratch, scr_bytes));
+        u->temb_scratch_cap = scr_bytes;
+    }
+    float* sin_ = u->temb_scratch;
+    float* h1 = sin_ + (size_t)m * c0;
+    float* emb = h1 + (size_t)m * temb;
+    const char* wb = u->dweights;
+    auto Wb = [&](const char* k) { return (const bf16_t*)(wb + u->woff.at(k)); };
+    auto Wf = [&](const char* k) { return (const float*)(wb + u->woff.at(k)); };
+    hipStream_t st = (hipStream_t)stream;
+    int rc;
+    if ((rc = sd_launch_timestep_sinusoid_rows(uniq.data(), m, sin_, c0, st))) return rc;
+    if ((rc = sd_launch_gemv_rows(sin_, c0, Wb("time_embedding.linear_1.weight"), Wf("time_embedding.linear_1.bias"), h1, temb, temb,
+                                  c0, 0, m, st))) return rc;
+    if ((rc = sd_launch_gemv_rows(h1, temb, Wb("time_embedding.linear_2.weight"), Wf("time_embedding.linear_2.bias"), emb, temb, temb,
+                                  temb, 1, m, st))) return rc;
+    if ((rc = sd_launch_gemv_rows(emb, temb, Wb("tproj.weight"), Wf("tproj.bias"), u->temb_tab, stride, N, temb, 1, m, st))) return rc;
+    u->temb_stride = stride;
+    u->temb_ts = uniq;
+    return 0;
+}
+
+extern "C" int sd_unet_timestep_rows(const sd_unet* u) { return u ? (int)u->temb_ts.size() : -1; }
 
 extern "C" int sd_unet_set_inpaint_cond_hw(sd_unet* u, void* stream, const float* mask, const float* masked_latents, int batch,
                                            int latent_h, int latent_w) {
@@ -1036,7 +1098,14 @@
     int rc = get_plan(u, unet_batch, cache_branch_id, &pl, rep, latent_h, latent_w, ip, cn);
     if (rc) return rc;
     if ((rc = ensure_tome_choice(u, pl->tome_choice_bytes, stream))) return rc;
-    return run_plan(u, *pl, "forward", workspace, workspace_bytes, latents, latent_batch, eps_out, timestep, stream, cache_mode);
+    u->temb_row = nullptr;
+    if (!u->temb_ts.empty() && !u->cond_set && !temb_table_off()) {
+        const auto it = std::find(u->temb_ts.begin(), u->temb_ts.end(), timestep);
+        if (it != u->temb_ts.end()) u->temb_row = u->temb_tab + (it - u->temb_ts.begin()) * u->temb_stride;
+    }
+    rc = run_plan(u, *pl, "forward", workspace, workspace_bytes, latents, latent_batch, eps_out, timestep, stream, cache_mode);
+    u->temb_row = nullptr;
+    return rc;
 }
 
 extern "C" int sd_unet_set_tome(sd_unet* u, double ratio, int max_downsample) {
diff --git a/sonicdiffusionbayeslab_amd/models.py b/sonicdiffusionbayeslab_amd/models.py
--- a/sonicdiffusionbayeslab_amd/models.py
+++ b/sonicdiffusionbayeslab_amd/models.py
@@ -966,6 +966,7 @@
         unet_batch = ctx.shape[0]
         self.scheduler.set_timesteps(num_inference_steps, device=device)
         ts_host = list(self.scheduler._timesteps_list)[t_start * self.scheduler.order:]
+        self.unet.set_timesteps(ts_host)
         dc = self._deepcache
         start, _ = self._img2img_start(img, sample_mode, generator, device, ts_host[0])
         self.img2img_start_latents = start
@@ -1065,6 +1066,7 @@
         unet_batch = ctx.shape[0]
         self.scheduler.set_timesteps(num_inference_steps, device=device)
         ts_host = list(self.scheduler._timesteps_list)[t_start * self.scheduler.order:]
+        self.unet.set_timesteps(ts_host)
         dc = self._deepcache
         img = img.to(device)
         masked_img, lmask = self.inpaint_prepare(img, mask)
@@ -1153,6 +1155,7 @@
 
         self.scheduler.set_timesteps(num_inference_steps, device=device)
         ts_host = list(self.scheduler._timesteps_list)
+        self.unet.set_timesteps(ts_host)
         dc = self._deepcache
         latents = self._start_loop(batch_size, device, generator, latents, ctx, dc.cache_branch_id if dc is not None else -1,
                                    control)
@@ -1375,6 +1378,7 @@
         unet_batch = ctx.shape[0]
         self.scheduler.set_timesteps(num_inference_steps, device=device)
         ts_host = list(self.scheduler._timesteps_list)
+        self.unet.set_timesteps(ts_host)
         latents = self._start_loop(batch_size, device, generator, latents, ctx, -1)
         eps = self._eps_buffer(unet_batch, device)
         self._num_timesteps = len(ts_host)
diff --git a/sonicdiffusionbayeslab_amd/unet.py b/sonicdiffusionbayeslab_amd/unet.py
--- a/sonicdiffusionbayeslab_amd/unet.py
+++ b/sonicdiffusionbayeslab_amd/unet.py
@@ -141,6 +141,11 @@
         _lib.check(self._lib.sd_unet_set_timestep_cond(self._handle, _lib.current_stream(), row.data_ptr()),
                    "sd_unet_set_timestep_cond")
         self._cond = row
+
+    def set_timesteps(self, timesteps) -> None:
+        ts = [float(t) for t in timesteps]
+        arr = (C.c_float * max(len(ts), 1))(*ts)
+        _lib.check(self._lib.sd_unet_set_timesteps(self._handle, _lib.current_stream(), arr, len(ts)), "sd_unet_set_timesteps")
 
     def set_inpaint_cond(self, mask: torch.Tensor, masked_latents: torch.Tensor) -> None:
         if self.config.in_channels != 9:
```
